# a16z/jolt

Measured on AMD Instinct MI355X. Metric: prover trace cycles/sec (sha3-shaped synthetic trace, sumcheck + HyperKZG hot path), higher is better.
Workload: dtype u256 (BN254 Fr / Fq, 8x u32 Montgomery limbs; integer, bit-exact)

## Files before the change

include/jolt_hip.h:

```cpp
#ifndef JOLT_HIP_H
#define JOLT_HIP_H

#include <stddef.h>
#include <stdint.h>

#ifdef __cplusplus
extern "C" {
#endif

#define JOLT_HIP_ABI_VERSION 1

typedef struct { uint64_t l[4]; } jolt_fr_t;
typedef struct { uint64_t l[4]; } jolt_fq_t;
typedef struct { jolt_fq_t x, y, z; } jolt_g1_t;

typedef struct jolt_ctx jolt_ctx;
typedef struct jolt_table jolt_table;
typedef struct jolt_member jolt_member;
typedef struct jolt_srs jolt_srs;

enum {
    JOLT_OK = 0,
    JOLT_ERR_INVALID_ARG = 1,
    JOLT_ERR_NO_DEVICE = 2,
// ... 297 lines not shown
int32_t jolt_host_lookup_prefix_table(uint32_t prefix, const jolt_fr_t *checkpoints, uint32_t b_len, uint32_t suffix_len, jolt_fr_t *out );
int32_t jolt_host_lookup_table_combine(uint32_t kind, const jolt_fr_t *prefixes, const jolt_fr_t *suffixes, jolt_fr_t *out);
int32_t jolt_host_read_raf_address_create(const jolt_fr_t *gamma, const uint8_t *table_present , int32_t canonical, jolt_read_raf_address **out);
int32_t jolt_host_read_raf_address_destroy(jolt_read_raf_address *h);
int32_t jolt_host_read_raf_address_init_phase(jolt_read_raf_address *h, uint32_t phase, const jolt_fr_t *raf_sums, const jolt_fr_t *suffix_sums);
int32_t jolt_host_read_raf_address_message(jolt_read_raf_address *h, const jolt_fr_t *previous_claim, jolt_fr_t *evals_out );
int32_t jolt_host_read_raf_address_bind(jolt_read_raf_address *h, const jolt_fr_t *challenge, int32_t *phase_done);
int32_t jolt_host_read_raf_address_bind_message(jolt_read_raf_address *h, const jolt_fr_t *challenge, const jolt_fr_t *previous_claim, jolt_fr_t *evals_out );
int32_t jolt_host_read_raf_address_prove_phase(jolt_read_raf_address *h, jolt_fr_t *claim, jolt_round_transcript_fn fn, void *user, jolt_host_transcript *test_transcript,
                                               jolt_fr_t *coeffs_out , jolt_fr_t *challenges_out );
int32_t jolt_host_read_raf_address_v_table(const jolt_read_raf_address *h, uint32_t phase, jolt_fr_t *out );
int32_t jolt_host_read_raf_address_finish(const jolt_read_raf_address *h, jolt_fr_t *table_values , jolt_fr_t *raf_interleaved, jolt_fr_t *raf_identity);

int32_t jolt_r1cs_uniskip_sums(jolt_ctx *ctx, jolt_table *const *inputs, size_t n_inputs, const jolt_table *eq, const jolt_fr_t *a_weights,
                               const jolt_fr_t *b_weights, size_t n_nodes, jolt_fr_t *out);
int32_t jolt_r1cs_materialize(jolt_ctx *ctx, jolt_table *const *inputs, size_t n_inputs, const jolt_fr_t *a_weights, const jolt_fr_t *b_weights,
                              jolt_table **az_out, jolt_table **bz_out);
int32_t jolt_tables_evaluate(jolt_ctx *ctx, jolt_table *const *tables, size_t k, const jolt_fr_t *point, size_t n, jolt_fr_t *out);

int32_t jolt_r1cs_uniskip_sums_small(jolt_ctx *ctx, const jolt_ints *const *inputs, size_t n_inputs, const jolt_table *eq, uint32_t n_streams,
                                     const int64_t *a_weights, const int64_t *b_weights, size_t n_nodes, jolt_fr_t *out);
int32_t jolt_r1cs_materialize_small(jolt_ctx *ctx, const jolt_ints *const *inputs, size_t n_inputs, uint32_t n_streams, const jolt_fr_t *a_weights,
                                    const jolt_fr_t *b_weights, jolt_table **az_out, jolt_table **bz_out);
int32_t jolt_ints_evaluate(jolt_ctx *ctx, const jolt_ints *const *columns, size_t k, const jolt_fr_t *point, size_t n, jolt_fr_t *out);
int32_t jolt_host_small_scalar_dot(const jolt_fr_t *values, const uint64_t *scalars, size_t n, jolt_fr_t *out);

typedef struct jolt_rw_matrix jolt_rw_matrix;
int32_t jolt_rw_matrix_create(jolt_ctx *ctx, const uint64_t *addresses, const uint64_t *pre_values, const uint64_t *post_values, size_t cycles,
                              const jolt_table *inc, const jolt_table *val_init, const jolt_fr_t *tau_low, const jolt_fr_t *gamma,
                              jolt_rw_matrix **out);
int32_t jolt_rw_matrix_create_resident(jolt_ctx *ctx, const jolt_ints *addresses, const jolt_ints *pre_values, const jolt_ints *post_values,
                                       const jolt_table *inc, const jolt_table *val_init, const jolt_fr_t *tau_low, const jolt_fr_t *gamma,
                                       jolt_rw_matrix **out);

int32_t jolt_registers_rw_create(jolt_ctx *ctx, const jolt_onehot *regs, const jolt_ints *rs1_val, const jolt_ints *rs2_val, const jolt_ints *rd_pre,
                                 const jolt_ints *rd_post, const jolt_table *inc, const jolt_fr_t *r_cycle, const jolt_fr_t *gamma, jolt_rw_matrix **out);
int32_t jolt_registers_rw_prove_round(jolt_rw_matrix *m, const jolt_fr_t *bind, jolt_fr_t *evals_out , jolt_fr_t *aux_out );
int32_t jolt_registers_rw_final_values(jolt_rw_matrix *m, jolt_fr_t *out );
int32_t jolt_registers_rw_download(jolt_rw_matrix *m, uint64_t *rows, uint64_t *cols, jolt_fr_t *val, jolt_fr_t *ra, jolt_fr_t *wa, uint64_t *prev, uint64_t *next);
int32_t jolt_rw_matrix_prove_round(jolt_rw_matrix *m, const jolt_fr_t *bind, jolt_fr_t *evals_out , jolt_fr_t *aux_out );
int32_t jolt_rw_matrix_finish(jolt_rw_matrix *m, const jolt_fr_t *bind);
int32_t jolt_rw_matrix_final_values(jolt_rw_matrix *m, jolt_fr_t *out );

typedef struct jolt_key_index jolt_key_index;
int32_t jolt_key_index_create(jolt_ctx *ctx, const jolt_ints *keys, uint64_t k, jolt_key_index **out);
int32_t jolt_key_index_size(const jolt_key_index *index, size_t *cycles, uint64_t *k, uint32_t *items);
int32_t jolt_key_index_pushforward(jolt_ctx *ctx, const jolt_key_index *index, jolt_table *const *weights, size_t n_weights, jolt_table **out);
int32_t jolt_key_index_last_value(jolt_ctx *ctx, const jolt_key_index *index, const jolt_ints *values, const jolt_table *init, jolt_table **out);
int32_t jolt_key_index_destroy(jolt_ctx *ctx, jolt_key_index *index);

int32_t jolt_rw_matrix_hold_row(jolt_rw_matrix *m);
int32_t jolt_rw_matrix_bind(jolt_rw_matrix *m, const jolt_fr_t *bind);
int32_t jolt_rw_matrix_export_row(jolt_rw_matrix *m, size_t cap, uint64_t *cols, uint64_t *prev, uint64_t *next, jolt_fr_t *val, jolt_fr_t *ra, jolt_fr_t *wa ,
                                  jolt_fr_t *inc_out, jolt_fr_t *scalar_out, size_t *n_out);
int32_t jolt_rw_matrix_create_merged(jolt_ctx *ctx, int32_t registers, size_t log_rows, size_t log_k, size_t n, const uint64_t *rows, const uint64_t *cols,
                                     const uint64_t *prev, const uint64_t *next, const jolt_fr_t *val, const jolt_fr_t *ra, const jolt_fr_t *wa, const jolt_fr_t *inc,
                                     const jolt_table *val_init, const jolt_fr_t *w, const jolt_fr_t *scalar, const jolt_fr_t *gamma, jolt_rw_matrix **out);
int32_t jolt_rw_matrix_len(const jolt_rw_matrix *m, size_t *entries);
int32_t jolt_rw_matrix_download(jolt_rw_matrix *m, uint64_t *rows, uint64_t *cols, jolt_fr_t *val, jolt_fr_t *ra, jolt_fr_t *prev, jolt_fr_t *next);
int32_t jolt_rw_matrix_destroy(jolt_rw_matrix *m);

typedef struct jolt_comm jolt_comm;
int32_t jolt_comm_unique_id(const char *rccl_path, uint8_t out[128]);
int32_t jolt_comm_create(jolt_ctx *ctx, const char *rccl_path, const uint8_t unique_id[128], int32_t rank, int32_t world, jolt_comm **out);
int32_t jolt_comm_destroy(jolt_comm *comm);
int32_t jolt_comm_world(const jolt_comm *comm, int32_t *rank, int32_t *world);
int32_t jolt_comm_all_gather_host(jolt_comm *comm, const void *local, size_t bytes, void *gathered);
int32_t jolt_comm_all_gather_device(jolt_comm *comm, const void *d_local, size_t bytes, void *d_gathered);
int32_t jolt_comm_all_gather_table(jolt_comm *comm, const jolt_table *local, size_t n, jolt_table *gathered);
int32_t jolt_comm_gather_round_sums(void *user, const jolt_fr_t *local, size_t count, jolt_fr_t *gathered);
typedef struct jolt_shm jolt_shm;
int32_t jolt_shm_create(const char *name, int32_t rank, int32_t world, size_t max_bytes, jolt_shm **out);
int32_t jolt_shm_create_nonce(const char *name, uint64_t nonce, int32_t rank, int32_t world, size_t max_bytes, jolt_shm **out);
int32_t jolt_shm_destroy(jolt_shm *shm);
int32_t jolt_shm_all_gather(jolt_shm *shm, const void *local, size_t bytes, void *gathered);
int32_t jolt_shm_gather_round_sums(void *user, const jolt_fr_t *local, size_t count, jolt_fr_t *gathered);
int32_t jolt_round_group_pack_tables(jolt_ctx *ctx, jolt_member *const *members, size_t n_members, size_t entries, jolt_table *dst);
int32_t jolt_tail_interleave(jolt_ctx *ctx, const jolt_table *gathered, size_t world, size_t n_tables, size_t entries, jolt_table *dst);
int32_t jolt_round_group_final_values(jolt_ctx *ctx, jolt_member *const *members, size_t n_members, jolt_fr_t *out, size_t capacity);

int32_t jolt_host_hyperkzg_commit(jolt_ctx *ctx, const jolt_srs *srs, const jolt_table *evals, jolt_g1_t *out);
int32_t jolt_host_hyperkzg_open(jolt_ctx *ctx, const jolt_srs *srs, const jolt_table *evals, const jolt_fr_t *point, size_t ell,
                                uint64_t transcript_label, jolt_g1_t *com, jolt_g1_t *w, jolt_fr_t *v, jolt_fr_t *challenges_out);

typedef int32_t (*jolt_open_transcript_fn)(void *user, int32_t phase, const jolt_g1_t *points, size_t n_points, const jolt_fr_t *values, size_t n_values,
                                           jolt_fr_t *challenge_out);
int32_t jolt_host_hyperkzg_open_with_transcript(jolt_ctx *ctx, const jolt_srs *srs, const jolt_table *evals, const jolt_fr_t *point, size_t ell,
                                                jolt_open_transcript_fn fn, void *user, jolt_g1_t *com, jolt_g1_t *w, jolt_fr_t *v, jolt_fr_t *challenges_out);
int32_t jolt_host_hyperkzg_open_with_levels(jolt_ctx *ctx, const jolt_srs *srs, const jolt_table *evals, const jolt_fr_t *point, size_t ell, uint64_t transcript_label,
                                            jolt_open_transcript_fn fn, void *user, const jolt_g1_t *known_levels, size_t n_known, jolt_g1_t *com, jolt_g1_t *w,
                                            jolt_fr_t *v, jolt_fr_t *challenges_out);

int32_t jolt_msm_g1_table_range(jolt_ctx *ctx, const jolt_srs *srs, size_t base_offset, const jolt_table *scalars, size_t scalar_offset,
                                size_t n, jolt_g1_t *out);
enum { JOLT_SCALAR_FR = 3 };
int32_t jolt_msm_g1_window(jolt_ctx *ctx, const jolt_srs *srs, size_t base_offset, int32_t kind, const void *host, size_t n, const jolt_g1_t *acc, jolt_g1_t *out);
int32_t jolt_grid_commit_onehot_range(jolt_ctx *ctx, const jolt_srs *srs, const jolt_onehot *source, size_t cycle_lo, size_t cycle_hi,
                                      jolt_g1_t *out );
int32_t jolt_grid_commit_onehot_classes(jolt_ctx *ctx, const jolt_srs *srs, const jolt_onehot *source, uint32_t shift, jolt_g1_t *out);
int32_t jolt_host_hyperkzg_open_sharded(jolt_ctx *ctx, const jolt_srs *srs, const jolt_table *evals, const jolt_fr_t *point, size_t ell,
                                        uint64_t transcript_label, int32_t rank, int32_t world, jolt_gather_fn gather, void *user,
                                        jolt_g1_t *com, jolt_g1_t *w, jolt_fr_t *v, jolt_fr_t *challenges_out);
int32_t jolt_host_owned_terms(size_t n, size_t block, int32_t rank, int32_t world, size_t *out);
int32_t jolt_srs_setup_from_secret_blocks(jolt_ctx *ctx, const jolt_fr_t *beta, size_t count_global, const jolt_g1_t *g1, size_t block,
                                          int32_t rank, int32_t world, jolt_srs **out);
int32_t jolt_msm_g1_table_blocks(jolt_ctx *ctx, const jolt_srs *srs, const jolt_table *scalars, size_t n, size_t block, int32_t rank,
                                 int32_t world, jolt_g1_t *out);
int32_t jolt_host_hyperkzg_open_sharded_blocks(jolt_ctx *ctx, const jolt_srs *srs, const jolt_table *evals, const jolt_fr_t *point,
                                               size_t ell, uint64_t transcript_label, int32_t rank, int32_t world, size_t block,
                                               jolt_gather_fn gather, void *user, jolt_g1_t *com, jolt_g1_t *w, jolt_fr_t *v,
                                               jolt_fr_t *challenges_out);
int32_t jolt_host_subtree_owned_terms(size_t n, int32_t rank, int32_t world, size_t *out);
int32_t jolt_host_subtree_term_index(size_t slot, int32_t rank, int32_t world, size_t *out);
int32_t jolt_srs_setup_from_secret_subtree(jolt_ctx *ctx, const jolt_fr_t *beta, size_t count_global, const jolt_g1_t *g1, int32_t rank,
                                           int32_t world, jolt_srs **out);
int32_t jolt_msm_g1_table_subtree(jolt_ctx *ctx, const jolt_srs *srs, const jolt_table *scalars, size_t n, int32_t rank, int32_t world,
                                  jolt_g1_t *out);
int32_t jolt_grid_joint_polynomial_subtree(jolt_ctx *ctx, const jolt_onehot *const *sources, size_t n_sources,
                                           const jolt_fr_t *onehot_scalars, jolt_table *const *dense, size_t n_dense,
                                           const jolt_fr_t *dense_scalars, uint32_t log_k, int32_t rank, int32_t world, jolt_table **out);
int32_t jolt_host_hyperkzg_open_subtree(jolt_ctx *ctx, const jolt_srs *srs, const jolt_table *evals, const jolt_fr_t *point, size_t ell,
                                        uint64_t transcript_label, int32_t rank, int32_t world, jolt_gather_fn gather, void *user,
                                        jolt_g1_t *com, jolt_g1_t *w, jolt_fr_t *v, jolt_fr_t *challenges_out);

typedef struct jolt_grid_hint jolt_grid_hint;
int32_t jolt_grid_hint_begin(jolt_ctx *ctx, const jolt_srs *srs, const jolt_onehot *const *sources, size_t n_sources, uint32_t levels, int32_t background,
                             jolt_grid_hint **out);
int32_t jolt_grid_hint_wait(jolt_ctx *ctx, jolt_grid_hint *hint);
int32_t jolt_grid_hint_download(jolt_ctx *ctx, jolt_grid_hint *hint, uint32_t level, jolt_g1_t *out );
int32_t jolt_grid_hint_free(jolt_ctx *ctx, jolt_grid_hint *hint);
int32_t jolt_host_hyperkzg_open_grid(jolt_ctx *ctx, const jolt_srs *srs, const jolt_table *evals, const jolt_fr_t *point, size_t ell, uint64_t transcript_label,
                                     jolt_open_transcript_fn fn, void *user, const jolt_grid_hint *hint, uint32_t levels, const jolt_fr_t *onehot_scalars,
                                     jolt_table *const *dense, size_t n_dense, const jolt_fr_t *dense_scalars, jolt_g1_t *com, jolt_g1_t *w, jolt_fr_t *v,
                                     jolt_fr_t *challenges_out);

typedef struct jolt_stage_op jolt_stage_op;
int32_t jolt_stage_op_num_rounds(const jolt_stage_op *op, size_t *rounds);
int32_t jolt_stage_op_degree(const jolt_stage_op *op, size_t *degree);
int32_t jolt_stage_op_input_claim(jolt_stage_op *op, jolt_fr_t *claim);
int32_t jolt_stage_op_prove_round(jolt_stage_op *op, const jolt_fr_t *bind, size_t round, const jolt_fr_t *previous_claim, jolt_fr_t *coeffs_out, size_t cap,
                                  size_t *n_coeffs);
int32_t jolt_stage_op_finish_rounds(jolt_stage_op *op, const jolt_fr_t *bind);
int32_t jolt_stage_op_output_claims(jolt_stage_op *op, jolt_fr_t *out, size_t cap, size_t *n);
int32_t jolt_stage_op_kept(const jolt_stage_op *op, const char *key, jolt_fr_t *out, size_t cap, size_t *n);
int32_t jolt_stage_op_window(jolt_stage_op *parent, size_t first, size_t n, jolt_stage_op **out);
int32_t jolt_stage_op_destroy(jolt_stage_op *op);

int32_t jolt_stage_spartan_uniskip_sums(jolt_ctx *ctx, const jolt_ints *const *cols, size_t n_cols, uint32_t n_streams, const jolt_fr_t *tau, size_t n_tau,
                                        const int64_t *a_weights, const int64_t *b_weights, size_t n_nodes, jolt_fr_t *sums_out);
int32_t jolt_stage_spartan_remainder_create(jolt_ctx *ctx, const jolt_ints *const *cols, size_t n_cols, uint32_t n_streams, const jolt_fr_t *a_weights,
                                            const jolt_fr_t *b_weights, const jolt_fr_t *tau, size_t n_tau, const jolt_fr_t *scale, jolt_stage_op **out);
int32_t jolt_stage_ram_read_write_create(jolt_ctx *ctx, const jolt_ints *addresses, const jolt_ints *pre_values, const jolt_ints *post_values, const jolt_ints *inc,
                                         const jolt_ints *val_init, const jolt_fr_t *tau_low, const jolt_fr_t *gamma, jolt_stage_op **out);
int32_t jolt_stage_registers_read_write_create(jolt_ctx *ctx, const jolt_onehot *regs, const jolt_ints *rs1_val, const jolt_ints *rs2_val, const jolt_ints *rd_pre,
                                               const jolt_ints *rd_post, const jolt_ints *inc, const jolt_fr_t *r_cycle, const jolt_fr_t *gamma, jolt_stage_op **out);
int32_t jolt_stage_booleanity_address_create(jolt_ctx *ctx, const jolt_onehot *cols, const jolt_fr_t *reference_cycle, size_t n_cycle, const jolt_fr_t *reference_address,
                                             const jolt_fr_t *gamma, jolt_stage_op **out);
int32_t jolt_stage_booleanity_cycle_create(jolt_ctx *ctx, const jolt_onehot *cols, const jolt_fr_t *r_address, const jolt_fr_t *reference_address, const jolt_fr_t *reference_cycle,
                                           size_t n_cycle, const jolt_fr_t *gamma, jolt_stage_op **out);
int32_t jolt_stage_hamming_weight_create(jolt_ctx *ctx, const jolt_onehot *cols, const jolt_fr_t *r_cycle, size_t n_cycle, const jolt_fr_t *r_address,
                                         const jolt_fr_t *virtualization_points, const jolt_fr_t *gamma, jolt_stage_op **out);
int32_t jolt_stage_instruction_read_raf_create(jolt_ctx *ctx, jolt_read_raf *rows, const jolt_onehot *claim_columns, const jolt_fr_t *r_reduction, size_t n_vars,
                                               const jolt_fr_t *gamma, const uint8_t *table_present , uint32_t ra_count, jolt_stage_op **out);
int32_t jolt_stage_bytecode_read_raf_address_create(jolt_ctx *ctx, const jolt_key_index *pc_index, const jolt_fr_t *stage_points , size_t n_vars,
                                                    const jolt_fr_t *stage_values , const jolt_fr_t *gamma, uint64_t first_pc, uint64_t entry_index,
                                                    jolt_stage_op **out);
// ... 22 lines not shown
```

jolt_amd/csrc/capi.hip:

```cpp
#include <algorithm>
#include <chrono>
#include <cstdlib>
#include <type_traits>

#include "host_mirror.hpp"
#include "ints.hpp"
#include "member.hpp"
#include "poly_kernels.hip.h"
#include "small_round.hip.h"
#include "onehot_kernels.hip.h"

using namespace jolt;

extern "C" const char* jolt_status_string(int32_t s) {
    switch (s) {
        case JOLT_OK: return "ok";
        case JOLT_ERR_INVALID_ARG: return "invalid argument";
        case JOLT_ERR_NO_DEVICE: return "no usable gfx950 device";
        case JOLT_ERR_OOM: return "out of device memory";
        case JOLT_ERR_HIP: return "HIP runtime error";
        case JOLT_ERR_SIZE_MISMATCH: return "size mismatch";
        case JOLT_ERR_UNSUPPORTED: return "unsupported descriptor";
        case JOLT_ERR_NOT_FULLY_BOUND: return "member not fully bound";
        case JOLT_ERR_ROUND_CHECK: return "round check failed";
// ... 13 lines not shown

extern "C" int32_t jolt_ctx_create(int32_t device_id, void* stream, jolt_ctx** out) {
    if (!out) return JOLT_ERR_INVALID_ARG;
    *out = nullptr;
    int count = 0;
    if (hipGetDeviceCount(&count) != hipSuccess || count <= 0 || device_id < 0 || device_id >= count) return JOLT_ERR_NO_DEVICE;
    hipDeviceProp_t prop;
    if (hipGetDeviceProperties(&prop, device_id) != hipSuccess) return JOLT_ERR_NO_DEVICE;
    if (std::strncmp(prop.gcnArchName, "gfx950", 6) != 0) return JOLT_ERR_NO_DEVICE;
    if (hipSetDevice(device_id) != hipSuccess) return JOLT_ERR_NO_DEVICE;
    jolt_ctx* ctx = new (std::nothrow) jolt_ctx();
    if (!ctx) return JOLT_ERR_OOM;
    ctx->device = device_id;
    if (const char* fr_ = std::getenv("JOLT_FUSE_RATIO")) ctx->fuse_ratio = (size_t)std::max(0, std::atoi(fr_));
    if (const char* tp = std::getenv("JOLT_TAIL_PAIRS")) { if (std::atoll(tp) > 0) ctx->tail_pairs = (size_t)std::atoll(tp); }
    if (const char* ft = std::getenv("JOLT_FUSE_TAIL")) ctx->fuse_tail = std::atoi(ft) != 0;
    if (const char* rt = std::getenv("JOLT_ROUND_TRACE")) ctx->round_trace = std::atoi(rt) != 0;
    if (const char* gf = std::getenv("JOLT_GRID_FLOOR")) { if (std::atoi(gf) > 0) ctx->grid_floor = (size_t)std::atoi(gf); }
    if (const char* gm = std::getenv("JOLT_GRID_MULT")) { if (std::atoi(gm) > 0) ctx->grid_mult = (size_t)std::atoi(gm); }
    if (const char* ss = std::getenv("JOLT_SERIAL_STREAMS")) ctx->serial_streams = std::atoi(ss) != 0;
    if (const char* ll = std::getenv("JOLT_LAZY_LDS")) ctx->lazy_lds = std::atoi(ll) != 0;
    if (const char* rp = std::getenv("JOLT_UNIFORM_ROWS_PAIRS")) { if (std::atoll(rp) > 0) ctx->uniform_rows_pairs = (size_t)std::atoll(rp); }
    ctx->num_cus = prop.multiProcessorCount > 0 ? prop.multiProcessorCount : 256;
    if (prop.sharedMemPerBlock > 0) ctx->max_lds_per_block = prop.sharedMemPerBlock;
    if (const char* ml = std::getenv("JOLT_MSM_LDS_SORT")) ctx->msm_lds_sort = std::atoi(ml) != 0;
    if (const char* pe = std::getenv("JOLT_POOL")) ctx->pool_enabled = std::atoi(pe) != 0;
    if (const char* la = std::getenv("JOLT_MSM_LANES")) ctx->msm_lanes = std::max(1, std::min(4, std::atoi(la)));
    if (stream) {
        ctx->stream = (hipStream_t)stream;
    } else {
        if (hipStreamCreateWithFlags(&ctx->stream, hipStreamNonBlocking) != hipSuccess) { delete ctx; return JOLT_ERR_HIP; }
        ctx->own_stream = true;
    }
    if (hipEventCreate(&ctx->ev_begin) != hipSuccess || hipEventCreate(&ctx->ev_end) != hipSuccess) { delete ctx; return JOLT_ERR_HIP; }
    int32_t s = jolt_internal_ensure_scratch(ctx, 4096 * 8, 1024);
    if (s == JOLT_OK) {
        ctx->round_cap = 1024;
        if (hipHostMalloc((void**)&ctx->h_round, ctx->round_cap * sizeof(Fr), hipHostMallocMapped | hipHostMallocCoherent) != hipSuccess ||
            hipHostMalloc((void**)&ctx->h_flag, 64, hipHostMallocMapped | hipHostMallocCoherent) != hipSuccess ||
            hipMalloc((void**)&ctx->d_counters, kTicketWords * sizeof(uint32_t)) != hipSuccess ||
            hipMalloc((void**)&ctx->d_round, ctx->round_cap * sizeof(Fr)) != hipSuccess ||
            hipMemset(ctx->d_counters, 0, kTicketWords * sizeof(uint32_t)) != hipSuccess)
            s = JOLT_ERR_HIP;
        else
            *ctx->h_flag = 0;
        for (int k = 0; k < 3 && s == JOLT_OK; ++k)
            if (hipStreamCreateWithFlags(&ctx->side[k], hipStreamNonBlocking) != hipSuccess) s = JOLT_ERR_HIP;
        if (s == JOLT_OK && hipEventCreateWithFlags(&ctx->ev_fork, hipEventDisableTiming) != hipSuccess) s = JOLT_ERR_HIP;
        for (int k = 0; k < 3 && s == JOLT_OK; ++k)
            if (hipEventCreateWithFlags(&ctx->ev_join[k], hipEventDisableTiming) != hipSuccess) s = JOLT_ERR_HIP;
    }
    if (s != JOLT_OK) { jolt_ctx_destroy(ctx); return s; }
    *out = ctx;
    return JOLT_OK;
}


extern "C" int32_t jolt_ctx_destroy(jolt_ctx* ctx) {
    if (!ctx) return JOLT_OK;
    (void)hipSetDevice(ctx->device);
    (void)jolt_internal_join_side_writers(ctx);
    (void)hipStreamSynchronize(ctx->stream);
    for (int k = 0; k < 3; ++k) if (ctx->side[k]) { (void)hipStreamSynchronize(ctx->side[k]); (void)hipStreamDestroy(ctx->side[k]); }
    if (ctx->ev_fork) (void)hipEventDestroy(ctx->ev_fork);
    for (int k = 0; k < 3; ++k) if (ctx->ev_join[k]) (void)hipEventDestroy(ctx->ev_join[k]);
    (void)jolt_internal_pool_trim(ctx);
    for (auto& kv : ctx->pool_live) (void)hipFree(kv.first);
    ctx->pool_live.clear();
    if (ctx->d_partials) (void)hipFree(ctx->d_partials);
    if (ctx->d_results) (void)hipFree(ctx->d_results);
    if (ctx->h_results) (void)hipHostFree(ctx->h_results);
    if (ctx->h_round) (void)hipHostFree(ctx->h_round);
    if (ctx->h_flag) (void)hipHostFree(ctx->h_flag);
    if (ctx->d_counters) (void)hipFree(ctx->d_counters);
    if (ctx->d_round) (void)hipFree(ctx->d_round);
    for (int k = 0; k < 4; ++k) {
        if (ctx->msm_ws[k]) (void)hipFree(ctx->msm_ws[k]);
        if (ctx->msm_host[k]) (void)hipHostFree(ctx->msm_host[k]);
    }
    if (ctx->msm_batch_stream) { (void)hipStreamSynchronize(ctx->msm_batch_stream); (void)hipStreamDestroy(ctx->msm_batch_stream); }
    if (ctx->hint_stream) { (void)hipStreamSynchronize(ctx->hint_stream); (void)hipStreamDestroy(ctx->hint_stream); }
    if (ctx->msm_batch_ws) (void)hipFree(ctx->msm_batch_ws);
    if (ctx->msm_aux_stream) { (void)hipStreamSynchronize(ctx->msm_aux_stream); (void)hipStreamDestroy(ctx->msm_aux_stream); }
    for (auto& pair : ctx->ev_aux) for (hipEvent_t e : pair) if (e) (void)hipEventDestroy(e);
    if (ctx->msm_batch_host) (void)hipHostFree(ctx->msm_batch_host);
    if (ctx->ev_begin) (void)hipEventDestroy(ctx->ev_begin);
    for (hipEvent_t e : ctx->ev_fx)
        if (e) (void)hipEventDestroy(e);
    if (ctx->copy_stream) { (void)hipStreamSynchronize(ctx->copy_stream); (void)hipStreamDestroy(ctx->copy_stream); }
    if (ctx->ev_copy_fork) (void)hipEventDestroy(ctx->ev_copy_fork);
    if (ctx->ev_end) (void)hipEventDestroy(ctx->ev_end);
    if (ctx->own_stream) (void)hipStreamDestroy(ctx->stream);
    delete ctx;
    return JOLT_OK;
}

extern "C" int32_t jolt_ctx_synchronize(jolt_ctx* ctx) {
    if (!ctx) return JOLT_ERR_INVALID_ARG;
    JOLT_TRY(jolt_internal_join_side_writers(ctx));
    for (int k = 0; k < 3; ++k) if (ctx->side[k]) JOLT_HIP_TRY(ctx, hipStreamSynchronize(ctx->side[k]));
    if (ctx->hint_stream) JOLT_HIP_TRY(ctx, hipStreamSynchronize(ctx->hint_stream));
    JOLT_HIP_TRY(ctx, hipStreamSynchronize(ctx->stream));
    return JOLT_OK;
}
extern "C" int32_t jolt_ctx_bind_thread(jolt_ctx* ctx) {
    if (!ctx) return JOLT_ERR_INVALID_ARG;
    JOLT_HIP_TRY(ctx, hipSetDevice(ctx->device));
    return JOLT_OK;
}

extern "C" int32_t jolt_ctx_synchronize_foreground(jolt_ctx* ctx) {
    if (!ctx) return JOLT_ERR_INVALID_ARG;
    JOLT_TRY(jolt_internal_join_side_writers(ctx));
    for (int k = 0; k < 3; ++k) if (ctx->side[k]) JOLT_HIP_TRY(ctx, hipStreamSynchronize(ctx->side[k]));
    JOLT_HIP_TRY(ctx, hipStreamSynchronize(ctx->stream));
    return JOLT_OK;
}
extern "C" const char* jolt_last_error(const jolt_ctx* ctx) { return ctx ? ctx->last_error.c_str() : ""; }

extern "C" int32_t jolt_timer_begin(jolt_ctx* ctx) {
    if (!ctx) return JOLT_ERR_INVALID_ARG;
    JOLT_HIP_TRY(ctx, hipEventRecord(ctx->ev_begin, ctx->stream));
    return JOLT_OK;
}
extern "C" int32_t jolt_timer_end(jolt_ctx* ctx, float* ms) {
    if (!ctx || !ms) return JOLT_ERR_INVALID_ARG;
    JOLT_HIP_TRY(ctx, hipEventRecord(ctx->ev_end, ctx->stream));
    JOLT_HIP_TRY(ctx, hipEventSynchronize(ctx->ev_end));
    JOLT_HIP_TRY(ctx, hipEventElapsedTime(ms, ctx->ev_begin, ctx->ev_end));
    return JOLT_OK;
}

static inline size_t pool_class(size_t bytes) {
    if (bytes <= 4096) return 4096;
    size_t top = (size_t)1 << (63 - __builtin_clzll((unsigned long long)bytes));
    size_t step = top >> 2;
    return (bytes + step - 1) / step * step;
}
int32_t jolt_internal_pool_trim(jolt_ctx* ctx) {
    if (ctx->pool_free.empty()) return JOLT_OK;
    (void)hipDeviceSynchronize();
    for (auto& kv : ctx->pool_free)
        for (void* p : kv.second) (void)hipFree(p);
    ctx->pool_free.clear();
    ctx->pool_cached_bytes = 0;
    return JOLT_OK;
}
int32_t jolt_internal_dev_alloc(jolt_ctx* ctx, size_t bytes, void** out) {
    const size_t cls = pool_class(std::max<size_t>(bytes, 1));
    auto it = ctx->pool_free.find(cls);
    if (it != ctx->pool_free.end() && !it->second.empty()) {
        JOLT_TRY(jolt_internal_join_side_writers(ctx));
        *out = it->second.back();
        it->second.pop_back();
        ctx->pool_cached_bytes -= cls;
    } else {
        void* p = nullptr;
        hipError_t e = hipMalloc(&p, cls);
        if (e == hipErrorOutOfMemory && ctx->pool_cached_bytes) {
            (void)hipGetLastError();
            JOLT_TRY(jolt_internal_pool_trim(ctx));
            e = hipMalloc(&p, cls);
        }
        if (e != hipSuccess) {
            (void)hipGetLastError();
            ctx->last_error = std::string("hipMalloc(") + std::to_string(cls) + "): " + hipGetErrorString(e);
            return e == hipErrorOutOfMemory ? JOLT_ERR_OOM : JOLT_ERR_HIP;
// ... 1841 lines not shown
```

jolt_amd/csrc/ctx.hpp:

```cpp
#pragma once
#include <hip/hip_runtime.h>

#include <cstdio>
#include <cstring>
#include <new>
#include <string>
#include <unordered_map>
#include <vector>

#include "../../include/jolt_hip.h"
#include "field.hip.h"

using jolt::Fq;
using jolt::Fr;

static_assert(sizeof(Fr) == sizeof(jolt_fr_t), "Fr must be layout-compatible with jolt_fr_t");

struct jolt_ctx {
    int device = 0;
    hipStream_t stream = nullptr;
    bool own_stream = false;
    int num_cus = 256;
    size_t max_lds_per_block = 65536;
    std::string last_error;
    Fr* d_partials = nullptr;
    size_t partials_cap = 0;
    Fr* d_results = nullptr;
    Fr* h_results = nullptr;
    size_t results_cap = 0;
    void* d_desc_scratch = nullptr;
    Fr* h_round = nullptr;
    uint64_t* h_flag = nullptr;
    Fr* d_round = nullptr;
    size_t d_round_count = 0;
    uint32_t* d_counters = nullptr;
    uint64_t seq = 0;
    size_t round_cap = 0;
    hipStream_t side[3] = {nullptr, nullptr, nullptr};
    hipEvent_t ev_fork = nullptr;
    hipEvent_t ev_join[3] = {nullptr, nullptr, nullptr};
    bool join_pending[3] = {false, false, false};
    void* msm_ws[4] = {nullptr, nullptr, nullptr, nullptr};
    size_t msm_ws_cap[4] = {0, 0, 0, 0};
    void* msm_host[4] = {nullptr, nullptr, nullptr, nullptr};
    hipStream_t msm_batch_stream = nullptr;
    hipStream_t hint_stream = nullptr;
    void* msm_batch_ws = nullptr;
    size_t msm_batch_ws_cap = 0;
    void* msm_batch_host = nullptr;
    size_t msm_batch_host_cap = 0;
    hipStream_t msm_aux_stream = nullptr;
    hipEvent_t ev_aux[4][2] = {{nullptr, nullptr}, {nullptr, nullptr}, {nullptr, nullptr}, {nullptr, nullptr}};
    bool msm_tables_pending = false;
    void* msm_pending_one = nullptr;
    hipEvent_t ev_begin = nullptr, ev_end = nullptr;
    hipStream_t copy_stream = nullptr;
    hipEvent_t ev_copy_fork = nullptr;
    bool fx_profile = false;
    hipEvent_t ev_fx[2] = {nullptr, nullptr};
    const uint32_t* fx_profile_info = nullptr;
    bool fx_profile_valid = false;
    size_t uniform_rows_pairs = (size_t)1 << 16;
    size_t grid_floor = 3;
    size_t grid_mult = 0;
    size_t fuse_ratio = 2;
    size_t tail_pairs = 16384;
    bool fuse_tail = false;
    bool msm_lds_attr_set = false;
    bool msm_fx_attr_set = false;
    bool grid_hint_attr_set = false;
    bool rows_many_attr_set = false;
    int msm_lanes = 4;
    int msm_fx_partition = 2;
    bool msm_uniform_scalars = false;
    bool msm_full_width_scalars = false;
    bool msm_fx_soa = true;
    bool msm_lds_sort = true;
    bool round_trace = false;
    bool serial_streams = false;
    bool lazy_lds = true;
    bool pool_enabled = true;
    std::unordered_map<void*, size_t> pool_live;
    std::unordered_map<size_t, std::vector<void*>> pool_free;
    size_t pool_cached_bytes = 0, pool_live_bytes = 0, pool_peak_bytes = 0;
};

int32_t jolt_internal_join_side_writers(jolt_ctx* ctx);

struct jolt_table {
    jolt_ctx* ctx = nullptr;
    Fr* buf[2] = {nullptr, nullptr};
    size_t cap[2] = {0, 0};
    int cur = 0;
    size_t len = 0;
    const Fr* view = nullptr;
    size_t view_len = 0;
    const void* ints = nullptr;
    const void* ints_src = nullptr;
    Fr* data() const { return cur < 0 ? const_cast<Fr*>(view) : buf[cur]; }
};

#define JOLT_HIP_TRY(ctx, expr)                                                                       \
    do {                                                                                              \
        hipError_t e_ = (expr);                                                                       \
        if (e_ != hipSuccess) {                                                                       \
            if (ctx) (ctx)->last_error = std::string(#expr) + ": " + hipGetErrorString(e_);           \
            return e_ == hipErrorOutOfMemory ? JOLT_ERR_OOM : JOLT_ERR_HIP;                           \
        }                                                                                             \
    } while (0)

#define JOLT_TRY(expr)                     \
    do {                                   \
        int32_t s_ = (expr);               \
        if (s_ != JOLT_OK) return s_;      \
    } while (0)

#define JOLT_REQUIRE(ctx, cond, msg)                            \
    do {                                                        \
        if (!(cond)) {                                          \
            if (ctx) (ctx)->last_error = (msg);                 \
            return JOLT_ERR_INVALID_ARG;                        \
        }                                                       \
    } while (0)

static inline Fr fr_from_abi(const jolt_fr_t* p) {
    Fr r;
    std::memcpy(&r, p, sizeof(Fr));
    return r;
}
static inline void fr_to_abi(jolt_fr_t* p, const Fr& v) { std::memcpy(p, &v, sizeof(Fr)); }
static inline bool fr_low_limbs_zero(const Fr& v) { return (v.l[0] | v.l[1] | v.l[2] | v.l[3]) == 0; }
static inline bool fr_is_canonical(const Fr& v) {
    Fr d;
    return jolt::sub_p(d, v) != 0;
}

int32_t jolt_internal_dev_alloc(jolt_ctx* ctx, size_t bytes, void** out);
// ... 6 lines not shown
```

jolt_amd/csrc/hyperkzg.hip:

```cpp
#include <algorithm>
#include <cstdlib>

#include "ctx.hpp"
#include "g1.hip.h"
#include "grid_hint.hpp"
#include "host_mirror.hpp"
#include "poly_kernels.hip.h"
#include "srs.hpp"
#include "term_map.hip.h"

using namespace jolt;

int32_t jolt_internal_msm(jolt_ctx* ctx, const jolt_srs* srs, const Fr* d_scalars, size_t n, G1Jac* out);
int32_t jolt_internal_msm_pair_and_one(jolt_ctx* ctx, const jolt_srs* srs, const Fr* d_a, size_t n_a, size_t shift, const Fr* d_b, size_t n_b, G1Jac* out);
int32_t jolt_internal_msm_one_begin(jolt_ctx* ctx, const jolt_srs* srs, size_t n_a, size_t shift, const Fr* d_b, size_t n_b);
int32_t jolt_internal_msm_pair_finish(jolt_ctx* ctx, const jolt_srs* srs, const Fr* d_a, size_t n_a, size_t shift, G1Jac* out);
void jolt_internal_msm_one_abandon(jolt_ctx* ctx);
int32_t jolt_internal_msm_many(jolt_ctx* ctx, const jolt_srs* srs, const Fr* const* d_scalars, const size_t* n, size_t count, G1Jac* out,
                               const size_t* base_offsets = nullptr);

namespace {

constexpr int kHornerChunk = 16;

struct Fr3 {
    Fr v[3];
};

static __global__ __launch_bounds__(kBlock) void k_power_table3(Fr3 base, Fr* __restrict__ table) {
#pragma unroll
    for (int t = 0; t < 3; ++t) {
        Fr w = Fr::one(), b = base.v[t];
        for (unsigned e = threadIdx.x; e; e >>= 1) {
            if (e & 1) w = mul(w, b);
            b = sqr(b);
        }
        st_fr(table + t * kBlock + threadIdx.x, w);
    }
}
__device__ __forceinline__ Fr fr_pow_u64(Fr b, uint64_t e) {
    Fr w = Fr::one();
    for (; e; e >>= 1) {
        if (e & 1) w = mul(w, b);
        b = sqr(b);
    }
    return w;
}
template <bool SUBTREE>
static __global__ __launch_bounds__(kBlock) void k_horner3(const Fr* __restrict__ c, size_t n, Fr3 u, const Fr* __restrict__ chunk_weights ,
                                                           Fr3 u_block , Fr* __restrict__ partials, TermMap map) {
    __shared__ Fr block_weight[3];
    if (threadIdx.x < 3) {
        if (SUBTREE) block_weight[threadIdx.x] = blockIdx.x ? fr_pow_u64(u.v[threadIdx.x], term_global(map, (size_t)blockIdx.x * kBlock * kHornerChunk)) : Fr::one();
        else block_weight[threadIdx.x] = fr_pow_u64(u_block.v[threadIdx.x], blockIdx.x);
    }
    size_t base = ((size_t)blockIdx.x * kBlock + threadIdx.x) * kHornerChunk;
    Fr acc[3] = {Fr::zero(), Fr::zero(), Fr::zero()};
    if (base < n) {
        size_t end = base + kHornerChunk < n ? base + kHornerChunk : n;
        if (SUBTREE && base == 0) {
            for (size_t i = base; i < end; ++i) {
                Fr ci = ld_fr(c + i);
                const uint64_t e = term_global(map, i);
#pragma unroll
                for (int t = 0; t < 3; ++t) acc[t] = add(acc[t], mul(ci, fr_pow_u64(u.v[t], e)));
            }
        } else {
            for (size_t i = end; i-- > base;) {
                Fr ci = ld_fr(c + i);
#pragma unroll
                for (int t = 0; t < 3; ++t) acc[t] = add(mul(acc[t], u.v[t]), ci);
            }
        }
    }
    __syncthreads();
    if (base < n) {
        if (SUBTREE && blockIdx.x == 0) {
            if (base) {
                const uint64_t e = term_global(map, base);
#pragma unroll
                for (int t = 0; t < 3; ++t) acc[t] = mul(acc[t], fr_pow_u64(u.v[t], e));
            }
        } else {
#pragma unroll
            for (int t = 0; t < 3; ++t) acc[t] = mul(mul(acc[t], ld_fr(chunk_weights + t * kBlock + threadIdx.x)), block_weight[t]);
        }
    }
    block_reduce_store<3>(acc, partials);
}

template <bool PLUS_MINUS>
static __global__ __launch_bounds__(kBlock) void k_horner3_strided(const Fr* __restrict__ c, size_t n, Fr3 u256, const Fr* __restrict__ lane_weights ,
                                                                   Fr3 u_block , Fr* __restrict__ partials) {
    __shared__ Fr block_weight[3];
    if (threadIdx.x < 3) block_weight[threadIdx.x] = fr_pow_u64(u_block.v[threadIdx.x], blockIdx.x);
    const size_t base = (size_t)blockIdx.x * kBlock * kHornerChunk + threadIdx.x;
    Fr ci[kHornerChunk];
#pragma unroll
    for (int e = 0; e < kHornerChunk; ++e) {
        const size_t i = base + (size_t)e * kBlock;
// ... 199 lines not shown
    if (!ctx || !f || !u || !out) return JOLT_ERR_INVALID_ARG;
    Fr uu = fr_from_abi(u);
    JOLT_REQUIRE(ctx, fr_is_canonical(uu), "u is not a canonical Fr");
    size_t d = f->len;
    jolt_table* h = nullptr;
    JOLT_TRY(jolt_internal_table_new(ctx, d > 1 ? d - 1 : 0, &h));
    if (d > 1) {
        int32_t s = suffix_horner(ctx, f->data(), d, uu, h->data(), 1);
        if (s != JOLT_OK) { jolt_table_free(ctx, h); return s; }
    }
    *out = h;
    return JOLT_OK;
}

using namespace jolt_host;

static void append_g1(Transcript& tr, const G1Jac& p) {
    uint8_t b[32];
    jolt_g1_t abi;
    std::memcpy(&abi, &p, sizeof(abi));
    jolt_host_g1_serialize_compressed(&abi, b);
    tr.append_bytes(b, 32);
}

extern "C" int32_t jolt_host_hyperkzg_commit(jolt_ctx* ctx, const jolt_srs* srs, const jolt_table* evals, jolt_g1_t* out) {
    if (!ctx || !srs || !evals || !out) return JOLT_ERR_INVALID_ARG;
    G1Jac r;
    JOLT_TRY(jolt_internal_msm(ctx, srs, evals->data(), evals->len, &r));
    std::memcpy(out, &r, sizeof(r));
    return JOLT_OK;
}

int32_t jolt_internal_gather_owned_terms(jolt_ctx* ctx, const Fr* src, size_t n, const TermMap& map, Fr* dst);
namespace {
int32_t gather_with_status(jolt_ctx* ctx, jolt_gather_fn gather, void* user, int32_t local_status, const jolt_fr_t* payload, size_t count, int world, std::vector<jolt_fr_t>* all);
}
static int32_t sharded_msm_many(jolt_ctx* ctx, const jolt_srs* srs, const std::vector<const Fr*>& ptrs, const std::vector<size_t>& lens, int rank, int world,
                                size_t block, jolt_gather_fn gather, void* user, G1Jac* out) {
    const size_t count = ptrs.size();
    if (count == 0) return JOLT_OK;
    if (world <= 1) return jolt_internal_msm_many(ctx, srs, ptrs.data(), lens.data(), count, out);
    std::vector<const Fr*> p(count);
    std::vector<size_t> n(count), off(count);
    std::vector<G1Jac> partial(count), all((size_t)world * count);
    int32_t ls = JOLT_OK;
    if (block) {
        TermMap map;
        if (!make_block_map(block, rank, world, &map)) return JOLT_ERR_INVALID_ARG;
        size_t total = 0;
        for (size_t i = 0; i < count; ++i) {
            n[i] = term_owned(map, lens[i]);
            if (n[i] > srs->n && ls == JOLT_OK) ls = JOLT_ERR_SRS_TOO_SMALL;
            off[i] = total;
            total += n[i];
        }
        Fr* compact = nullptr;
        int32_t s = ls;
        if (s == JOLT_OK) s = jolt_internal_dev_alloc(ctx, std::max<size_t>(total, 1) * sizeof(Fr), (void**)&compact);
        for (size_t i = 0; i < count && s == JOLT_OK; ++i) {
            s = jolt_internal_gather_owned_terms(ctx, ptrs[i], lens[i], map, compact + off[i]);
            p[i] = compact + off[i];
        }
        if (s == JOLT_OK) s = jolt_internal_msm_many(ctx, srs, p.data(), n.data(), count, partial.data());
        if (compact) jolt_internal_dev_free(ctx, compact);
        ls = s;
    } else {
        for (size_t i = 0; i < count; ++i) {
            const size_t lo = lens[i] * (size_t)rank / (size_t)world, hi = lens[i] * (size_t)(rank + 1) / (size_t)world;
            p[i] = ptrs[i] + lo;
            n[i] = hi - lo;
            off[i] = lo;
        }
        ls = jolt_internal_msm_many(ctx, srs, p.data(), n.data(), count, partial.data(), off.data());
    }
    static_assert(sizeof(G1Jac) == 3 * sizeof(jolt_fr_t), "a Jacobian point travels as three 32-byte words");
    std::vector<jolt_fr_t> raw;
    JOLT_TRY(gather_with_status(ctx, gather, user, ls, reinterpret_cast<const jolt_fr_t*>(partial.data()), 3 * count, world, &raw));
    std::memcpy(all.data(), raw.data(), raw.size() * sizeof(jolt_fr_t));
    for (size_t i = 0; i < count; ++i) {
        G1Jac acc = all[i];
        for (int r = 1; r < world; ++r) acc = g1_add(acc, all[(size_t)r * count + i]);
        out[i] = acc;
    }
    return JOLT_OK;
}

namespace {
struct OpenTranscript {
    LabelledTranscript mock;
    jolt_open_transcript_fn fn;
    void* user;
    int32_t after_points(int32_t phase, const G1Jac* pts, size_t n, Fr* out) {
        if (!fn) {
            for (size_t i = 0; i < n; ++i) append_g1(mock, pts[i]);
            *out = mock.challenge();
            return JOLT_OK;
        }
        static_assert(sizeof(G1Jac) == sizeof(jolt_g1_t), "a Jacobian point crosses the ABI as it lies in memory");
        jolt_fr_t ch;
        JOLT_TRY(fn(user, phase, reinterpret_cast<const jolt_g1_t*>(pts), n, nullptr, 0, &ch));
        *out = fr_from_abi(&ch);
        return fr_is_canonical(*out) ? JOLT_OK : JOLT_ERR_INVALID_ARG;
    }
    int32_t after_values(int32_t phase, const jolt_fr_t* vals, size_t n, Fr* out) {
        if (!fn) {
            for (size_t i = 0; i < n; ++i) mock.append_fr(fr_from_abi(&vals[i]));
            *out = mock.challenge();
            return JOLT_OK;
        }
        jolt_fr_t ch;
        JOLT_TRY(fn(user, phase, nullptr, 0, vals, n, &ch));
        *out = fr_from_abi(&ch);
        return fr_is_canonical(*out) ? JOLT_OK : JOLT_ERR_INVALID_ARG;
    }
};
}

namespace {
struct GridLinear {
    const jolt_grid_hint* hint;
    const jolt_fr_t* onehot_scalars;
    jolt_table* const* dense;
    size_t n_dense;
    const jolt_fr_t* dense_scalars;
    uint32_t levels;
};
}

static int32_t hyperkzg_open_impl(jolt_ctx* ctx, const jolt_srs* srs, const jolt_table* evals, const jolt_fr_t* point, size_t ell, uint64_t transcript_label,
                                  int rank, int world, size_t block, jolt_gather_fn gather, void* user, jolt_g1_t* com, jolt_g1_t* w, jolt_fr_t* v, jolt_fr_t* challenges_out,
                                  jolt_open_transcript_fn transcript_fn = nullptr, void* transcript_user = nullptr, const jolt_g1_t* known_levels = nullptr, size_t n_known = 0,
                                  const GridLinear* lin = nullptr) {
    if (!ctx || !srs || !evals || !point || !w || !v || (ell > 1 && !com)) return JOLT_ERR_INVALID_ARG;
    if (world < 1 || rank < 0 || rank >= world || (world > 1 && !gather)) return JOLT_ERR_INVALID_ARG;
    if (ell == 0) return JOLT_ERR_EMPTY_POINT;
    if (ell > 40) return JOLT_ERR_UNSUPPORTED;
    OpenTranscript tr{LabelledTranscript(transcript_label), transcript_fn, transcript_user};
    std::vector<jolt_table*> polys(ell, nullptr);
    auto cleanup = [&](jolt_table* extra1 = nullptr, jolt_table* extra2 = nullptr) {
        for (jolt_table* t : polys) if (t) jolt_table_free(ctx, t);
        if (extra1) jolt_table_free(ctx, extra1);
        if (extra2) jolt_table_free(ctx, extra2);
    };
    int32_t s = jolt_hyperkzg_fold(ctx, evals, point, ell, polys.data());
    if (s != JOLT_OK) { cleanup(); return s; }
    std::vector<G1Jac> coms(ell > 1 ? ell - 1 : 0);
    {
        if (n_known > coms.size() || (n_known && !known_levels) || (n_known && world != 1)) { cleanup(); return JOLT_ERR_INVALID_ARG; }
        for (size_t i = 0; i < n_known; ++i) {
            std::memcpy(&coms[i], &known_levels[i], sizeof(G1Jac));
            if (!g1_is_on_curve(coms[i])) {
                ctx->last_error = "a supplied level commitment is not a point of BN254 G1 (coordinates not canonical or off the curve)";
                cleanup();
                return JOLT_ERR_INVALID_ARG;
            }
        }
        size_t n_lin = 0;
        G1Jac* d_small = nullptr;
        void* d_temp = nullptr;
        std::vector<jolt_table*> dense_levels;
        jolt_table* dense_rlc = nullptr;
        auto lin_cleanup = [&]() {
            if (d_small) jolt_internal_dev_free(ctx, d_small);
            if (d_temp) jolt_internal_dev_free(ctx, d_temp);
            for (jolt_table* t : dense_levels) if (t) jolt_table_free(ctx, t);
            if (dense_rlc) jolt_table_free(ctx, dense_rlc);
            d_small = nullptr;
            d_temp = nullptr;
            dense_levels.clear();
            dense_rlc = nullptr;
        };
        if (lin && lin->hint && world == 1 && n_known == 0) {
            const jolt_grid_hint* h = lin->hint;
            size_t log_t = 0;
            while (((size_t)1 << log_t) < h->cycles) ++log_t;
            n_lin = std::min<size_t>({(size_t)lin->levels, (size_t)h->levels, coms.size(), log_t ? log_t - 1 : 0});
            if ((size_t)h->k * h->cycles != evals->len || (lin->n_dense && (!lin->dense || !lin->dense_scalars)) || !lin->onehot_scalars) { cleanup(); return JOLT_ERR_INVALID_ARG; }
            if (n_lin) {
                std::vector<Fr> sc(h->n_cols), xs(n_lin);
                for (size_t p = 0; p < h->n_cols; ++p) sc[p] = fr_from_abi(&lin->onehot_scalars[p]);
                for (size_t b = 0; b < n_lin; ++b) xs[b] = fr_from_abi(&point[ell - 1 - b]);
                s = jolt_internal_grid_hint_combine(ctx, h, (uint32_t)n_lin, sc.data(), xs.data(), &d_small, &d_temp);
                if (s == JOLT_OK && lin->n_dense) {
                    for (size_t dd = 0; dd < lin->n_dense && s == JOLT_OK; ++dd)
                        if (!lin->dense[dd] || lin->dense[dd]->len != h->cycles) s = JOLT_ERR_SIZE_MISMATCH;
                    if (s == JOLT_OK) s = jolt_rlc(ctx, lin->dense, lin->n_dense, lin->dense_scalars, &dense_rlc);
                    if (s == JOLT_OK) {
                        dense_levels.assign(log_t, nullptr);
                        s = jolt_hyperkzg_fold(ctx, dense_rlc, point + (ell - log_t), log_t, dense_levels.data());
                    }
                }
                if (s != JOLT_OK) { lin_cleanup(); cleanup(); return s; }
            }
        }
        const size_t first_msm = std::max(n_known, n_lin);
        std::vector<const Fr*> ptrs;
        std::vector<size_t> lens;
        for (size_t i = 1 + first_msm; i < ell; ++i) { ptrs.push_back(polys[i]->data()); lens.push_back(polys[i]->len); }
        const size_t n_level_msms = ptrs.size();
        if (n_lin && dense_rlc)
            for (size_t s_ = 1; s_ <= n_lin; ++s_) { ptrs.push_back(dense_levels[s_]->data()); lens.push_back(dense_levels[s_]->len); }
        std::vector<G1Jac> msm_out(ptrs.size());
        ctx->msm_full_width_scalars = true;
        s = ptrs.empty() ? JOLT_OK : sharded_msm_many(ctx, srs, ptrs, lens, rank, world, block, gather, user, msm_out.data());
        ctx->msm_full_width_scalars = false;
        if (s == JOLT_OK && n_lin) {
            std::vector<G1Jac> small(n_lin);
            hipError_t e = hipMemcpyAsync(small.data(), d_small, n_lin * sizeof(G1Jac), hipMemcpyDeviceToHost, lin->hint->stream);
            if (e == hipSuccess) e = hipStreamSynchronize(lin->hint->stream);
            if (e != hipSuccess) { (void)hipGetLastError(); ctx->last_error = std::string("hyperkzg open (levels by linearity): ") + hipGetErrorString(e); s = JOLT_ERR_HIP; }
            for (size_t i = 0; i < n_lin && s == JOLT_OK; ++i) coms[i] = dense_rlc ? g1_add(small[i], msm_out[n_level_msms + i]) : small[i];
        } else if (n_lin) {
            (void)hipStreamSynchronize(lin->hint->stream);
        }
        for (size_t i = 0; i < n_level_msms && s == JOLT_OK; ++i) coms[first_msm + i] = msm_out[i];
        lin_cleanup();
        if (s != JOLT_OK) { cleanup(); return s; }
    }
    Fr r;
    s = tr.after_points(0, coms.data(), coms.size(), &r);
    if (s != JOLT_OK) { cleanup(); return s; }
    Fr u[3] = {r, neg(r), mul(r, r)};
    jolt_fr_t u_abi[3];
    for (int t = 0; t < 3; ++t) fr_to_abi(&u_abi[t], u[t]);
    s = jolt_hyperkzg_eval3(ctx, polys.data(), ell, u_abi, v);
    if (s != JOLT_OK) { cleanup(); return s; }
    Fr q;
    s = tr.after_values(1, v, 3 * ell, &q);
    if (s != JOLT_OK) { cleanup(); return s; }
    jolt_fr_t q_abi;
    fr_to_abi(&q_abi, q);
    jolt_table* b_poly = nullptr;
    s = jolt_hyperkzg_rlc(ctx, polys.data(), ell, &q_abi, &b_poly);
    if (s != JOLT_OK) { cleanup(); return s; }
    G1Jac ws[3];
    bool paired = false;
    if (world == 1 && b_poly->len >= 4) {
        jolt_table *h0 = nullptr, *qp = nullptr, *h2 = nullptr;
        bool direct = false, begun = false;
        s = jolt_hyperkzg_witness_poly(ctx, b_poly, &u_abi[2], &h2);
        if (s == JOLT_OK) {
            ctx->msm_full_width_scalars = ctx->msm_uniform_scalars = true;
            const int32_t bs = jolt_internal_msm_one_begin(ctx, srs, b_poly->len - 2, 1, h2->data(), h2->len);
            ctx->msm_full_width_scalars = ctx->msm_uniform_scalars = false;
            if (bs == JOLT_OK) begun = true;
            else if (bs != JOLT_ERR_UNSUPPORTED) s = bs;
        }
        if (s == JOLT_OK && b_poly->len % 2 == 0) {
            s = jolt_internal_table_new(ctx, b_poly->len - 2, &qp);
            if (s == JOLT_OK) {
                const int32_t qs = suffix_scan<2>(ctx, b_poly->data(), b_poly->len, u[2], qp->data(), 2, Fr::zero());
                if (qs == JOLT_OK) direct = true;
                else if (qs == JOLT_ERR_UNSUPPORTED) { jolt_table_free(ctx, qp); qp = nullptr; }
                else s = qs;
            }
        }
        if (s == JOLT_OK && !direct) {
            s = jolt_hyperkzg_witness_poly(ctx, b_poly, &u_abi[0], &h0);
            if (s == JOLT_OK) s = jolt_hyperkzg_witness_poly(ctx, h0, &u_abi[1], &qp);
        }
        Fr a_lo, q_lo;
        G1Affine g0;
        if (s == JOLT_OK) {
            hipError_t e = hipMemcpyAsync(&a_lo, direct ? b_poly->data() + 1 : h0->data(), sizeof(Fr), hipMemcpyDeviceToHost, ctx->stream);
            if (e == hipSuccess) e = hipMemcpyAsync(&q_lo, direct ? qp->data() + 1 : qp->data(), sizeof(Fr), hipMemcpyDeviceToHost, ctx->stream);
            if (e == hipSuccess) e = hipMemcpyAsync(&g0, srs->pts, sizeof(G1Affine), hipMemcpyDeviceToHost, ctx->stream);
            if (e == hipSuccess) e = hipStreamSynchronize(ctx->stream);
            if (e != hipSuccess) { ctx->last_error = std::string("hyperkzg open: ") + hipGetErrorString(e); s = JOLT_ERR_HIP; }
        }
        if (s == JOLT_OK) {
            G1Jac three[3];
            ctx->msm_full_width_scalars = ctx->msm_uniform_scalars = true;
            const int32_t ps = begun ? jolt_internal_msm_pair_finish(ctx, srs, qp->data(), qp->len, 1, three)
                                     : jolt_internal_msm_pair_and_one(ctx, srs, qp->data(), qp->len, 1, h2->data(), h2->len, three);
            ctx->msm_full_width_scalars = ctx->msm_uniform_scalars = false;
            begun = false;
            if (ps == JOLT_OK) {
                const Fr alpha = direct ? add(a_lo, mul(q_lo, u[2])) : add(a_lo, mul(q_lo, u[1])), r_can = from_mont(r), a_can = from_mont(alpha);
                const G1Jac r_cq = g1_mul_canonical(three[0], r_can.l), base = g1_add(three[1], g1_mul_canonical(g1_from_affine(g0), a_can.l));
                ws[0] = g1_add(base, r_cq);
                ws[1] = g1_add(base, g1_neg(r_cq));
                ws[2] = three[2];
                paired = true;
            } else if (ps != JOLT_ERR_UNSUPPORTED) {
                s = ps;
            }
        }
        if (begun) jolt_internal_msm_one_abandon(ctx);
        for (jolt_table* t : {h0, qp, h2}) if (t) jolt_table_free(ctx, t);
        if (s != JOLT_OK) { cleanup(b_poly); return s; }
    }
    if (!paired) {
        jolt_table* h[3] = {nullptr, nullptr, nullptr};
        std::vector<const Fr*> ptrs;
        std::vector<size_t> lens;
        for (int t = 0; t < 3 && s == JOLT_OK; ++t) {
            s = jolt_hyperkzg_witness_poly(ctx, b_poly, &u_abi[t], &h[t]);
            if (s == JOLT_OK) { ptrs.push_back(h[t]->data()); lens.push_back(h[t]->len); }
        }
        if (s == JOLT_OK) s = sharded_msm_many(ctx, srs, ptrs, lens, rank, world, block, gather, user, ws);
        for (int t = 0; t < 3; ++t) if (h[t]) jolt_table_free(ctx, h[t]);
        if (s != JOLT_OK) { cleanup(b_poly); return s; }
    }
    Fr d0;
    s = tr.after_points(2, ws, 3, &d0);
    if (s != JOLT_OK) { cleanup(b_poly); return s; }
    for (size_t i = 0; i + 1 < ell; ++i) std::memcpy(&com[i], &coms[i], sizeof(G1Jac));
    for (int t = 0; t < 3; ++t) std::memcpy(&w[t], &ws[t], sizeof(G1Jac));
    if (challenges_out) { fr_to_abi(&challenges_out[0], r); fr_to_abi(&challenges_out[1], q); fr_to_abi(&challenges_out[2], d0); }
    cleanup(b_poly);
    return JOLT_OK;
}

namespace {
int32_t read_slot(jolt_ctx* ctx, const jolt_table* t, size_t slot, Fr* out) {
    JOLT_HIP_TRY(ctx, hipMemcpyAsync(out, t->data() + slot, sizeof(Fr), hipMemcpyDeviceToHost, ctx->stream));
    return JOLT_OK;
}
int32_t write_slot(jolt_ctx* ctx, Fr* dst, const Fr& v) {
    JOLT_HIP_TRY(ctx, hipMemcpyAsync(dst, &v, sizeof(Fr), hipMemcpyHostToDevice, ctx->stream));
    return JOLT_OK;
}
int32_t gather_with_status(jolt_ctx* ctx, jolt_gather_fn gather, void* user, int32_t local_status, const jolt_fr_t* payload, size_t count, int world, std::vector<jolt_fr_t>* all) {
    std::vector<jolt_fr_t> send(count + 1), recv((count + 1) * (size_t)world);
    std::memset(send.data(), 0, send.size() * sizeof(jolt_fr_t));
    send[0].l[0] = (uint64_t)(uint32_t)local_status;
    if (local_status == JOLT_OK && count) std::memcpy(&send[1], payload, count * sizeof(jolt_fr_t));
    ctx->d_round_count = 0;
    const int32_t gs = gather(user, send.data(), count + 1, recv.data());
    if (gs != JOLT_OK) return gs;
    all->resize(count * (size_t)world);
    int32_t first = JOLT_OK;
    for (int r = 0; r < world; ++r) {
        const int32_t st = (int32_t)(uint32_t)recv[(size_t)r * (count + 1)].l[0];
        if (st != JOLT_OK && first == JOLT_OK) first = st;
        if (count) std::memcpy(all->data() + (size_t)r * count, &recv[(size_t)r * (count + 1) + 1], count * sizeof(jolt_fr_t));
    }
    return local_status != JOLT_OK ? local_status : first;
}
int32_t gather_words(jolt_ctx* ctx, jolt_gather_fn gather, void* user, int32_t local_status, const std::vector<Fr>& local, int world, std::vector<Fr>* all) {
    std::vector<jolt_fr_t> raw;
    JOLT_TRY(gather_with_status(ctx, gather, user, local_status, reinterpret_cast<const jolt_fr_t*>(local.data()), local.size(), world, &raw));
    all->resize(raw.size());
    if (!raw.empty()) std::memcpy(all->data(), raw.data(), raw.size() * sizeof(jolt_fr_t));
    return JOLT_OK;
}
int32_t gather_points(jolt_ctx* ctx, jolt_gather_fn gather, void* user, int32_t local_status, const std::vector<G1Jac>& partial, int world, G1Jac* out) {
    const size_t count = partial.size();
    std::vector<jolt_fr_t> raw;
    JOLT_TRY(gather_with_status(ctx, gather, user, local_status, reinterpret_cast<const jolt_fr_t*>(partial.data()), 3 * count, world, &raw));
    const G1Jac* all = reinterpret_cast<const G1Jac*>(raw.data());
    for (size_t i = 0; i < count; ++i) {
        G1Jac acc = all[i];
        for (int r = 1; r < world; ++r) acc = g1_add(acc, all[(size_t)r * count + i]);
        out[i] = acc;
    }
    return JOLT_OK;
}
}

extern "C" int32_t jolt_host_hyperkzg_open_subtree(jolt_ctx* ctx, const jolt_srs* srs, const jolt_table* evals, const jolt_fr_t* point, size_t ell,
                                                   uint64_t transcript_label, int32_t rank, int32_t world, jolt_gather_fn gather, void* user, jolt_g1_t* com,
                                                   jolt_g1_t* w, jolt_fr_t* v, jolt_fr_t* challenges_out) {
    if (!ctx || !srs || !evals || !point || !w || !v || !gather || (ell > 1 && !com)) return JOLT_ERR_INVALID_ARG;
    TermMap map;
    if (world < 2 || !make_subtree_map(rank, world, &map)) return JOLT_ERR_INVALID_ARG;
    if (ell > 40) return JOLT_ERR_UNSUPPORTED;
    const size_t gamma = map.gamma, G = (size_t)world;
    if (ell <= gamma) return JOLT_ERR_UNSUPPORTED;
    const size_t lam = ell - gamma;
    if (evals->len != ((size_t)1 << lam)) return JOLT_ERR_SIZE_MISMATCH;
    if (srs->n < evals->len) return JOLT_ERR_SRS_TOO_SMALL;
// ... 231 lines not shown
```

jolt_amd/csrc/msm.hip:

```cpp
#include <algorithm>
#include <cstring>
#include <vector>

#include "ctx.hpp"
#include "msm_kernels.hip.h"
#include "srs.hpp"
#include "term_map.hip.h"

using namespace jolt;
using namespace jolt::msmk;

static_assert(sizeof(G1Jac) == sizeof(jolt_g1_t), "G1Jac must be layout-compatible with jolt_g1_t");

namespace {

__global__ __launch_bounds__(kBlock) void k_jac_to_affine(const G1Jac* __restrict__ in, G1Affine* __restrict__ out, size_t n) {
    size_t i = (size_t)blockIdx.x * kBlock + threadIdx.x;
    if (i < n) out[i] = g1_to_affine(in[i]);
}
__global__ __launch_bounds__(kBlock) void k_affine_to_jac(const G1Affine* __restrict__ in, G1Jac* __restrict__ out, size_t n) {
    size_t i = (size_t)blockIdx.x * kBlock + threadIdx.x;
    if (i < n) out[i] = g1_from_affine(in[i]);
}

__global__ __launch_bounds__(kBlock) void k_srs_powers(Fr beta, G1Jac g, G1Affine* __restrict__ out, size_t n, TermMap map) {
    size_t i = (size_t)blockIdx.x * kBlock + threadIdx.x;
    if (i >= n) return;
    const size_t exponent = term_global(map, i);
    Fr acc = Fr::one(), base = beta;
    for (size_t e = exponent; e; e >>= 1) {
        if (e & 1) acc = mul(acc, base);
        base = sqr(base);
    }
    Fr k = from_mont(acc);
    out[i] = g1_to_affine(g1_mul_canonical(g, k.l));
}

}
struct MsmJob {
    size_t n = 0;
    int lane = 0, c = 0, W = 0;
    uint32_t nb = 0;
    int results = 1;
};
int32_t jolt_internal_msm_fixed_enqueue(jolt_ctx* ctx, const jolt_srs* srs, const Fr* d_scalars, size_t n, int lane, MsmJob* job, size_t pair_shift = 0);
namespace {
struct MsmPlan {
    int c, W, L;
    uint32_t B, G, nb, heavy_threshold;
};
MsmPlan plan_for(size_t n) {
    int lg = 0;
    while (((size_t)2 << lg) <= n) lg++;
    MsmPlan p;
    p.c = std::max(2, std::min(16, lg - 4));
    p.W = (255 + p.c - 1) / p.c;
    p.B = 1u << (p.c - 1);
    uint32_t threads = std::min<uint32_t>(p.B, 4096);
    p.nb = (threads + kBlock - 1) / kBlock;
    p.G = (p.B + p.nb * kBlock - 1) / (p.nb * kBlock);
    size_t wb = (size_t)p.W * p.B;
    p.L = 1;
    while (p.L < 64 && wb * (size_t)(2 * p.L) <= 524288) p.L *= 2;
    size_t avg = (n + (size_t)p.B - 1) / (size_t)p.B;
    p.heavy_threshold = (uint32_t)std::min<size_t>((size_t)p.L * std::max<size_t>(kLaneCap, 4 * avg), 0x7FFFFFFFu);
    return p;
}

}

extern "C" int32_t jolt_srs_upload_g1(jolt_ctx* ctx, const jolt_g1_t* bases, size_t n, jolt_srs** out) {
    if (!ctx || !out || (!bases && n)) return JOLT_ERR_INVALID_ARG;
    jolt_srs* s = new (std::nothrow) jolt_srs();
    if (!s) return JOLT_ERR_OOM;
    s->ctx = ctx;
    s->n = n;
    G1Jac* tmp = nullptr;
    hipError_t e = hipMalloc((void**)&s->pts, std::max<size_t>(n, 1) * sizeof(G1Affine));
    if (e == hipSuccess && n) e = hipMalloc((void**)&tmp, n * sizeof(G1Jac));
    if (e == hipSuccess && n) e = hipMemcpyAsync(tmp, bases, n * sizeof(G1Jac), hipMemcpyHostToDevice, ctx->stream);
    if (e == hipSuccess && n) {
        hipLaunchKernelGGL(k_jac_to_affine, dim3((unsigned)((n + kBlock - 1) / kBlock)), dim3(kBlock), 0, ctx->stream, (const G1Jac*)tmp, s->pts, n);
        e = hipGetLastError();
    }
    if (e == hipSuccess) e = hipStreamSynchronize(ctx->stream);
    if (tmp) (void)hipFree(tmp);
    if (e != hipSuccess) {
        ctx->last_error = std::string("srs upload: ") + hipGetErrorString(e);
        if (s->pts) (void)hipFree(s->pts);
        delete s;
        return e == hipErrorOutOfMemory ? JOLT_ERR_OOM : JOLT_ERR_HIP;
    }
    *out = s;
    return JOLT_OK;
}

static int32_t srs_setup_impl(jolt_ctx* ctx, const jolt_fr_t* beta, size_t count, const jolt_g1_t* g1, const TermMap& map, jolt_srs** out);
extern "C" int32_t jolt_srs_setup_from_secret(jolt_ctx* ctx, const jolt_fr_t* beta, size_t count, const jolt_g1_t* g1, jolt_srs** out) {
    return srs_setup_impl(ctx, beta, count, g1, TermMap{}, out);
}
extern "C" int32_t jolt_srs_setup_from_secret_blocks(jolt_ctx* ctx, const jolt_fr_t* beta, size_t count_global, const jolt_g1_t* g1, size_t block, int32_t rank,
                                                     int32_t world, jolt_srs** out) {
    TermMap m;
    if (!make_block_map(block, rank, world, &m)) return JOLT_ERR_INVALID_ARG;
    if (count_global % (block * (size_t)world) != 0) return JOLT_ERR_SIZE_MISMATCH;
    return srs_setup_impl(ctx, beta, count_global / (size_t)world, g1, m, out);
}
extern "C" int32_t jolt_srs_setup_from_secret_subtree(jolt_ctx* ctx, const jolt_fr_t* beta, size_t count_global, const jolt_g1_t* g1, int32_t rank, int32_t world,
                                                      jolt_srs** out) {
    TermMap m;
    if (!make_subtree_map(rank, world, &m)) return JOLT_ERR_INVALID_ARG;
    if (count_global < (size_t)world || (count_global & (count_global - 1)) != 0) return JOLT_ERR_SIZE_MISMATCH;
    return srs_setup_impl(ctx, beta, count_global / (size_t)world, g1, m, out);
}
static int32_t srs_setup_impl(jolt_ctx* ctx, const jolt_fr_t* beta, size_t count, const jolt_g1_t* g1, const TermMap& map, jolt_srs** out) {
    if (!ctx || !beta || !g1 || !out) return JOLT_ERR_INVALID_ARG;
    Fr b = fr_from_abi(beta);
    JOLT_REQUIRE(ctx, fr_is_canonical(b), "beta is not a canonical Fr");
    G1Jac g;
    std::memcpy(&g, g1, sizeof(g));
    jolt_srs* s = new (std::nothrow) jolt_srs();
    if (!s) return JOLT_ERR_OOM;
    s->ctx = ctx;
    s->n = count;
    hipError_t e = hipMalloc((void**)&s->pts, std::max<size_t>(count, 1) * sizeof(G1Affine));
    if (e == hipSuccess && count) {
        hipLaunchKernelGGL(k_srs_powers, dim3((unsigned)((count + kBlock - 1) / kBlock)), dim3(kBlock), 0, ctx->stream, b, g, s->pts, count, map);
        e = hipGetLastError();
// ... 77 lines not shown
            ctx->msm_ws_cap[lane] = 0;
        }
        JOLT_HIP_TRY(ctx, hipMalloc(&ctx->msm_ws[lane], off));
        ctx->msm_ws_cap[lane] = off;
    }
    if (!ctx->msm_host[lane]) JOLT_HIP_TRY(ctx, hipHostMalloc(&ctx->msm_host[lane], kMsmHostEntries * sizeof(G1Jac), hipHostMallocDefault));
    if ((size_t)p.W > kMsmHostEntries) return JOLT_ERR_UNSUPPORTED;
    char* ws = (char*)ctx->msm_ws[lane];
    uint32_t* keys = (uint32_t*)(ws + o_keys);
    uint32_t* sorted = (uint32_t*)(ws + o_sorted);
    uint32_t* hist = (uint32_t*)(ws + o_hist);
    uint32_t* offs = (uint32_t*)(ws + o_offs);
    uint32_t* cur = (uint32_t*)(ws + o_cur);
    uint32_t* heavy = (uint32_t*)(ws + o_heavy);
    uint32_t* hcnt = (uint32_t*)(ws + o_hcnt);
    G1Jac* buckets = (G1Jac*)(ws + o_buckets);
    G1Jac* part = (G1Jac*)(ws + o_part);
    G1Jac* seg = (G1Jac*)(ws + o_seg);
    G1Jac* wsum = (G1Jac*)(ws + o_wsum);
    hipError_t e = hipMemsetAsync(hist, 0, WB * 4, st);
    if (e == hipSuccess) e = hipMemsetAsync(hcnt, 0, 256, st);
    if (e == hipSuccess) e = hipMemsetAsync(buckets, 0, WB * sizeof(G1Jac), st);
    if (e == hipSuccess) {
        unsigned gn = (unsigned)((n + kBlock - 1) / kBlock);
        unsigned gh = std::min<uint32_t>((heavy_cap + 3) / 4, 4096);
        const size_t lds_bytes = ((size_t)p.B + 1) * sizeof(uint32_t);
        const bool lds_sort = ctx->msm_lds_sort && n >= ((size_t)1 << 16) && lds_bytes <= ctx->max_lds_per_block;
        const unsigned slices = (unsigned)std::max<size_t>(1, std::min<size_t>((size_t)ctx->num_cus / p.W, n / 8192));
        if (lds_sort && !ctx->msm_lds_attr_set) {
            hipError_t a1 = hipFuncSetAttribute((const void*)k_msm_hist_lds, hipFuncAttributeMaxDynamicSharedMemorySize, (int)ctx->max_lds_per_block);
            hipError_t a2 = hipFuncSetAttribute((const void*)k_msm_scatter_lds, hipFuncAttributeMaxDynamicSharedMemorySize, (int)ctx->max_lds_per_block);
            if (a1 != hipSuccess || a2 != hipSuccess) {
                (void)hipGetLastError();
                ctx->msm_lds_sort = false;
            }
            ctx->msm_lds_attr_set = true;
        }
        const bool use_lds_sort = lds_sort && ctx->msm_lds_sort;
        if (use_lds_sort) {
            hipLaunchKernelGGL(k_msm_digits, dim3(gn), dim3(kBlock), 0, st, d_scalars, n, p.c, p.W, keys, (uint32_t*)nullptr);
            hipLaunchKernelGGL(k_msm_hist_lds, dim3(slices, p.W), dim3(kSortBlock), lds_bytes, st, (const uint32_t*)keys, n, p.B, hist);
        } else {
            hipLaunchKernelGGL(k_msm_digits, dim3(gn), dim3(kBlock), 0, st, d_scalars, n, p.c, p.W, keys, hist);
        }
        hipLaunchKernelGGL(k_msm_scan, dim3(p.W), dim3(kBlock), 0, st, (const uint32_t*)hist, offs, cur, p.B, p.heavy_threshold, heavy, hcnt, heavy_cap);
        if (use_lds_sort) hipLaunchKernelGGL(k_msm_scatter_lds, dim3(slices, p.W), dim3(kSortBlock), lds_bytes, st, (const uint32_t*)keys, n, p.B, cur, sorted);
        else hipLaunchKernelGGL(k_msm_scatter, dim3(gn, p.W), dim3(kBlock), 0, st, (const uint32_t*)keys, n, p.B, cur, sorted, (size_t)p.W);
        hipLaunchKernelGGL(k_msm_buckets_light<true>, dim3((unsigned)(((size_t)p.B * p.L + kBlock - 1) / kBlock), p.W), dim3(kBlock), 0, st, (const uint32_t*)hist,
                           (const uint32_t*)offs, (const uint32_t*)sorted, (const G1Affine*)srs->pts, n, p.B, p.L, p.heavy_threshold, buckets, (size_t)p.W);
        hipLaunchKernelGGL(k_msm_buckets_heavy<false>, dim3(gh), dim3(kBlock), 0, st, (const uint32_t*)heavy, (const uint32_t*)hcnt, (const uint32_t*)hist,
                           (const uint32_t*)offs, (const uint32_t*)sorted, (const G1Affine*)srs->pts, n, p.B, seg, LformConsts{});
        hipLaunchKernelGGL(k_msm_heavy_combine, dim3(gh), dim3(kBlock), 0, st, (const uint32_t*)heavy, (const uint32_t*)hcnt, (const uint32_t*)hist,
                           (const G1Jac*)seg, buckets);
        hipLaunchKernelGGL(k_msm_window_reduce, dim3(p.nb, p.W), dim3(kBlock), 0, st, (const G1Jac*)buckets, p.B, p.G, part);
        hipLaunchKernelGGL(k_msm_window_combine, dim3(p.W), dim3(64), 0, st, (const G1Jac*)part, p.nb, wsum);
        e = hipGetLastError();
    }
    if (e == hipSuccess) e = hipMemcpyAsync(ctx->msm_host[lane], wsum, (size_t)p.W * sizeof(G1Jac), hipMemcpyDeviceToHost, st);
    if (e != hipSuccess) {
        ctx->last_error = std::string("msm: ") + hipGetErrorString(e);
        return e == hipErrorOutOfMemory ? JOLT_ERR_OOM : JOLT_ERR_HIP;
    }
    return JOLT_OK;
}

int32_t jolt_internal_msm_collect(jolt_ctx* ctx, const MsmJob* job, G1Jac* out) {
    if (job->n == 0) {
        for (int r = 0; r < job->results; ++r) out[r] = g1_identity();
        return JOLT_OK;
    }
    hipStream_t st = job->lane == 0 ? ctx->stream : ctx->side[job->lane - 1];
    JOLT_HIP_TRY(ctx, hipStreamSynchronize(st));
    for (int r = 0; r < job->results; ++r) {
        const G1Jac* wsum = (const G1Jac*)ctx->msm_host[job->lane] + (size_t)r * job->W;
        G1Jac acc = g1_identity();
        for (int w = job->W - 1; w >= 0; --w) {
            for (int k = 0; k < job->c; ++k) acc = g1_double(acc);
            acc = g1_add(acc, wsum[w]);
        }
        out[r] = acc;
    }
    return JOLT_OK;
}
int32_t jolt_internal_msm_enqueue_pair(jolt_ctx* ctx, const jolt_srs* srs, const Fr* d_scalars, size_t n, size_t shift, int lane, MsmJob* job) {
    job->n = n;
    job->lane = lane;
    job->results = 2;
    if (shift > srs->n || n > srs->n - shift) return JOLT_ERR_SRS_TOO_SMALL;
    if (n == 0) return JOLT_OK;
    if (n >= ((size_t)1 << 31)) return JOLT_ERR_UNSUPPORTED;
    if (!(srs->pre && n >= srs->pre_min_n)) return JOLT_ERR_UNSUPPORTED;
    return jolt_internal_msm_fixed_enqueue(ctx, srs, d_scalars, n, lane, job, shift);
}

extern "C" int32_t jolt_host_owned_terms(size_t n, size_t block, int32_t rank, int32_t world, size_t* out) {
    TermMap m;
    if (!out || !make_block_map(block, rank, world, &m)) return JOLT_ERR_INVALID_ARG;
    *out = term_owned(m, n);
    return JOLT_OK;
}
extern "C" int32_t jolt_host_subtree_owned_terms(size_t n, int32_t rank, int32_t world, size_t* out) {
    TermMap m;
    if (!out || !make_subtree_map(rank, world, &m)) return JOLT_ERR_INVALID_ARG;
    *out = term_owned(m, n);
    return JOLT_OK;
}
extern "C" int32_t jolt_host_subtree_term_index(size_t slot, int32_t rank, int32_t world, size_t* out) {
    TermMap m;
    if (!out || !make_subtree_map(rank, world, &m)) return JOLT_ERR_INVALID_ARG;
    *out = term_global(m, slot);
    return JOLT_OK;
}
namespace {
__global__ __launch_bounds__(kBlock) void k_gather_owned_terms(const Fr* __restrict__ src, Fr* __restrict__ dst, size_t len, TermMap map) {
    const size_t j = (size_t)blockIdx.x * kBlock + threadIdx.x;
    if (j >= len) return;
    dst[j] = src[term_global(map, j)];
}
}
int32_t jolt_internal_gather_owned_terms(jolt_ctx* ctx, const Fr* src, size_t n, const TermMap& map, Fr* dst) {
    const size_t len = term_owned(map, n);
    if (!len) return JOLT_OK;
    hipLaunchKernelGGL(k_gather_owned_terms, dim3((unsigned)((len + kBlock - 1) / kBlock)), dim3(kBlock), 0, ctx->stream, src, dst, len, map);
    JOLT_HIP_TRY(ctx, hipGetLastError());
    return JOLT_OK;
}

int32_t jolt_internal_msm(jolt_ctx* ctx, const jolt_srs* srs, const Fr* d_scalars, size_t n, G1Jac* out) {
    MsmJob job;
    if (ctx->msm_tables_pending) { ctx->last_error = "an MSM while jolt_msm_g1_tables_begin's MSMs are in flight (finish them first)"; return JOLT_ERR_INVALID_ARG; }
    JOLT_TRY(jolt_internal_msm_enqueue(ctx, srs, d_scalars, n, 0, &job));
    return jolt_internal_msm_collect(ctx, &job, out);
}

constexpr int kBatchMax = 32;
constexpr size_t kBatchMaxLen = (size_t)1 << 18;
struct BatchScalars {
    const Fr* ptr[kBatchMax];
    uint32_t len[kBatchMax];
};
struct MsmBatchJob {
    int count = 0, c = 0, W = 0;
    bool queued = false;
};
namespace {
__global__ __launch_bounds__(kBlock) void k_msm_digits_batch(BatchScalars b, size_t N, int c, int W, uint32_t* __restrict__ keys) {
    const size_t i = (size_t)blockIdx.x * kBlock + threadIdx.x;
    const uint32_t j = blockIdx.y;
    if (i >= N) return;
    const bool live = i < b.len[j];
    Fr s = live ? from_mont(ld_fr(b.ptr[j] + i)) : Fr::zero();
    const uint32_t B = 1u << (c - 1);
    uint32_t carry = 0;
    for (int w = 0; w < W; ++w) {
        const int bit = w * c;
        uint32_t raw = 0;
        if (bit < 256) {
            const int limb = bit >> 5, off = bit & 31;
            const uint64_t two = (uint64_t)s.l[limb] | (limb + 1 < 8 ? (uint64_t)s.l[limb + 1] << 32 : 0ull);
            raw = (uint32_t)(two >> off) & ((1u << c) - 1);
        }
        raw += carry;
        uint32_t mag, negf;
        if (raw > B) { mag = (1u << c) - raw; negf = 1; carry = 1; }
        else { mag = raw; negf = 0; carry = 0; }
        keys[((size_t)j * W + w) * N + i] = mag | (negf << 31);
    }
}
}
static int32_t msm_batch_enqueue(jolt_ctx* ctx, const jolt_srs* srs, const Fr* const* d_scalars, const size_t* n, const int* members, int count, MsmBatchJob* job) {
    job->count = count;
    job->queued = false;
    if (count == 0) return JOLT_OK;
    size_t N = 0;
    BatchScalars bs;
// ... 35 lines not shown
             *heavy = (uint32_t*)(ws + o_heavy), *hcnt = (uint32_t*)(ws + o_hcnt);
    G1Jac *buckets = (G1Jac*)(ws + o_buckets), *part = (G1Jac*)(ws + o_part), *seg = (G1Jac*)(ws + o_seg), *wsum = (G1Jac*)(ws + o_wsum);
    JOLT_HIP_TRY(ctx, hipStreamWaitEvent(st, ctx->ev_fork, 0));
    JOLT_HIP_TRY(ctx, hipMemsetAsync(hist, 0, WB * 4, st));
    JOLT_HIP_TRY(ctx, hipMemsetAsync(hcnt, 0, 256, st));
    JOLT_HIP_TRY(ctx, hipMemsetAsync(buckets, 0, WB * sizeof(G1Jac), st));
    const unsigned gn = (unsigned)((N + kBlock - 1) / kBlock), gh = std::min<uint32_t>((heavy_cap + 3) / 4, 4096);
    hipLaunchKernelGGL(k_msm_digits_batch, dim3(gn, count), dim3(kBlock), 0, st, bs, N, c, W, keys);
    const size_t lds_bytes = ((size_t)B + 1) * sizeof(uint32_t);
    hipLaunchKernelGGL(k_msm_hist_lds, dim3(1, Wv), dim3(kSortBlock), lds_bytes, st, (const uint32_t*)keys, N, B, hist);
    hipLaunchKernelGGL(k_msm_scan, dim3(Wv), dim3(kBlock), 0, st, (const uint32_t*)hist, offs, cur, B, heavy_threshold, heavy, hcnt, heavy_cap);
    hipLaunchKernelGGL(k_msm_scatter_lds, dim3(1, Wv), dim3(kSortBlock), lds_bytes, st, (const uint32_t*)keys, N, B, cur, sorted);
    hipLaunchKernelGGL(k_msm_buckets_light<true>, dim3((unsigned)(((size_t)B + kBlock - 1) / kBlock), Wv), dim3(kBlock), 0, st, (const uint32_t*)hist, (const uint32_t*)offs,
                       (const uint32_t*)sorted, (const G1Affine*)srs->pts, N, B, 1, heavy_threshold, buckets, (size_t)Wv);
    hipLaunchKernelGGL(k_msm_buckets_heavy<false>, dim3(gh), dim3(kBlock), 0, st, (const uint32_t*)heavy, (const uint32_t*)hcnt, (const uint32_t*)hist, (const uint32_t*)offs,
                       (const uint32_t*)sorted, (const G1Affine*)srs->pts, N, B, seg, LformConsts{});
    hipLaunchKernelGGL(k_msm_heavy_combine, dim3(gh), dim3(kBlock), 0, st, (const uint32_t*)heavy, (const uint32_t*)hcnt, (const uint32_t*)hist, (const G1Jac*)seg, buckets);
    hipLaunchKernelGGL(k_msm_window_reduce, dim3(nb, Wv), dim3(kBlock), 0, st, (const G1Jac*)buckets, B, G, part);
    hipLaunchKernelGGL(k_msm_window_combine, dim3(Wv), dim3(64), 0, st, (const G1Jac*)part, nb, wsum);
    JOLT_HIP_TRY(ctx, hipGetLastError());
    JOLT_HIP_TRY(ctx, hipMemcpyAsync(ctx->msm_batch_host, wsum, (size_t)Wv * sizeof(G1Jac), hipMemcpyDeviceToHost, st));
    job->c = c;
    job->W = W;
    job->queued = true;
    return JOLT_OK;
}
static int32_t msm_batch_collect(jolt_ctx* ctx, const MsmBatchJob* job, const int* members, G1Jac* out) {
    if (!job->queued) return JOLT_OK;
    JOLT_HIP_TRY(ctx, hipStreamSynchronize(ctx->msm_batch_stream));
    for (int k = 0; k < job->count; ++k) {
        const G1Jac* wsum = (const G1Jac*)ctx->msm_batch_host + (size_t)k * job->W;
        G1Jac acc = g1_identity();
        for (int w = job->W - 1; w >= 0; --w) {
            for (int d = 0; d < job->c; ++d) acc = g1_double(acc);
            acc = g1_add(acc, wsum[w]);
        }
        out[members[k]] = acc;
    }
    return JOLT_OK;
}

int32_t jolt_internal_msm_many(jolt_ctx* ctx, const jolt_srs* srs, const Fr* const* d_scalars, const size_t* n, size_t count, G1Jac* out,
                               const size_t* base_offsets ) {
    if (count == 0) return JOLT_OK;
    if (ctx->msm_tables_pending) { ctx->last_error = "MSMs while jolt_msm_g1_tables_begin's MSMs are in flight (finish them first)"; return JOLT_ERR_INVALID_ARG; }
    JOLT_HIP_TRY(ctx, hipEventRecord(ctx->ev_fork, ctx->stream));
    for (int k = 0; k < 3; ++k) JOLT_HIP_TRY(ctx, hipStreamWaitEvent(ctx->side[k], ctx->ev_fork, 0));
    MsmJob jobs[4];
    int32_t status = JOLT_OK;
    const size_t L = (size_t)ctx->msm_lanes;
    int members[kBatchMax], n_members = 0;
    std::vector<size_t> rest;
    for (size_t i = 0; i < count; ++i) {
        const bool prefix = !base_offsets || base_offsets[i] == 0;
        if (prefix && n[i] >= 2 && n[i] <= kBatchMaxLen && n[i] <= srs->n && n_members < kBatchMax) members[n_members++] = (int)i;
        else rest.push_back(i);
    }
    if (n_members < 2) {
        rest.clear();
        for (size_t i = 0; i < count; ++i) rest.push_back(i);
        n_members = 0;
    }
    MsmBatchJob batch;
    if (n_members) status = msm_batch_enqueue(ctx, srs, d_scalars, n, members, n_members, &batch);
    const size_t R = rest.size();
    for (size_t k = 0; k < R + L; ++k) {
        int lane = (int)(k % L);
        if (k == R && status == JOLT_OK && n_members) status = msm_batch_collect(ctx, &batch, members, out);
        if (k >= L && k - L < R && status == JOLT_OK) status = jolt_internal_msm_collect(ctx, &jobs[lane], &out[rest[k - L]]);
        if (k < R && status == JOLT_OK) {
            const size_t i = rest[k];
            if (base_offsets && base_offsets[i] + n[i] > srs->n) status = JOLT_ERR_SRS_TOO_SMALL;
            const jolt_srs view = jolt_srs_range_view(*srs, base_offsets && status == JOLT_OK ? base_offsets[i] : 0);
            if (status == JOLT_OK) status = jolt_internal_msm_enqueue(ctx, &view, d_scalars[i], n[i], lane, &jobs[lane]);
        }
    }
    if (status != JOLT_OK) {
        for (int k = 0; k < 3; ++k) (void)hipStreamSynchronize(ctx->side[k]);
        if (ctx->msm_batch_stream) (void)hipStreamSynchronize(ctx->msm_batch_stream);
    }
    return status;
}

int32_t jolt_internal_msm_pair_and_one(jolt_ctx* ctx, const jolt_srs* srs, const Fr* d_a, size_t n_a, size_t shift, const Fr* d_b, size_t n_b, G1Jac* out) {
    if (shift > srs->n || n_a > srs->n - shift) return JOLT_ERR_SRS_TOO_SMALL;
    if (n_a == 0 || !(srs->pre && n_a >= srs->pre_min_n) || ctx->msm_tables_pending) return JOLT_ERR_UNSUPPORTED;
    JOLT_HIP_TRY(ctx, hipEventRecord(ctx->ev_fork, ctx->stream));
    for (int k = 0; k < 3; ++k) JOLT_HIP_TRY(ctx, hipStreamWaitEvent(ctx->side[k], ctx->ev_fork, 0));
    MsmJob pair, one;
    int32_t status = jolt_internal_msm_enqueue_pair(ctx, srs, d_a, n_a, shift, 0, &pair);
    if (status == JOLT_ERR_UNSUPPORTED) return status;
    const int lane_b = ctx->msm_lanes > 1 ? 1 : 0;
    if (status == JOLT_OK && lane_b == 0) status = jolt_internal_msm_collect(ctx, &pair, out);
    if (status == JOLT_OK) status = jolt_internal_msm_enqueue(ctx, srs, d_b, n_b, lane_b, &one);
    if (status == JOLT_OK && lane_b != 0) status = jolt_internal_msm_collect(ctx, &pair, out);
    if (status == JOLT_OK) status = jolt_internal_msm_collect(ctx, &one, out + 2);
    if (status != JOLT_OK)
        for (int k = 0; k < 3; ++k) (void)hipStreamSynchronize(ctx->side[k]);
    return status;
}

struct MsmPendingOne {
    MsmJob job;
};
int32_t jolt_internal_msm_one_begin(jolt_ctx* ctx, const jolt_srs* srs, size_t n_a, size_t shift, const Fr* d_b, size_t n_b) {
    if (shift > srs->n || n_a > srs->n - shift) return JOLT_ERR_SRS_TOO_SMALL;
    if (n_a == 0 || !(srs->pre && n_a >= srs->pre_min_n) || ctx->msm_lanes < 2 || ctx->msm_pending_one || ctx->msm_tables_pending) return JOLT_ERR_UNSUPPORTED;
    if ((size_t)srs->pre_W * n_a >= ((size_t)1 << 32)) return JOLT_ERR_UNSUPPORTED;
    MsmPendingOne* p = new (std::nothrow) MsmPendingOne();
    if (!p) return JOLT_ERR_OOM;
    int32_t status = JOLT_OK;
    hipError_t e = hipEventRecord(ctx->ev_fork, ctx->stream);
    if (e == hipSuccess) e = hipStreamWaitEvent(ctx->side[0], ctx->ev_fork, 0);
    if (e != hipSuccess) { ctx->last_error = hipGetErrorString(e); status = JOLT_ERR_HIP; }
    if (status == JOLT_OK) status = jolt_internal_msm_enqueue(ctx, srs, d_b, n_b, 1, &p->job);
    if (status != JOLT_OK) { (void)hipStreamSynchronize(ctx->side[0]); delete p; return status; }
    ctx->msm_pending_one = p;
    return JOLT_OK;
}
int32_t jolt_internal_msm_pair_finish(jolt_ctx* ctx, const jolt_srs* srs, const Fr* d_a, size_t n_a, size_t shift, G1Jac* out) {
    MsmPendingOne* p = static_cast<MsmPendingOne*>(ctx->msm_pending_one);
    if (!p) return JOLT_ERR_INVALID_ARG;
    ctx->msm_pending_one = nullptr;
    MsmJob pair;
    int32_t status = jolt_internal_msm_enqueue_pair(ctx, srs, d_a, n_a, shift, 0, &pair);
    if (status == JOLT_OK) status = jolt_internal_msm_collect(ctx, &pair, out);
    else if (status == JOLT_ERR_UNSUPPORTED) {
        status = jolt_internal_msm(ctx, srs, d_a, n_a, &out[0]);
        const jolt_srs view = jolt_srs_range_view(*srs, shift);
        if (status == JOLT_OK) status = jolt_internal_msm(ctx, &view, d_a, n_a, &out[1]);
    }
    const int32_t one_status = jolt_internal_msm_collect(ctx, &p->job, out + 2);
    delete p;
    if (status != JOLT_OK) (void)hipStreamSynchronize(ctx->side[0]);
    return status != JOLT_OK ? status : one_status;
}
void jolt_internal_msm_one_abandon(jolt_ctx* ctx) {
    MsmPendingOne* p = static_cast<MsmPendingOne*>(ctx->msm_pending_one);
    if (!p) return;
    ctx->msm_pending_one = nullptr;
    (void)hipStreamSynchronize(ctx->side[0]);
    delete p;
}

struct jolt_msm_pending {
    int count = 0;
    MsmJob jobs[3];
};
extern "C" int32_t jolt_msm_g1_tables_begin(jolt_ctx* ctx, const jolt_srs* srs, const jolt_table* const* scalars, const size_t* n, size_t count, jolt_msm_pending** out) {
    if (!ctx || !srs || !scalars || !n || !out || count == 0) return JOLT_ERR_INVALID_ARG;
    *out = nullptr;
    if (count > 3 || (size_t)ctx->msm_lanes < count + 1 || ctx->msm_tables_pending || ctx->msm_pending_one) return JOLT_ERR_UNSUPPORTED;
    for (size_t i = 0; i < count; ++i) {
        if (!scalars[i]) return JOLT_ERR_INVALID_ARG;
        if (n[i] > scalars[i]->len) return JOLT_ERR_SIZE_MISMATCH;
        if (n[i] > srs->n) return JOLT_ERR_SRS_TOO_SMALL;
    }
    JOLT_TRY(jolt_internal_join_side_writers(ctx));
    jolt_msm_pending* p = new (std::nothrow) jolt_msm_pending();
    if (!p) return JOLT_ERR_OOM;
    int32_t status = JOLT_OK;
    hipError_t e = hipEventRecord(ctx->ev_fork, ctx->stream);
    for (size_t i = 0; i < count && e == hipSuccess; ++i) e = hipStreamWaitEvent(ctx->side[i], ctx->ev_fork, 0);
    if (e != hipSuccess) { ctx->last_error = hipGetErrorString(e); status = JOLT_ERR_HIP; }
    for (size_t i = 0; i < count && status == JOLT_OK; ++i) {
        status = jolt_internal_msm_enqueue(ctx, srs, scalars[i]->data(), n[i], (int)i + 1, &p->jobs[i]);
        if (status == JOLT_OK) p->count = (int)i + 1;
    }
    if (status != JOLT_OK) {
        for (int k = 0; k < 3; ++k) (void)hipStreamSynchronize(ctx->side[k]);
        delete p;
        return status;
    }
    ctx->msm_tables_pending = true;
    *out = p;
    return JOLT_OK;
}
extern "C" int32_t jolt_msm_g1_tables_finish(jolt_ctx* ctx, jolt_msm_pending* p, jolt_g1_t* out) {
    if (!ctx || !p) return JOLT_ERR_INVALID_ARG;
    int32_t status = JOLT_OK;
    for (int i = 0; i < p->count; ++i) {
        G1Jac r;
        const int32_t s = jolt_internal_msm_collect(ctx, &p->jobs[i], &r);
        if (s == JOLT_OK && out) std::memcpy(&out[i], &r, sizeof(r));
        if (status == JOLT_OK) status = s;
    }
    ctx->msm_tables_pending = false;
    delete p;
    if (status == JOLT_OK && !out) status = JOLT_ERR_INVALID_ARG;
    return status;
}

extern "C" int32_t jolt_msm_g1_table(jolt_ctx* ctx, const jolt_srs* srs, const jolt_table* scalars, size_t n, jolt_g1_t* out) {
    if (!ctx || !srs || !scalars || !out) return JOLT_ERR_INVALID_ARG;
    if (n > scalars->len) return JOLT_ERR_SIZE_MISMATCH;
    G1Jac r;
    JOLT_TRY(jolt_internal_msm(ctx, srs, scalars->data(), n, &r));
    std::memcpy(out, &r, sizeof(r));
    return JOLT_OK;
}

extern "C" int32_t jolt_msm_g1_table_full_width(jolt_ctx* ctx, const jolt_srs* srs, const jolt_table* scalars, size_t n, jolt_g1_t* out) {
    if (!ctx) return JOLT_ERR_INVALID_ARG;
    ctx->msm_full_width_scalars = ctx->msm_uniform_scalars = true;
    const int32_t s = jolt_msm_g1_table(ctx, srs, scalars, n, out);
    ctx->msm_full_width_scalars = ctx->msm_uniform_scalars = false;
    return s;
}

extern "C" int32_t jolt_msm_g1_table_range(jolt_ctx* ctx, const jolt_srs* srs, size_t base_offset, const jolt_table* scalars, size_t scalar_offset, size_t n,
                                           jolt_g1_t* out) {
    if (!ctx || !srs || !scalars || !out) return JOLT_ERR_INVALID_ARG;
    if (n > scalars->len || scalar_offset > scalars->len - n) return JOLT_ERR_SIZE_MISMATCH;
    if (n > srs->n || base_offset > srs->n - n) return JOLT_ERR_SRS_TOO_SMALL;
    const jolt_srs view = jolt_srs_range_view(*srs, base_offset);
    G1Jac r;
    JOLT_TRY(jolt_internal_msm(ctx, &view, scalars->data() + scalar_offset, n, &r));
    std::memcpy(out, &r, sizeof(r));
    return JOLT_OK;
}

extern "C" int32_t jolt_msm_g1_window(jolt_ctx* ctx, const jolt_srs* srs, size_t base_offset, int32_t kind, const void* host, size_t n, const jolt_g1_t* acc, jolt_g1_t* out) {
    if (!ctx || !srs || !out || (!host && n)) return JOLT_ERR_INVALID_ARG;
    if (kind != JOLT_SCALAR_FR && kind != JOLT_INT_U64 && kind != JOLT_INT_I64 && kind != JOLT_INT_I128) return JOLT_ERR_INVALID_ARG;
    if (n > srs->n || base_offset > srs->n - n) return JOLT_ERR_SRS_TOO_SMALL;
    G1Jac sum = g1_identity();
    if (acc) std::memcpy(&sum, acc, sizeof(sum));
    if (n) {
        jolt_table* t = nullptr;
        if (kind == JOLT_SCALAR_FR) {
            JOLT_TRY(jolt_table_upload(ctx, (const jolt_fr_t*)host, n, &t));
        } else {
            jolt_ints* v = nullptr;
            JOLT_TRY(jolt_ints_upload(ctx, host, kind, n, &v));
            const int32_t s = jolt_table_from_ints(ctx, v, 0, n, &t);
// ... 93 lines not shown
```

jolt_amd/csrc/msm_fixed.hip:

```cpp
#include <algorithm>
#include <cstdlib>

#include "ctx.hpp"
#include "msm_kernels.hip.h"
#include "srs.hpp"

using namespace jolt;
using namespace jolt::msmk;

struct MsmJob {
    size_t n = 0;
    int lane = 0, c = 0, W = 0;
    uint32_t nb = 0;
    int results = 1;
};

namespace {

constexpr int kLoBitsMin = 8;
static inline int fx_lo_bits(int c) { return c > 24 ? 11 : 8; }
constexpr uint32_t kFxHeavySeg = 128;
constexpr uint32_t kClasses = 512;
__device__ __forceinline__ uint32_t bucket_class(uint32_t count, uint32_t heavy_threshold) {
    return count > heavy_threshold ? 0u : (count < kClasses ? count : kClasses - 1);
}

__global__ __launch_bounds__(kBlock) void k_fx_next_window(const G1Affine* __restrict__ prev, G1Affine* __restrict__ next, size_t n, int c) {
    size_t i = (size_t)blockIdx.x * kBlock + threadIdx.x;
    if (i >= n) return;
    G1Jac p = g1_from_affine(ld_aff(prev + i));
    for (int k = 0; k < c; ++k) p = g1_double(p);
    next[i] = g1_to_affine(p);
}

JOLT_HD void fx_digits_of(Fr s , int c, int W, uint32_t* __restrict__ keys, size_t key_stride) {
    bool flip = false;
#pragma unroll
    for (int j = 7; j >= 0; --j) {
        const uint32_t half = ((uint32_t)FrParams::P[j] >> 1) | (j < 7 ? (uint32_t)FrParams::P[j + 1] << 31 : 0u);
        if (s.l[j] != half) { flip = s.l[j] > half; break; }
    }
    if (flip) {
        uint32_t br = 0;
#pragma unroll
        for (int j = 0; j < 8; ++j) s.l[j] = __builtin_subc((uint32_t)FrParams::P[j], s.l[j], br, &br);
    }
    const uint32_t B = 1u << (c - 1), fl = flip ? 0x80000000u : 0u;
    uint32_t carry = 0;
    for (int w = 0; w < W; ++w) {
        const int bit = w * c, limb = bit >> 5, off = bit & 31;
        const uint64_t two = (uint64_t)s.l[limb] | (limb + 1 < 8 ? (uint64_t)s.l[limb + 1] << 32 : 0ull);
        if (w + 1 < W) {
            uint32_t raw = ((uint32_t)(two >> off) & ((1u << c) - 1)) + carry;
            uint32_t mag, negf;
            if (raw > B) { mag = (1u << c) - raw; negf = 0x80000000u; carry = 1; }
            else { mag = raw; negf = 0u; carry = 0; }
            keys[(size_t)w * key_stride] = mag | (negf ^ fl);
        } else {
            keys[(size_t)w * key_stride] = (((uint32_t)(two >> off) & 0x7FFFFFFFu) + carry) | fl;
        }
    }
}
__global__ __launch_bounds__(kBlock) void k_fx_digits(const Fr* __restrict__ scalars, size_t n, int c, int W, uint32_t* __restrict__ keys) {
    size_t i = (size_t)blockIdx.x * kBlock + threadIdx.x;
    if (i >= n) return;
    fx_digits_of(from_mont(ld_fr(scalars + i)), c, W, keys + i, n);
}

template <int LO>
__global__ __launch_bounds__(kSortBlock) void k_fx_hist(const uint32_t* __restrict__ keys, size_t total, uint32_t nb1, uint32_t* __restrict__ hist1) {
    extern __shared__ uint32_t fx_sh[];
    for (uint32_t b = threadIdx.x; b < nb1; b += kSortBlock) fx_sh[b] = 0;
    __syncthreads();
    const size_t per = (total + gridDim.x - 1) / gridDim.x, lo = blockIdx.x * per, hi = lo + per < total ? lo + per : total;
    for (size_t base = lo; base < hi; base += kSortBlock) {
        size_t k = base + threadIdx.x;
        uint32_t mag = k < hi ? keys[k] & 0x7FFFFFFFu : 0u;
        WaveAgg ag = wave_aggregate(mag >> LO, mag != 0);
        if (ag.do_atomic) atomicAdd(&fx_sh[mag >> LO], ag.count);
    }
    __syncthreads();
    for (uint32_t b = threadIdx.x; b < nb1; b += kSortBlock) {
        uint32_t cnt = fx_sh[b];
        if (cnt) atomicAdd(&hist1[b], cnt);
    }
}
__global__ __launch_bounds__(kSortBlock) void k_fx_scan(const uint32_t* __restrict__ hist1, uint32_t nb1, uint32_t* __restrict__ offs1, uint32_t* __restrict__ cursor1,
                                                       uint32_t* __restrict__ info, const uint32_t* __restrict__ run_if = nullptr) {
    __shared__ uint32_t sm[kSortBlock];
    __shared__ uint32_t smax[kSortBlock];
    if (run_if && *run_if == 0) return;
    const uint32_t per = (nb1 + kSortBlock - 1) / kSortBlock;
    const uint32_t lo = min(threadIdx.x * per, nb1), hi = min(lo + per, nb1);
    uint32_t local = 0, mx = 0;
    for (uint32_t k = lo; k < hi; ++k) { local += hist1[k]; mx = max(mx, hist1[k]); }
    sm[threadIdx.x] = local;
    smax[threadIdx.x] = mx;
    __syncthreads();
// ... 739 lines not shown
    JOLT_TRY(fx_precompute_into(ctx, srs, window_bits, min_terms));
    constexpr size_t kMidN = (size_t)1 << 23, kMidMin = (size_t)1 << 19;
    if (window_bits == 0 && srs->n >= 4 * kMidN && srs->pre_c >= 23 && srs->pre_min_n > kMidMin && !srs->mid_tables) {
        jolt_srs* mt = new (std::nothrow) jolt_srs();
        if (!mt) return JOLT_ERR_OOM;
        mt->ctx = ctx;
        mt->pts = srs->pts;
        mt->n = kMidN;
        const int32_t s = fx_precompute_into(ctx, mt, 20, kMidMin);
        if (s != JOLT_OK) { delete mt; (void)hipGetLastError(); return JOLT_OK; }
        srs->mid_tables = mt;
    }
    return JOLT_OK;
}
static int32_t fx_precompute_into(jolt_ctx* ctx, jolt_srs* srs, uint32_t window_bits, size_t min_terms) {
    if (srs->n == 0) return JOLT_ERR_INVALID_ARG;
    int lg = 0;
    while (((size_t)2 << lg) <= srs->n) lg++;
    int c = window_bits ? (int)window_bits : (lg >= 24 ? 23 : std::max(kLoBitsMin + 1, std::min(24, lg - 2)));
    if (c <= kLoBitsMin || c > 26) return JOLT_ERR_UNSUPPORTED;
    const int W = (253 + c - 1) / c;
    const int shift = c * (W - 1) + 1;
    if (254 - shift > 31) return JOLT_ERR_UNSUPPORTED;
    auto limb32 = [](int j) -> uint64_t { return j < 8 ? (uint64_t)(uint32_t)FrParams::P[j] : 0ull; };
    const uint64_t top_max = ((limb32(shift >> 5) | (limb32((shift >> 5) + 1) << 32)) >> (shift & 31)) + 1;
    if (top_max >= ((uint64_t)1 << 31)) return JOLT_ERR_UNSUPPORTED;
    const uint32_t n_bucket_max = (uint32_t)std::max<uint64_t>((uint64_t)1 << (c - 1), top_max);
    if ((size_t)W * srs->n >= ((size_t)1 << 31)) return JOLT_ERR_UNSUPPORTED;
    G1Affine* pre = nullptr;
    hipError_t e = hipMalloc((void**)&pre, (size_t)W * srs->n * sizeof(G1Affine));
    if (e != hipSuccess) {
        (void)hipGetLastError();
        ctx->last_error = std::string("precompute windows: ") + hipGetErrorString(e);
        return e == hipErrorOutOfMemory ? JOLT_ERR_OOM : JOLT_ERR_HIP;
    }
    e = hipMemcpyAsync(pre, srs->pts, srs->n * sizeof(G1Affine), hipMemcpyDeviceToDevice, ctx->stream);
    const unsigned grid = (unsigned)((srs->n + kBlock - 1) / kBlock);
    for (int w = 1; w < W && e == hipSuccess; ++w) {
        hipLaunchKernelGGL(k_fx_next_window, dim3(grid), dim3(kBlock), 0, ctx->stream, (const G1Affine*)(pre + (size_t)(w - 1) * srs->n), pre + (size_t)w * srs->n, srs->n, c);
        e = hipGetLastError();
    }
    if (e == hipSuccess) {
        Fq thirty_two = Fq::zero();
        thirty_two.l[0] = 32;
        const size_t count = (size_t)W * srs->n;
        hipLaunchKernelGGL(k_fx_to_lform, dim3((unsigned)((count + kBlock - 1) / kBlock)), dim3(kBlock), 0, ctx->stream, pre, count, to_mont(thirty_two));
        e = hipGetLastError();
    }
    if (e == hipSuccess) e = hipStreamSynchronize(ctx->stream);
    if (e != hipSuccess) { (void)hipFree(pre); ctx->last_error = std::string("precompute windows: ") + hipGetErrorString(e); return JOLT_ERR_HIP; }
    srs->pre = pre;
    srs->pre_c = c;
    srs->pre_W = W;
    srs->pre_B = n_bucket_max;
    srs->pre_stride = srs->n;
    srs->pre_min_n = min_terms ? min_terms : std::max<size_t>((size_t)1 << (c - 2), 256);
    return JOLT_OK;
}

constexpr size_t kMsmHostEntries = 128;

static bool fx_capacity_model(size_t n, int c, int W, FxCapModel* m) {
    const int top_shift = c * (W - 1) + 1;
    if (254 - top_shift > 31 || top_shift < 1) return false;
    auto limb32 = [](int j) -> uint64_t { return j < 8 ? (uint64_t)(uint32_t)FrParams::P[j] : 0ull; };
    const uint64_t top_max = ((limb32(top_shift >> 5) | (limb32((top_shift >> 5) + 1) << 32)) >> (top_shift & 31)) + 1;
    if (top_max == 0 || top_max > 0xFFFFFFFFull) return false;
    m->n = (double)n;
    m->p_signed = 2.0 / (double)((uint64_t)1 << c) * (double)(W - 1);
    m->p_top = 1.0 / (double)top_max;
    m->half = 1u << (c - 1);
    m->top_max = (uint32_t)top_max;
    return true;
}
extern "C" int32_t jolt_host_fx_segment_capacity(uint64_t n, uint32_t window_bits, uint32_t segment, uint32_t* capacity) {
    if (!capacity || window_bits < 2 || window_bits > 26) return JOLT_ERR_INVALID_ARG;
    const int c = (int)window_bits, W = (253 + c - 1) / c;
    FxCapModel m;
    if (!fx_capacity_model((size_t)n, c, W, &m)) return JOLT_ERR_UNSUPPORTED;
    *capacity = fx_segment_capacity(m, segment, 1u << fx_lo_bits(c));
    return JOLT_OK;
}

int32_t jolt_internal_msm_fixed_enqueue(jolt_ctx* ctx, const jolt_srs* srs, const Fr* d_scalars, size_t n, int lane, MsmJob* job, size_t pair_shift) {
    const int c = srs->pre_c, W = srs->pre_W;
    const int lo_bits = fx_lo_bits(c);
    const uint32_t kSegBuckets = 1u << lo_bits;
    const uint32_t B = srs->pre_B;
    const uint32_t nb1 = (B >> lo_bits) + 1;
    const size_t total = (size_t)W * n;
    if (total >= ((size_t)1 << 32)) return JOLT_ERR_UNSUPPORTED;
    const size_t n_buckets = (size_t)nb1 * kSegBuckets;
    const uint32_t threads = (uint32_t)std::min<size_t>(std::max<size_t>(B / (size_t)24, std::min<size_t>(B, 4096)), 262144);
    const uint32_t nb = (threads + kBlock - 1) / kBlock;
    const uint32_t G = (B + nb * kBlock - 1) / (nb * kBlock);
    const bool grid_reduce = B >= (1u << 16);
    const uint32_t red_H = (B >> kRedS) + 1, red_chunks = (red_H + kRedRC - 1) / kRedRC, red_per_row = kRedCols / kRedCW;
    const size_t red_points = grid_reduce ? (size_t)red_chunks * kRedCols + (size_t)red_H * red_per_row + kRedCols + red_H + 64 : 0;
    const size_t avg = (total + B - 1) / B;
    const uint32_t heavy_threshold = (uint32_t)std::min<size_t>(std::max<size_t>(2 * kLaneCap, 4 * avg), kClasses - 2);
    const uint32_t heavy_cap = (uint32_t)(total / kFxHeavySeg + total / heavy_threshold + 16);
    const bool wide = W > kPartPerS;
    const bool soa = ctx->msm_fx_soa && lo_bits == 8 && ctx->msm_fx_partition == 2 && W <= kPartPerWide &&
                     ((nb1 + kGroupBins - 1) >> kGroupBits) <= (uint32_t)kPartBins &&
                     (wide ? sizeof(PartSharedN<kPartPerWide, kPartThreadsS>) : sizeof(PartSharedN<kPartPerS, kPartThreadsS>)) + 2048 <= ctx->max_lds_per_block;
    FxCapModel cap_model;
    size_t cap_total = 0;
    bool capacity = soa && ctx->msm_uniform_scalars && n >= ((size_t)1 << 16);
    if (capacity) {
        capacity = fx_capacity_model(n, c, W, &cap_model);
        const uint64_t top_max = cap_model.top_max;
        if (capacity) {
            uint64_t key_prev = ~0ull;
            uint32_t cap_prev = 0;
            for (uint32_t sgm = 0; sgm < nb1; ++sgm) {
                const uint64_t lo = (uint64_t)sgm * kSegBuckets, hi = lo + kSegBuckets;
                const uint64_t below_half = lo < cap_model.half ? std::min<uint64_t>(hi, cap_model.half) - lo : 0, below_top = lo < top_max ? std::min<uint64_t>(hi, top_max) - lo : 0;
                const uint64_t key = below_half | (below_top << 20) | ((uint64_t)(lo <= cap_model.half && cap_model.half < hi) << 40);
                if (key != key_prev) { cap_prev = fx_segment_capacity(cap_model, sgm, kSegBuckets); key_prev = key; }
                cap_total += cap_prev + 8;
            }
            capacity = cap_total < ((size_t)1 << 32) - 4096;
        }
    }
    const size_t span = capacity ? std::max(cap_total, total) : total;
    size_t off = 0;
    auto take = [&](size_t bytes) { size_t o = off; off += (bytes + 255) & ~(size_t)255; return o; };
    size_t o_keys = soa ? 0 : take(span * 4);
    const size_t o_entries = take(soa ? span * 5 + 512 : total * 8), o_hist = take((size_t)nb1 * 4), o_offs = take((size_t)nb1 * 4), o_cur = take((size_t)nb1 * 4),
                 o_info = take(256), o_buckets = take(n_buckets * sizeof(G1Jac)), o_part = take((size_t)nb * sizeof(G1Jac)), o_wsum = take(2 * sizeof(G1Jac)),
                 o_red = take(std::max<size_t>(red_points, 1) * sizeof(G1Jac)),
                 o_bhist = take(n_buckets * 4), o_boffs = take(n_buckets * 4), o_heavy = take((size_t)heavy_cap * 8), o_hcnt = take(256),
                 o_seg = take((size_t)heavy_cap * sizeof(G1Jac)), o_cls = take(kClasses * 4 * 2), o_order = take(n_buckets * 4),
                 o_grouped = take(soa ? span * 6 + 512 : (ctx->msm_fx_partition == 2 ? total * 8 : 256)), o_gcur = take(kPartBins * 4), o_glim = take(kPartBins * 4);
    if (soa) o_keys = o_grouped;
    const bool overlap_reduction = pair_shift != 0 && grid_reduce;
    const size_t o_buckets2 = take(overlap_reduction ? n_buckets * sizeof(G1Jac) : 256), o_red2 = take(overlap_reduction ? red_points * sizeof(G1Jac) : 256),
                 o_wsum2 = take(2 * sizeof(G1Jac));
    hipStream_t st = lane == 0 ? ctx->stream : ctx->side[lane - 1];
    if (off > ctx->msm_ws_cap[lane]) {
        if (ctx->msm_ws[lane]) {
            JOLT_HIP_TRY(ctx, hipStreamSynchronize(st));
            JOLT_HIP_TRY(ctx, hipFree(ctx->msm_ws[lane]));
            ctx->msm_ws[lane] = nullptr;
            ctx->msm_ws_cap[lane] = 0;
        }
        JOLT_HIP_TRY(ctx, hipMalloc(&ctx->msm_ws[lane], off));
        ctx->msm_ws_cap[lane] = off;
    }
    if (!ctx->msm_host[lane]) JOLT_HIP_TRY(ctx, hipHostMalloc(&ctx->msm_host[lane], kMsmHostEntries * sizeof(G1Jac), hipHostMallocDefault));
    char* ws = (char*)ctx->msm_ws[lane];
    uint32_t* keys = (uint32_t*)(ws + o_keys);
    uint64_t* entries = (uint64_t*)(ws + o_entries);
    uint32_t *hist1 = (uint32_t*)(ws + o_hist), *offs1 = (uint32_t*)(ws + o_offs), *cur1 = (uint32_t*)(ws + o_cur), *info = (uint32_t*)(ws + o_info);
    G1Jac *buckets = (G1Jac*)(ws + o_buckets), *part = (G1Jac*)(ws + o_part), *wsum = (G1Jac*)(ws + o_wsum), *seg = (G1Jac*)(ws + o_seg);
    uint32_t *hist = (uint32_t*)(ws + o_bhist), *offs = (uint32_t*)(ws + o_boffs), *heavy = (uint32_t*)(ws + o_heavy), *hcnt = (uint32_t*)(ws + o_hcnt);
    uint32_t *class_hist = (uint32_t*)(ws + o_cls), *class_cursor = class_hist + kClasses, *order = (uint32_t*)(ws + o_order);
    uint64_t* grouped = (uint64_t*)(ws + o_grouped);
    uint32_t* group_cursor = (uint32_t*)(ws + o_gcur);
    uint32_t* group_limit = (uint32_t*)(ws + o_glim);
    const uint32_t n_groups = (nb1 + kGroupBins - 1) >> kGroupBits;
    const size_t lds_bytes = (size_t)nb1 * sizeof(uint32_t);
    if (lds_bytes > ctx->max_lds_per_block) return JOLT_ERR_UNSUPPORTED;
    if (!ctx->msm_fx_attr_set) {
        hipError_t a1 = hipFuncSetAttribute((const void*)k_fx_hist<8>, hipFuncAttributeMaxDynamicSharedMemorySize, (int)ctx->max_lds_per_block);
        hipError_t a2 = hipFuncSetAttribute((const void*)k_fx_scatter<8>, hipFuncAttributeMaxDynamicSharedMemorySize, (int)ctx->max_lds_per_block);
        hipError_t a3 = hipFuncSetAttribute((const void*)k_fx_hist<11>, hipFuncAttributeMaxDynamicSharedMemorySize, (int)ctx->max_lds_per_block);
        hipError_t a4 = hipFuncSetAttribute((const void*)k_fx_scatter<11>, hipFuncAttributeMaxDynamicSharedMemorySize, (int)ctx->max_lds_per_block);
        (void)hipFuncSetAttribute((const void*)k_fx_segment_sort_staged<8>, hipFuncAttributeMaxDynamicSharedMemorySize, (int)(ctx->max_lds_per_block > 12288 ? ctx->max_lds_per_block - 12288 : 0));
        (void)hipGetLastError();
        hipError_t p1 = hipFuncSetAttribute((const void*)k_fx_partition_groups<8>, hipFuncAttributeMaxDynamicSharedMemorySize, (int)sizeof(PartShared));
        hipError_t p2 = hipFuncSetAttribute((const void*)k_fx_partition_groups<11>, hipFuncAttributeMaxDynamicSharedMemorySize, (int)sizeof(PartShared));
        hipError_t p3 = hipFuncSetAttribute((const void*)k_fx_partition_segments<8>, hipFuncAttributeMaxDynamicSharedMemorySize, (int)sizeof(PartShared));
        hipError_t p4 = hipFuncSetAttribute((const void*)k_fx_partition_segments<11>, hipFuncAttributeMaxDynamicSharedMemorySize, (int)sizeof(PartShared));
        hipError_t q1 = hipFuncSetAttribute((const void*)k_fx_hist_scalars<8>, hipFuncAttributeMaxDynamicSharedMemorySize, (int)ctx->max_lds_per_block);
        hipError_t q2 = hipFuncSetAttribute((const void*)k_fx_partition_groups_scalars<8>, hipFuncAttributeMaxDynamicSharedMemorySize, (int)sizeof(PartSharedN<kPartPerS, kPartThreadsS>));
        (void)hipFuncSetAttribute((const void*)k_fx_hist_scalars<8, kPartPerWide>, hipFuncAttributeMaxDynamicSharedMemorySize, (int)ctx->max_lds_per_block);
        (void)hipFuncSetAttribute((const void*)k_fx_partition_groups_scalars<8, kPartPerWide>, hipFuncAttributeMaxDynamicSharedMemorySize, (int)sizeof(PartSharedN<kPartPerWide, kPartThreadsS>));
        (void)hipGetLastError();
        hipError_t q3 = hipFuncSetAttribute((const void*)k_fx_partition_segments_soa<8>, hipFuncAttributeMaxDynamicSharedMemorySize, (int)sizeof(PartSharedN<kPartPer>));
        (void)hipFuncSetAttribute((const void*)k_fx_segment_sort_staged<8, true>, hipFuncAttributeMaxDynamicSharedMemorySize, (int)(ctx->max_lds_per_block > 12288 ? ctx->max_lds_per_block - 12288 : 0));
        (void)hipGetLastError();
        if (q1 != hipSuccess || q2 != hipSuccess || q3 != hipSuccess) ctx->msm_fx_soa = false;
        if (p1 != hipSuccess || p2 != hipSuccess || p3 != hipSuccess || p4 != hipSuccess) {
            (void)hipGetLastError();
            ctx->msm_fx_partition = 1;
        }
        if (a1 != hipSuccess || a2 != hipSuccess || a3 != hipSuccess || a4 != hipSuccess) {
            (void)hipGetLastError();
            if (lds_bytes > 64 * 1024) return JOLT_ERR_UNSUPPORTED;
        }
        ctx->msm_fx_attr_set = true;
    }
    const unsigned gn = (unsigned)((n + kBlock - 1) / kBlock);
    const unsigned slices = (unsigned)std::max<size_t>(1, std::min<size_t>((size_t)ctx->num_cus * 2, total / 16384));
    const unsigned hist_grid = (unsigned)std::max<size_t>(1, std::min<size_t>((size_t)ctx->num_cus * 2, n / 4096));
    auto hist_from_scalars = [&](const uint32_t* run_if) {
        if (wide) hipLaunchKernelGGL((k_fx_hist_scalars<8, kPartPerWide>), dim3(hist_grid), dim3(kSortBlock), lds_bytes, st, d_scalars, n, c, W, nb1, hist1, run_if);
        else hipLaunchKernelGGL(k_fx_hist_scalars<8>, dim3(hist_grid), dim3(kSortBlock), lds_bytes, st, d_scalars, n, c, W, nb1, hist1, run_if);
    };
    if (capacity) {
        hipLaunchKernelGGL(k_fx_capacity_regions, dim3((nb1 + kBlock - 1) / kBlock), dim3(kBlock), 0, st, cap_model, nb1, kSegBuckets, hist1, info);
    } else if (soa) {
        JOLT_HIP_TRY(ctx, hipMemsetAsync(hist1, 0, (size_t)nb1 * 4, st));
        hist_from_scalars(nullptr);
    } else {
        JOLT_HIP_TRY(ctx, hipMemsetAsync(hist1, 0, (size_t)nb1 * 4, st));
        hipLaunchKernelGGL(k_fx_digits, dim3(gn), dim3(kBlock), 0, st, d_scalars, n, c, W, keys);
        if (lo_bits == 8) hipLaunchKernelGGL(k_fx_hist<8>, dim3(slices), dim3(kSortBlock), lds_bytes, st, (const uint32_t*)keys, total, nb1, hist1);
        else hipLaunchKernelGGL(k_fx_hist<11>, dim3(slices), dim3(kSortBlock), lds_bytes, st, (const uint32_t*)keys, total, nb1, hist1);
    }
    hipLaunchKernelGGL(k_fx_scan, dim3(1), dim3(kSortBlock), 0, st, (const uint32_t*)hist1, nb1, offs1, cur1, info);
    JOLT_HIP_TRY(ctx, hipGetLastError());
    JOLT_HIP_TRY(ctx, hipMemsetAsync(buckets, 0, n_buckets * sizeof(G1Jac), st));
    JOLT_HIP_TRY(ctx, hipMemsetAsync(hcnt, 0, 256, st));
    JOLT_HIP_TRY(ctx, hipMemsetAsync(class_hist, 0, kClasses * 4, st));
    const bool two_pass = ctx->msm_fx_partition == 2 && n_groups <= (uint32_t)kPartBins && sizeof(PartShared) + 2048 <= ctx->max_lds_per_block;
    const unsigned part_grid = (unsigned)std::max<size_t>(1, std::min<size_t>((size_t)ctx->num_cus * 2, (total + kPartTile - 1) / kPartTile));
    uint32_t* g_val = (uint32_t*)grouped;
    uint16_t* g_low = (uint16_t*)((char*)grouped + ((span * 4 + 255) & ~(size_t)255));
    uint32_t* s_val = (uint32_t*)entries;
    uint8_t* s_low = (uint8_t*)((char*)entries + ((span * 4 + 255) & ~(size_t)255));
    if (soa) {
        const unsigned grid_s = (unsigned)std::max<size_t>(1, std::min<size_t>((size_t)ctx->num_cus, (n + kPartThreadsS - 1) / kPartThreadsS));
        auto partition_passes = [&](bool regions, const uint32_t* run_if) {
            const uint32_t* glim = regions ? group_limit : nullptr;
            uint32_t* flag = regions ? info + 2 : nullptr;
            if (wide)
                hipLaunchKernelGGL((k_fx_partition_groups_scalars<8, kPartPerWide>), dim3(grid_s), dim3(kPartThreadsS), sizeof(PartSharedN<kPartPerWide, kPartThreadsS>), st, d_scalars, n, c, W,
                                   srs->pre_stride, n_groups, group_cursor, g_val, g_low, glim, flag, run_if);
            else
                hipLaunchKernelGGL(k_fx_partition_groups_scalars<8>, dim3(grid_s), dim3(kPartThreadsS), sizeof(PartSharedN<kPartPerS, kPartThreadsS>), st, d_scalars, n, c, W, srs->pre_stride,
                                   n_groups, group_cursor, g_val, g_low, glim, flag, run_if);
            hipLaunchKernelGGL(k_fx_partition_segments_soa<8>, dim3(part_grid), dim3(kPartThreads), sizeof(PartSharedN<kPartPer>), st, (const uint32_t*)g_val, (const uint16_t*)g_low,
                               (const uint32_t*)offs1, nb1, (const uint32_t*)info, cur1, s_val, s_low, regions ? (const uint32_t*)group_cursor : nullptr, glim,
                               regions ? (const uint32_t*)hist1 : nullptr, flag, run_if);
        };
        if (capacity) {
            hipLaunchKernelGGL(k_fx_group_regions, dim3(1), dim3(kPartBins), 0, st, (const uint32_t*)offs1, (const uint32_t*)hist1, nb1, n_groups, group_cursor, group_limit);
            partition_passes(true, nullptr);
            hipLaunchKernelGGL(k_fx_counts_from_cursors, dim3((nb1 + kBlock - 1) / kBlock), dim3(kBlock), 0, st, (const uint32_t*)offs1, (const uint32_t*)cur1, nb1, hist1, info);
            const uint32_t* flag = info + 2;
            hipLaunchKernelGGL(k_fx_clear_if, dim3((nb1 + kBlock - 1) / kBlock), dim3(kBlock), 0, st, hist1, nb1, flag);
            hist_from_scalars(flag);
            hipLaunchKernelGGL(k_fx_scan, dim3(1), dim3(kSortBlock), 0, st, (const uint32_t*)hist1, nb1, offs1, cur1, info, flag);
            hipLaunchKernelGGL(k_fx_group_cursors, dim3(1), dim3(kPartBins), 0, st, (const uint32_t*)offs1, n_groups, group_cursor, flag);
            partition_passes(false, flag);
        } else {
            hipLaunchKernelGGL(k_fx_group_cursors, dim3(1), dim3(kPartBins), 0, st, (const uint32_t*)offs1, n_groups, group_cursor);
            partition_passes(false, nullptr);
        }
    } else if (two_pass) {
        hipLaunchKernelGGL(k_fx_group_cursors, dim3(1), dim3(kPartBins), 0, st, (const uint32_t*)offs1, n_groups, group_cursor);
        if (lo_bits == 8) {
            hipLaunchKernelGGL(k_fx_partition_groups<8>, dim3(part_grid), dim3(kPartThreads), sizeof(PartShared), st, (const uint32_t*)keys, total, n, srs->pre_stride, n_groups,
                               group_cursor, grouped);
            hipLaunchKernelGGL(k_fx_partition_segments<8>, dim3(part_grid), dim3(kPartThreads), sizeof(PartShared), st, (const uint64_t*)grouped, (const uint32_t*)offs1, nb1,
                               (const uint32_t*)info, cur1, entries);
        } else {
            hipLaunchKernelGGL(k_fx_partition_groups<11>, dim3(part_grid), dim3(kPartThreads), sizeof(PartShared), st, (const uint32_t*)keys, total, n, srs->pre_stride, n_groups,
                               group_cursor, grouped);
            hipLaunchKernelGGL(k_fx_partition_segments<11>, dim3(part_grid), dim3(kPartThreads), sizeof(PartShared), st, (const uint64_t*)grouped, (const uint32_t*)offs1, nb1,
                               (const uint32_t*)info, cur1, entries);
        }
    } else if (lo_bits == 8) {
        hipLaunchKernelGGL(k_fx_scatter<8>, dim3(slices), dim3(kSortBlock), lds_bytes, st, (const uint32_t*)keys, total, n, srs->pre_stride, nb1, cur1, entries);
    } else {
        hipLaunchKernelGGL(k_fx_scatter<11>, dim3(slices), dim3(kSortBlock), lds_bytes, st, (const uint32_t*)keys, total, n, srs->pre_stride, nb1, cur1, entries);
    }
    if (lo_bits == 8) {
        const size_t lds_max = ctx->max_lds_per_block > 12288 ? ctx->max_lds_per_block - 12288 : 0;
        const size_t want = (2 * (total / nb1) + 2048) * 4;
        const size_t stage_bytes = std::min(lds_max, want);
        if (soa)
            hipLaunchKernelGGL((k_fx_segment_sort_staged<8, true>), dim3(nb1), dim3(kSegThreads), stage_bytes, st, (const uint32_t*)hist1, (const uint32_t*)offs1, (const uint64_t*)nullptr,
                               (const uint32_t*)s_val, (const uint8_t*)s_low, keys, hist, offs, heavy_threshold, heavy, hcnt, heavy_cap, class_hist, (uint32_t)(stage_bytes / 4));
        else
            hipLaunchKernelGGL((k_fx_segment_sort_staged<8, false>), dim3(nb1), dim3(kSegThreads), stage_bytes, st, (const uint32_t*)hist1, (const uint32_t*)offs1, (const uint64_t*)entries,
                               (const uint32_t*)nullptr, (const uint8_t*)nullptr, keys, hist, offs, heavy_threshold, heavy, hcnt, heavy_cap, class_hist, (uint32_t)(stage_bytes / 4));
    }
    else
        hipLaunchKernelGGL(k_fx_segment_sort<11>, dim3(nb1), dim3(kBlock), 0, st, (const uint32_t*)hist1, (const uint32_t*)offs1, (const uint64_t*)entries, keys, hist, offs,
                           heavy_threshold, heavy, hcnt, heavy_cap, class_hist);
    const unsigned gh = std::min<uint32_t>((heavy_cap + kBlock - 1) / kBlock, (uint32_t)ctx->num_cus * 64);
    hipLaunchKernelGGL(k_fx_order_scan, dim3(1), dim3(kClasses), 0, st, (const uint32_t*)class_hist, class_cursor);
    hipLaunchKernelGGL(k_fx_order, dim3((unsigned)((n_buckets + kBlock * kOrderPer - 1) / (kBlock * kOrderPer))), dim3(kBlock), 0, st, (const uint32_t*)hist, (uint32_t)n_buckets,
                       heavy_threshold, class_cursor, order);
    LformConsts lc;
    {
        Fq thirty_two = Fq::zero();
        thirty_two.l[0] = 32;
        lc.one_l = to_mont(thirty_two);
        lc.r256 = Fq::one();
    }
    const unsigned bucket_grid = (unsigned)((n_buckets + kBlock - 1) / kBlock);
    const int per_result = grid_reduce ? 2 : 1;
    if ((size_t)per_result * (pair_shift ? 2 : 1) > kMsmHostEntries) return JOLT_ERR_UNSUPPORTED;
    auto bucket_sums = [&](const G1Affine* bases, G1Jac* buckets) -> int32_t {
        const bool profile = ctx->fx_profile && ctx->ev_fx[0] && ctx->ev_fx[1];
        if (profile) JOLT_HIP_TRY(ctx, hipEventRecord(ctx->ev_fx[0], st));
        hipLaunchKernelGGL(k_fx_buckets_ordered_staged, dim3(bucket_grid), dim3(kBlock), 0, st, (const uint32_t*)order, (uint32_t)n_buckets, (const uint32_t*)hist,
                           (const uint32_t*)offs, (const uint32_t*)keys, bases, heavy_threshold, buckets, lc);
        if (profile) {
            JOLT_HIP_TRY(ctx, hipEventRecord(ctx->ev_fx[1], st));
            ctx->fx_profile_info = info;
            ctx->fx_profile_valid = true;
        }
        hipLaunchKernelGGL(k_fx_heavy_segments_staged, dim3(gh), dim3(kBlock), 0, st, (const uint32_t*)heavy, (const uint32_t*)hcnt, heavy_cap, (const uint32_t*)hist,
                           (const uint32_t*)offs, (const uint32_t*)keys, bases, seg, lc);
        hipLaunchKernelGGL(k_fx_heavy_combine, dim3(std::min<uint32_t>(gh, 2048)), dim3(kBlock), 0, st, (const uint32_t*)heavy, (const uint32_t*)hcnt, heavy_cap, (const uint32_t*)hist,
                           (const G1Jac*)seg, buckets);
        JOLT_HIP_TRY(ctx, hipGetLastError());
        return JOLT_OK;
    };
    auto reduction = [&](const G1Jac* buckets, size_t o_red, G1Jac* wsum, int slot, hipStream_t rs) -> int32_t {
        if (grid_reduce) {
            G1Jac* colpart = (G1Jac*)(ws + o_red);
            G1Jac* rowpart = colpart + (size_t)red_chunks * kRedCols;
            G1Jac* cols = rowpart + (size_t)red_H * red_per_row;
            G1Jac* rows = cols + kRedCols;
            G1Jac* small_part = rows + red_H;
            hipLaunchKernelGGL(k_fx_red_cols, dim3(kRedCols / kBlock, red_chunks), dim3(kBlock), 0, rs, (const G1Jac*)buckets, B, red_H, colpart);
            hipLaunchKernelGGL(k_fx_red_rows, dim3((red_H * red_per_row + kBlock - 1) / kBlock), dim3(kBlock), 0, rs, (const G1Jac*)buckets, B, red_H, rowpart);
            hipLaunchKernelGGL(k_fx_red_fold, dim3(kRedCols * 64 / kBlock), dim3(kBlock), 0, rs, (const G1Jac*)colpart, kRedCols, red_chunks, (size_t)kRedCols, (size_t)1, cols);
            hipLaunchKernelGGL(k_fx_red_fold, dim3((red_H * 64 + kBlock - 1) / kBlock), dim3(kBlock), 0, rs, (const G1Jac*)rowpart, red_H, red_per_row, (size_t)1, (size_t)red_per_row, rows);
            const uint32_t g_small = 8, nb_c = (kRedCols / g_small + kBlock - 1) / kBlock, nb_r = (red_H / g_small + kBlock) / kBlock;
            hipLaunchKernelGGL(k_msm_window_reduce, dim3(nb_c, 1), dim3(kBlock), 0, rs, (const G1Jac*)cols, kRedCols - 1, g_small, small_part);
            hipLaunchKernelGGL(k_msm_window_combine, dim3(1), dim3(64), 0, rs, (const G1Jac*)small_part, nb_c, wsum);
            if (red_H > 1) {
                hipLaunchKernelGGL(k_msm_window_reduce, dim3(nb_r, 1), dim3(kBlock), 0, rs, (const G1Jac*)rows, red_H - 1, g_small, small_part + 32);
                hipLaunchKernelGGL(k_msm_window_combine, dim3(1), dim3(64), 0, rs, (const G1Jac*)(small_part + 32), nb_r, wsum + 1);
            } else {
                JOLT_HIP_TRY(ctx, hipMemsetAsync(wsum + 1, 0, sizeof(G1Jac), rs));
            }
        } else {
            hipLaunchKernelGGL(k_msm_window_reduce, dim3(nb, 1), dim3(kBlock), 0, rs, (const G1Jac*)buckets, B, G, part);
            hipLaunchKernelGGL(k_msm_window_combine, dim3(1), dim3(64), 0, rs, (const G1Jac*)part, nb, wsum);
        }
        JOLT_HIP_TRY(ctx, hipGetLastError());
        JOLT_HIP_TRY(ctx, hipMemcpyAsync((G1Jac*)ctx->msm_host[lane] + slot, wsum, (size_t)per_result * sizeof(G1Jac), hipMemcpyDeviceToHost, rs));
        return JOLT_OK;
    };
    JOLT_TRY(bucket_sums((const G1Affine*)srs->pre, buckets));
    if (!pair_shift) {
        JOLT_TRY(reduction(buckets, o_red, wsum, 0, st));
    } else if (overlap_reduction) {
        if (!ctx->msm_aux_stream) JOLT_HIP_TRY(ctx, hipStreamCreateWithFlags(&ctx->msm_aux_stream, hipStreamNonBlocking));
        if (!ctx->ev_aux[lane][0]) for (hipEvent_t& ev : ctx->ev_aux[lane]) JOLT_HIP_TRY(ctx, hipEventCreateWithFlags(&ev, hipEventDisableTiming));
        G1Jac* buckets2 = (G1Jac*)(ws + o_buckets2);
        JOLT_HIP_TRY(ctx, hipEventRecord(ctx->ev_aux[lane][0], st));
        JOLT_HIP_TRY(ctx, hipStreamWaitEvent(ctx->msm_aux_stream, ctx->ev_aux[lane][0], 0));
        JOLT_TRY(reduction(buckets, o_red, wsum, 0, ctx->msm_aux_stream));
        JOLT_HIP_TRY(ctx, hipEventRecord(ctx->ev_aux[lane][1], ctx->msm_aux_stream));
        JOLT_HIP_TRY(ctx, hipMemsetAsync(buckets2, 0, n_buckets * sizeof(G1Jac), st));
        JOLT_TRY(bucket_sums((const G1Affine*)srs->pre + pair_shift, buckets2));
        JOLT_TRY(reduction(buckets2, o_red2, (G1Jac*)(ws + o_wsum2), per_result, st));
        JOLT_HIP_TRY(ctx, hipStreamWaitEvent(st, ctx->ev_aux[lane][1], 0));
    } else {
        JOLT_TRY(reduction(buckets, o_red, wsum, 0, st));
        JOLT_HIP_TRY(ctx, hipMemsetAsync(buckets, 0, n_buckets * sizeof(G1Jac), st));
        JOLT_TRY(bucket_sums((const G1Affine*)srs->pre + pair_shift, buckets));
        JOLT_TRY(reduction(buckets, o_red, wsum, per_result, st));
    }
    job->n = n;
    job->lane = lane;
    job->c = grid_reduce ? kRedS : 0;
    job->W = per_result;
    job->nb = nb;
    job->results = pair_shift ? 2 : 1;
    return JOLT_OK;
}

extern "C" int32_t jolt_host_fx_digits(const jolt_fr_t* scalar, uint32_t window_bits, uint32_t* keys_out, uint32_t* n_windows_out, uint32_t* buckets_out) {
    if (!scalar || !keys_out || window_bits < 2 || window_bits > 26) return JOLT_ERR_INVALID_ARG;
    const int c = (int)window_bits, W = (253 + c - 1) / c;
    const int shift = c * (W - 1) + 1;
    if (254 - shift > 31) return JOLT_ERR_UNSUPPORTED;
    auto limb32 = [](int j) -> uint64_t { return j < 8 ? (uint64_t)(uint32_t)FrParams::P[j] : 0ull; };
    const uint64_t top_max = ((limb32(shift >> 5) | (limb32((shift >> 5) + 1) << 32)) >> (shift & 31)) + 1;
    Fr s = fr_from_abi(scalar);
    if (!fr_is_canonical(s)) return JOLT_ERR_INVALID_ARG;
    fx_digits_of(from_mont(s), c, W, keys_out, 1);
    if (n_windows_out) *n_windows_out = (uint32_t)W;
    if (buckets_out) *buckets_out = (uint32_t)std::max<uint64_t>((uint64_t)1 << (c - 1), top_max);
    return JOLT_OK;
}


extern "C" int32_t jolt_msm_profile_buckets(jolt_ctx* ctx, int32_t enable) {
    if (!ctx) return JOLT_ERR_INVALID_ARG;
    if (enable && !ctx->ev_fx[0]) {
        JOLT_HIP_TRY(ctx, hipEventCreate(&ctx->ev_fx[0]));
        JOLT_HIP_TRY(ctx, hipEventCreate(&ctx->ev_fx[1]));
    }
    ctx->fx_profile = enable != 0;
    ctx->fx_profile_valid = false;
    return JOLT_OK;
}
extern "C" int32_t jolt_msm_profile_buckets_last(jolt_ctx* ctx, float* ms, uint64_t* additions) {
    if (!ctx || !ms || !additions) return JOLT_ERR_INVALID_ARG;
    if (!ctx->fx_profile_valid) { ctx->last_error = "no profiled fixed-base MSM since jolt_msm_profile_buckets"; return JOLT_ERR_INVALID_ARG; }
    JOLT_HIP_TRY(ctx, hipEventSynchronize(ctx->ev_fx[1]));
    JOLT_HIP_TRY(ctx, hipEventElapsedTime(ms, ctx->ev_fx[0], ctx->ev_fx[1]));
    uint32_t info[4] = {0, 0, 0, 0};
    JOLT_HIP_TRY(ctx, hipMemcpy(info, ctx->fx_profile_info, sizeof(info), hipMemcpyDeviceToHost));
    *additions = info[3] ? info[3] : info[1];
    return JOLT_OK;
}


namespace {
__global__ __launch_bounds__(256) void k_mad_peak(uint64_t* out, uint32_t a0, uint32_t b0, int iters) {
    uint32_t a = a0 + threadIdx.x, b = b0 ^ threadIdx.x;
    uint64_t acc[8];
#pragma unroll
    for (int k = 0; k < 8; ++k) acc[k] = k;
    for (int it = 0; it < iters; ++it) {
#pragma unroll
        for (int k = 0; k < 8; ++k) acc[k] = (uint64_t)a * (uint32_t)(b + k) + acc[k];
        a += (uint32_t)acc[0];
    }
    uint64_t s = 0;
#pragma unroll
    for (int k = 0; k < 8; ++k) s ^= acc[k];
    out[(size_t)blockIdx.x * blockDim.x + threadIdx.x] = s;
}
}
extern "C" int32_t jolt_ctx_measure_mad_peak(jolt_ctx* ctx, float target_ms, double* mads_per_s, float* timed_ms, uint32_t* launches) {
    if (!ctx || !mads_per_s || !(target_ms > 0.f) || target_ms > 5000.f) return JOLT_ERR_INVALID_ARG;
    JOLT_TRY(jolt_internal_join_side_writers(ctx));
    const int blocks = (int)ctx->num_cus * 8, iters = 4096;
    uint64_t* out = nullptr;
    JOLT_TRY(jolt_internal_dev_alloc(ctx, (size_t)blocks * 256 * sizeof(uint64_t), (void**)&out));
    hipEvent_t e0 = nullptr, e1 = nullptr;
    hipError_t e = hipEventCreate(&e0);
    if (e == hipSuccess) e = hipEventCreate(&e1);
    double best = 0.0;
    float total = 0.f;
    uint32_t count = 0;
    const double mads = (double)blocks * 256.0 * (double)iters * 8.0;
    if (e == hipSuccess) {
        hipLaunchKernelGGL(k_mad_peak, dim3(blocks), dim3(256), 0, ctx->stream, out, 12345u, 67891u, iters);
        e = hipStreamSynchronize(ctx->stream);
    }
    while (e == hipSuccess && total < target_ms && count < 10000) {
        e = hipEventRecord(e0, ctx->stream);
        hipLaunchKernelGGL(k_mad_peak, dim3(blocks), dim3(256), 0, ctx->stream, out, 12345u + count, 67891u, iters);
        if (e == hipSuccess) e = hipEventRecord(e1, ctx->stream);
        if (e == hipSuccess) e = hipEventSynchronize(e1);
        float ms = 0.f;
        if (e == hipSuccess) e = hipEventElapsedTime(&ms, e0, e1);
        if (e != hipSuccess || !(ms > 0.f)) break;
// ... 18 lines not shown
```

jolt_amd/ffi.py:

```python
import ctypes as C
import os

import numpy as np

_HERE = os.path.dirname(os.path.abspath(__file__))
LIB_PATH = os.path.join(_HERE, "libjolt_hip.so")

STATUS = {0: "ok", 1: "invalid argument", 2: "no device", 3: "oom", 4: "hip error", 5: "size mismatch", 6: "unsupported",
          7: "not fully bound", 8: "round check failed", 9: "srs too small", 10: "empty point", 11: "not invertible"}
ORDER_LOW_TO_HIGH, ORDER_HIGH_TO_LOW = 0, 1
MEMBER_FLAG_SKIP_ONE = 1
MEMBER_FLAG_BORROW_TABLES = 2


class JoltError(RuntimeError):
    def __init__(self, status, where, detail=""):
        self.status = status
        super().__init__(f"{where}: status {status} ({STATUS.get(status, '?')}) {detail}")


class MemberDesc(C.Structure):
    _fields_ = [("n_tables", C.c_uint32), ("n_terms", C.c_uint32), ("degree", C.c_uint32), ("order", C.c_int32),
                ("term_offsets", C.c_void_p), ("factors", C.c_void_p), ("coeffs", C.c_void_p)]

# ... 1112 lines not shown
    w = fr(w).reshape(-1, 4)
    co = np.ascontiguousarray(np.stack([fr(c) for c in coeffs])).reshape(-1, 4)
    st = np.ascontiguousarray(scale_tables, dtype=np.uint64).reshape(-1, 4)
    h = C.c_void_p()
    if shard_scale is not None:
        _ck(lib().jolt_member_create_lazy_ra_uniform_sharded(self.h, source.h, _p(st), C.c_uint32(V), C.c_uint32(F), _p(co), _p(w), C.c_size_t(w.shape[0]),
                                                             _p(fr(scale)) if scale is not None else None, _p(fr(shard_scale)), C.byref(h)),
            "jolt_member_create_lazy_ra_uniform_sharded", self)
    else:
        _ck(lib().jolt_member_create_lazy_ra_uniform(self.h, source.h, _p(st), C.c_uint32(V), C.c_uint32(F), _p(co), _p(w), C.c_size_t(w.shape[0]),
                                                     _p(fr(scale)) if scale is not None else None, C.byref(h)), "jolt_member_create_lazy_ra_uniform", self)
    m = Member(self, h, F + 1, V * F, True, False)
    m.n_evals = F
    m.uniform = True
    m._keepalive = [source]
    return m


def _member_lazy_booleanity(self, source, scale_tables, rho, w, scale=None):
    w = fr(w).reshape(-1, 4)
    st = np.ascontiguousarray(scale_tables, dtype=np.uint64).reshape(-1, 4)
    rh = np.ascontiguousarray(np.stack([fr(c) for c in rho])).reshape(-1, 4)
    h = C.c_void_p()
    _ck(lib().jolt_member_create_lazy_booleanity(self.h, source.h, _p(st), _p(rh), _p(w), C.c_size_t(w.shape[0]),
                                                 _p(fr(scale)) if scale is not None else None, C.byref(h)), "jolt_member_create_lazy_booleanity", self)
    m = Member(self, h, 3, rh.shape[0], True, False)
    m.n_evals = 2
    m._keepalive = [source]
    return m


Context.member_lazy_booleanity = _member_lazy_booleanity
Context.member_lazy_ra_uniform = _member_lazy_ra_uniform
Context.onehot = lambda self, indices, k: OneHot(self, indices, k)
Context.ints = lambda self, values, kind=None: Ints(self, values, kind)
Context.dory_commit_rows = _dory_commit_rows
Context.dory_commit_onehot = _dory_commit_onehot


DORY_COMBINE_WINDOW = 5


def dory_combine_ops_per_row(n_hints, window=DORY_COMBINE_WINDOW):
    windows = (254 + 1 + window - 1) // window
    return windows * (n_hints + (1 << (window - 1)) + window + 1)


def dory_onehot_hint(chunk_commitments):
    c = np.asarray(chunk_commitments, dtype=np.uint64)
    return np.ascontiguousarray(c.transpose(1, 0, 2)).reshape(-1, c.shape[2])


def _dory_fold_rows_grid(self, sources, onehot_scalars, dense, dense_scalars, log_k, sigma, left):
    hs = (C.c_void_p * max(len(sources), 1))(*[s.h for s in sources])
    ds = (C.c_void_p * max(len(dense), 1))(*[t.h for t in dense])
    osc = fr(np.stack([fr(c) for c in onehot_scalars])).reshape(-1, 4) if len(onehot_scalars) else None
    dsc = fr(np.stack([fr(c) for c in dense_scalars])).reshape(-1, 4) if len(dense_scalars) else None
    h = C.c_void_p()
    _ck(lib().jolt_dory_fold_rows_grid(self.h, hs if sources else None, C.c_size_t(len(sources)), _p(osc), ds if dense else None, C.c_size_t(len(dense)),
                                       _p(dsc), C.c_uint32(log_k), C.c_uint32(sigma), left.h, C.byref(h)), "jolt_dory_fold_rows_grid", self)
    return Table(self, h)


def _dory_combine_hints(self, hints, scalars):
    hs = [np.ascontiguousarray(h, dtype=np.uint64).reshape(-1, 12) for h in hints]
    n = len(hs)
    ptrs = (C.c_void_p * max(n, 1))(*[h.ctypes.data for h in hs])
    rows = (C.c_size_t * max(n, 1))(*[h.shape[0] for h in hs])
    sc = fr(np.stack([fr(c) for c in scalars])).reshape(-1, 4) if n else fr_array(1)
    width = max([h.shape[0] for h in hs], default=0)
    out = g1_array(max(width, 1))
    _ck(lib().jolt_dory_combine_hints(self.h, ptrs, rows, C.c_size_t(n), _p(sc), _p(out)), "jolt_dory_combine_hints", self)
    return out[:width]


def host_dory_combine_row(points, scalars):
    pts = np.ascontiguousarray(points, dtype=np.uint64).reshape(-1, 12)
    sc = fr(np.stack([fr(c) for c in scalars])).reshape(-1, 4) if pts.shape[0] else fr_array(1)
    out = g1_array(1)
    _ck(lib().jolt_host_dory_combine_row(_p(pts), _p(sc), C.c_size_t(pts.shape[0]), _p(out)), "jolt_host_dory_combine_row")
    return out[0]


Context.dory_fold_rows_grid = _dory_fold_rows_grid
Context.dory_combine_hints = _dory_combine_hints


def _table_op2(name):
    def f(self, a, b):
        h = C.c_void_p()
        _ck(getattr(lib(), name)(self.h, a.h, b.h, C.byref(h)), name, self)
        return Table(self, h)
    return f


def _tile(self, base, copies):
    h = C.c_void_p()
    _ck(lib().jolt_tile(self.h, base.h, C.c_size_t(copies), C.byref(h)), "jolt_tile", self)
    return Table(self, h)


def _replicate_stream_lsb(self, base):
    h = C.c_void_p()
    _ck(lib().jolt_replicate_stream_lsb(self.h, base.h, C.byref(h)), "jolt_replicate_stream_lsb", self)
    return Table(self, h)


def _rlc(self, tables, scalars):
    hs = (C.c_void_p * len(tables))(*[t.h for t in tables])
    sc = fr(scalars).reshape(-1, 4)
    h = C.c_void_p()
    _ck(lib().jolt_rlc(self.h, hs, C.c_size_t(len(tables)), _p(sc), C.byref(h)), "jolt_rlc", self)
    return Table(self, h)


Context.address_fold = _table_op2("jolt_address_fold")
Context.cycle_fold = _table_op2("jolt_cycle_fold")
Context.tile = _tile
Context.replicate_stream_lsb = _replicate_stream_lsb
Context.rlc = _rlc


def _table_from_ints(self, values, offset=0, length=None):
    length = values.count - offset if length is None else length
    h = C.c_void_p()
    _ck(lib().jolt_table_from_ints(self.h, values.h, C.c_size_t(offset), C.c_size_t(length), C.byref(h)), "jolt_table_from_ints", self)
    return Table(self, h)


def _grid_commit_onehot(self, srs, source):
    out = g1_array(source.n_polys)
    _ck(lib().jolt_grid_commit_onehot(self.h, srs.h, source.h, _p(out)), "jolt_grid_commit_onehot", self)
    return out


def _grid_commit_onehot_classes(self, srs, source, shift):
    out = g1_array(source.n_polys << shift)
    _ck(lib().jolt_grid_commit_onehot_classes(self.h, srs.h, source.h, C.c_uint32(shift), _p(out)), "jolt_grid_commit_onehot_classes", self)
    return out.reshape(1 << shift, source.n_polys, 12)


def _grid_joint_polynomial(self, sources, onehot_scalars, dense, dense_scalars, log_k):
    hs = (C.c_void_p * max(len(sources), 1))(*[s.h for s in sources])
    ds = (C.c_void_p * max(len(dense), 1))(*[t.h for t in dense])
    osc = fr(np.stack([fr(c) for c in onehot_scalars])).reshape(-1, 4) if len(onehot_scalars) else None
    dsc = fr(np.stack([fr(c) for c in dense_scalars])).reshape(-1, 4) if len(dense_scalars) else None
    h = C.c_void_p()
    _ck(lib().jolt_grid_joint_polynomial(self.h, hs if sources else None, C.c_size_t(len(sources)), _p(osc), ds if dense else None, C.c_size_t(len(dense)),
                                         _p(dsc), C.c_uint32(log_k), C.byref(h)), "jolt_grid_joint_polynomial", self)
    return Table(self, h)


def _grid_joint_polynomial_subtree(self, sources, onehot_scalars, dense, dense_scalars, log_k, rank, world):
    hs = (C.c_void_p * max(len(sources), 1))(*[s.h for s in sources])
    ds = (C.c_void_p * max(len(dense), 1))(*[t.h for t in dense])
    osc = fr(np.stack([fr(c) for c in onehot_scalars])).reshape(-1, 4) if len(onehot_scalars) else None
    dsc = fr(np.stack([fr(c) for c in dense_scalars])).reshape(-1, 4) if len(dense_scalars) else None
    h = C.c_void_p()
    _ck(lib().jolt_grid_joint_polynomial_subtree(self.h, hs if sources else None, C.c_size_t(len(sources)), _p(osc), ds if dense else None, C.c_size_t(len(dense)),
                                                 _p(dsc), C.c_uint32(log_k), C.c_int32(rank), C.c_int32(world), C.byref(h)), "jolt_grid_joint_polynomial_subtree", self)
    return Table(self, h)


def _trim(self):
    _ck(lib().jolt_ctx_trim(self.h), "jolt_ctx_trim", self)

# ... 782 lines not shown
```

rust/jolt-kernels-hip/src/ffi.rs:

```rust
#![allow(non_camel_case_types, clippy::too_many_arguments, clippy::missing_safety_doc)]
use core::ffi::{c_char, c_void};

pub const JOLT_HIP_ABI_VERSION: i32 = 1;

#[repr(C)]
#[derive(Clone, Copy, Debug, Default, PartialEq, Eq)]
pub struct jolt_fr_t {
    pub l: [u64; 4],
}
#[repr(C)]
#[derive(Clone, Copy, Debug, Default, PartialEq, Eq)]
pub struct jolt_fq_t {
    pub l: [u64; 4],
}
#[repr(C)]
#[derive(Clone, Copy, Debug, Default, PartialEq, Eq)]
pub struct jolt_g1_t {
    pub x: jolt_fq_t,
    pub y: jolt_fq_t,
    pub z: jolt_fq_t,
}
#[repr(C)]
pub struct jolt_ctx {
    _private: [u8; 0],
// ... 283 lines not shown
    pub fn jolt_onehot_from_rows_sentinel(ctx: *mut jolt_ctx, rows: *const jolt_rows, offset: usize, width: u32, shifts: *const u32, n_polys: usize, log_k: u32, cycles: usize, out: *mut *mut jolt_onehot) -> i32;
    pub fn jolt_member_create_lazy_booleanity(ctx: *mut jolt_ctx, source: *const jolt_onehot, scale_tables: *const jolt_fr_t, rho: *const jolt_fr_t, w: *const jolt_fr_t, n: usize, scale: *const jolt_fr_t, out: *mut *mut jolt_member) -> i32;
    pub fn jolt_ints_upload(ctx: *mut jolt_ctx, host: *const c_void, kind: i32, count: usize, out: *mut *mut jolt_ints) -> i32;
    pub fn jolt_ints_free(ctx: *mut jolt_ctx, values: *mut jolt_ints) -> i32;
    pub fn jolt_dory_commit_rows(ctx: *mut jolt_ctx, srs: *const jolt_srs, values: *const jolt_ints, row_width: usize, out: *mut jolt_g1_t) -> i32;
    pub fn jolt_dory_commit_onehot(ctx: *mut jolt_ctx, srs: *const jolt_srs, source: *const jolt_onehot, poly: usize, chunk_width: usize, out: *mut jolt_g1_t) -> i32;
    pub fn jolt_dory_fold_rows_grid(ctx: *mut jolt_ctx, sources: *const *const jolt_onehot, n_sources: usize, onehot_scalars: *const jolt_fr_t, dense: *const *mut jolt_table, n_dense: usize, dense_scalars: *const jolt_fr_t, log_k: u32, sigma: u32, left: *const jolt_table, out: *mut *mut jolt_table) -> i32;
    pub fn jolt_dory_combine_hints(ctx: *mut jolt_ctx, hints: *const *const jolt_g1_t, hint_rows: *const usize, n_hints: usize, scalars: *const jolt_fr_t, out: *mut jolt_g1_t) -> i32;
    pub fn jolt_host_dory_combine_row(points: *const jolt_g1_t, scalars: *const jolt_fr_t, n: usize, out: *mut jolt_g1_t) -> i32;
    pub fn jolt_table_from_ints(ctx: *mut jolt_ctx, values: *const jolt_ints, offset: usize, len: usize, out: *mut *mut jolt_table) -> i32;
    pub fn jolt_grid_commit_onehot(ctx: *mut jolt_ctx, srs: *const jolt_srs, source: *const jolt_onehot, out: *mut jolt_g1_t) -> i32;
    pub fn jolt_grid_joint_polynomial(ctx: *mut jolt_ctx, sources: *const *const jolt_onehot, n_sources: usize, onehot_scalars: *const jolt_fr_t, dense: *const *mut jolt_table, n_dense: usize, dense_scalars: *const jolt_fr_t, log_k: u32, out: *mut *mut jolt_table) -> i32;
    pub fn jolt_read_raf_create(ctx: *mut jolt_ctx, lookup_index: *const u64, table_index: *const u8, raf_flag: *const u8, cycles: usize, n_tables: u32, out: *mut *mut jolt_read_raf) -> i32;
    pub fn jolt_read_raf_destroy(ctx: *mut jolt_ctx, rr: *mut jolt_read_raf) -> i32;
    pub fn jolt_read_raf_cycles(rr: *const jolt_read_raf, cycles: *mut usize, n_tables: *mut u32) -> i32;
    pub fn jolt_read_raf_phase_scan(ctx: *mut jolt_ctx, rr: *mut jolt_read_raf, u: *const jolt_table, suffix_len: u32, address_bits: u32, canonical: i32, suffix_offsets: *const u32, suffix_kinds: *const u8, raf_out: *mut jolt_fr_t, suffix_out: *mut jolt_fr_t) -> i32;
    pub fn jolt_read_raf_condense(ctx: *mut jolt_ctx, rr: *mut jolt_read_raf, u: *mut jolt_table, v_table: *const jolt_fr_t, shift: u32) -> i32;
    pub fn jolt_read_raf_cycle_tables(ctx: *mut jolt_ctx, rr: *mut jolt_read_raf, table_values: *const jolt_fr_t, raf_interleaved: *const jolt_fr_t, raf_identity: *const jolt_fr_t, v_tables: *const jolt_fr_t, phases: u32, address_bits: u32, ra_count: u32, combined_out: *mut *mut jolt_table, ra_out: *mut *mut jolt_table) -> i32;
    pub fn jolt_host_suffix_mle(kind: u32, lo: u64, hi: u64, len: u32, out: *mut u64) -> i32;
    pub fn jolt_lookup_table_count() -> u32;
    pub fn jolt_lookup_prefix_count() -> u32;
    pub fn jolt_lookup_table_suffixes(kind: u32, kinds_out: *mut u8, n_out: *mut u32) -> i32;
    pub fn jolt_lookup_table_prefixes(kind: u32, prefixes_out: *mut u8, n_out: *mut u32) -> i32;
    pub fn jolt_lookup_suffix_layout(offsets_out: *mut u32, kinds_out: *mut u8) -> i32;
    pub fn jolt_host_lookup_prefix_default_checkpoints(out: *mut jolt_fr_t) -> i32;
    pub fn jolt_host_lookup_prefix_evaluate(prefix: u32, checkpoints: *const jolt_fr_t, b: u32, b_len: u32, suffix_len: u32, out: *mut jolt_fr_t) -> i32;
    pub fn jolt_host_lookup_prefix_table(prefix: u32, checkpoints: *const jolt_fr_t, b_len: u32, suffix_len: u32, out: *mut jolt_fr_t) -> i32;
    pub fn jolt_host_lookup_table_combine(kind: u32, prefixes: *const jolt_fr_t, suffixes: *const jolt_fr_t, out: *mut jolt_fr_t) -> i32;
    pub fn jolt_host_read_raf_address_create(gamma: *const jolt_fr_t, table_present: *const u8, canonical: i32, out: *mut *mut jolt_read_raf_address) -> i32;
    pub fn jolt_host_read_raf_address_destroy(h: *mut jolt_read_raf_address) -> i32;
    pub fn jolt_host_read_raf_address_init_phase(h: *mut jolt_read_raf_address, phase: u32, raf_sums: *const jolt_fr_t, suffix_sums: *const jolt_fr_t) -> i32;
    pub fn jolt_host_read_raf_address_message(h: *mut jolt_read_raf_address, previous_claim: *const jolt_fr_t, evals_out: *mut jolt_fr_t) -> i32;
    pub fn jolt_host_read_raf_address_bind(h: *mut jolt_read_raf_address, challenge: *const jolt_fr_t, phase_done: *mut i32) -> i32;
    pub fn jolt_host_read_raf_address_bind_message(h: *mut jolt_read_raf_address, challenge: *const jolt_fr_t, previous_claim: *const jolt_fr_t, evals_out: *mut jolt_fr_t) -> i32;
    pub fn jolt_host_read_raf_address_prove_phase(h: *mut jolt_read_raf_address, claim: *mut jolt_fr_t, r#fn: jolt_round_transcript_fn, user: *mut c_void, test_transcript: *mut jolt_host_transcript, coeffs_out: *mut jolt_fr_t, challenges_out: *mut jolt_fr_t) -> i32;
    pub fn jolt_host_read_raf_address_v_table(h: *const jolt_read_raf_address, phase: u32, out: *mut jolt_fr_t) -> i32;
    pub fn jolt_host_read_raf_address_finish(h: *const jolt_read_raf_address, table_values: *mut jolt_fr_t, raf_interleaved: *mut jolt_fr_t, raf_identity: *mut jolt_fr_t) -> i32;
    pub fn jolt_r1cs_uniskip_sums(ctx: *mut jolt_ctx, inputs: *const *mut jolt_table, n_inputs: usize, eq: *const jolt_table, a_weights: *const jolt_fr_t, b_weights: *const jolt_fr_t, n_nodes: usize, out: *mut jolt_fr_t) -> i32;
    pub fn jolt_r1cs_materialize(ctx: *mut jolt_ctx, inputs: *const *mut jolt_table, n_inputs: usize, a_weights: *const jolt_fr_t, b_weights: *const jolt_fr_t, az_out: *mut *mut jolt_table, bz_out: *mut *mut jolt_table) -> i32;
    pub fn jolt_tables_evaluate(ctx: *mut jolt_ctx, tables: *const *mut jolt_table, k: usize, point: *const jolt_fr_t, n: usize, out: *mut jolt_fr_t) -> i32;
    pub fn jolt_r1cs_uniskip_sums_small(ctx: *mut jolt_ctx, inputs: *const *const jolt_ints, n_inputs: usize, eq: *const jolt_table, n_streams: u32, a_weights: *const i64, b_weights: *const i64, n_nodes: usize, out: *mut jolt_fr_t) -> i32;
    pub fn jolt_r1cs_materialize_small(ctx: *mut jolt_ctx, inputs: *const *const jolt_ints, n_inputs: usize, n_streams: u32, a_weights: *const jolt_fr_t, b_weights: *const jolt_fr_t, az_out: *mut *mut jolt_table, bz_out: *mut *mut jolt_table) -> i32;
    pub fn jolt_ints_evaluate(ctx: *mut jolt_ctx, columns: *const *const jolt_ints, k: usize, point: *const jolt_fr_t, n: usize, out: *mut jolt_fr_t) -> i32;
    pub fn jolt_host_small_scalar_dot(values: *const jolt_fr_t, scalars: *const u64, n: usize, out: *mut jolt_fr_t) -> i32;
    pub fn jolt_rw_matrix_create(ctx: *mut jolt_ctx, addresses: *const u64, pre_values: *const u64, post_values: *const u64, cycles: usize, inc: *const jolt_table, val_init: *const jolt_table, tau_low: *const jolt_fr_t, gamma: *const jolt_fr_t, out: *mut *mut jolt_rw_matrix) -> i32;
    pub fn jolt_rw_matrix_create_resident(ctx: *mut jolt_ctx, addresses: *const jolt_ints, pre_values: *const jolt_ints, post_values: *const jolt_ints, inc: *const jolt_table, val_init: *const jolt_table, tau_low: *const jolt_fr_t, gamma: *const jolt_fr_t, out: *mut *mut jolt_rw_matrix) -> i32;
    pub fn jolt_registers_rw_create(ctx: *mut jolt_ctx, regs: *const jolt_onehot, rs1_val: *const jolt_ints, rs2_val: *const jolt_ints, rd_pre: *const jolt_ints, rd_post: *const jolt_ints, inc: *const jolt_table, r_cycle: *const jolt_fr_t, gamma: *const jolt_fr_t, out: *mut *mut jolt_rw_matrix) -> i32;
    pub fn jolt_registers_rw_prove_round(m: *mut jolt_rw_matrix, bind: *const jolt_fr_t, evals_out: *mut jolt_fr_t, aux_out: *mut jolt_fr_t) -> i32;
    pub fn jolt_registers_rw_final_values(m: *mut jolt_rw_matrix, out: *mut jolt_fr_t) -> i32;
    pub fn jolt_registers_rw_download(m: *mut jolt_rw_matrix, rows: *mut u64, cols: *mut u64, val: *mut jolt_fr_t, ra: *mut jolt_fr_t, wa: *mut jolt_fr_t, prev: *mut u64, next: *mut u64) -> i32;
    pub fn jolt_rw_matrix_prove_round(m: *mut jolt_rw_matrix, bind: *const jolt_fr_t, evals_out: *mut jolt_fr_t, aux_out: *mut jolt_fr_t) -> i32;
    pub fn jolt_rw_matrix_finish(m: *mut jolt_rw_matrix, bind: *const jolt_fr_t) -> i32;
    pub fn jolt_rw_matrix_final_values(m: *mut jolt_rw_matrix, out: *mut jolt_fr_t) -> i32;
    pub fn jolt_key_index_create(ctx: *mut jolt_ctx, keys: *const jolt_ints, k: u64, out: *mut *mut jolt_key_index) -> i32;
    pub fn jolt_key_index_size(index: *const jolt_key_index, cycles: *mut usize, k: *mut u64, items: *mut u32) -> i32;
    pub fn jolt_key_index_pushforward(ctx: *mut jolt_ctx, index: *const jolt_key_index, weights: *const *mut jolt_table, n_weights: usize, out: *mut *mut jolt_table) -> i32;
    pub fn jolt_key_index_last_value(ctx: *mut jolt_ctx, index: *const jolt_key_index, values: *const jolt_ints, init: *const jolt_table, out: *mut *mut jolt_table) -> i32;
    pub fn jolt_key_index_destroy(ctx: *mut jolt_ctx, index: *mut jolt_key_index) -> i32;
    pub fn jolt_rw_matrix_hold_row(m: *mut jolt_rw_matrix) -> i32;
    pub fn jolt_rw_matrix_bind(m: *mut jolt_rw_matrix, bind: *const jolt_fr_t) -> i32;
    pub fn jolt_rw_matrix_export_row(m: *mut jolt_rw_matrix, cap: usize, cols: *mut u64, prev: *mut u64, next: *mut u64, val: *mut jolt_fr_t, ra: *mut jolt_fr_t, wa: *mut jolt_fr_t, inc_out: *mut jolt_fr_t, scalar_out: *mut jolt_fr_t, n_out: *mut usize) -> i32;
    pub fn jolt_rw_matrix_create_merged(ctx: *mut jolt_ctx, registers: i32, log_rows: usize, log_k: usize, n: usize, rows: *const u64, cols: *const u64, prev: *const u64, next: *const u64, val: *const jolt_fr_t, ra: *const jolt_fr_t, wa: *const jolt_fr_t, inc: *const jolt_fr_t, val_init: *const jolt_table, w: *const jolt_fr_t, scalar: *const jolt_fr_t, gamma: *const jolt_fr_t, out: *mut *mut jolt_rw_matrix) -> i32;
    pub fn jolt_rw_matrix_len(m: *const jolt_rw_matrix, entries: *mut usize) -> i32;
    pub fn jolt_rw_matrix_download(m: *mut jolt_rw_matrix, rows: *mut u64, cols: *mut u64, val: *mut jolt_fr_t, ra: *mut jolt_fr_t, prev: *mut jolt_fr_t, next: *mut jolt_fr_t) -> i32;
    pub fn jolt_rw_matrix_destroy(m: *mut jolt_rw_matrix) -> i32;
    pub fn jolt_comm_unique_id(rccl_path: *const c_char, out: *mut u8) -> i32;
    pub fn jolt_comm_create(ctx: *mut jolt_ctx, rccl_path: *const c_char, unique_id: *const u8, rank: i32, world: i32, out: *mut *mut jolt_comm) -> i32;
    pub fn jolt_comm_destroy(comm: *mut jolt_comm) -> i32;
    pub fn jolt_comm_world(comm: *const jolt_comm, rank: *mut i32, world: *mut i32) -> i32;
    pub fn jolt_comm_all_gather_host(comm: *mut jolt_comm, local: *const c_void, bytes: usize, gathered: *mut c_void) -> i32;
    pub fn jolt_comm_all_gather_device(comm: *mut jolt_comm, d_local: *const c_void, bytes: usize, d_gathered: *mut c_void) -> i32;
    pub fn jolt_comm_all_gather_table(comm: *mut jolt_comm, local: *const jolt_table, n: usize, gathered: *mut jolt_table) -> i32;
    pub fn jolt_comm_gather_round_sums(user: *mut c_void, local: *const jolt_fr_t, count: usize, gathered: *mut jolt_fr_t) -> i32;
    pub fn jolt_shm_create(name: *const c_char, rank: i32, world: i32, max_bytes: usize, out: *mut *mut jolt_shm) -> i32;
    pub fn jolt_shm_create_nonce(name: *const c_char, nonce: u64, rank: i32, world: i32, max_bytes: usize, out: *mut *mut jolt_shm) -> i32;
    pub fn jolt_shm_destroy(shm: *mut jolt_shm) -> i32;
    pub fn jolt_shm_all_gather(shm: *mut jolt_shm, local: *const c_void, bytes: usize, gathered: *mut c_void) -> i32;
    pub fn jolt_shm_gather_round_sums(user: *mut c_void, local: *const jolt_fr_t, count: usize, gathered: *mut jolt_fr_t) -> i32;
    pub fn jolt_round_group_pack_tables(ctx: *mut jolt_ctx, members: *const *mut jolt_member, n_members: usize, entries: usize, dst: *mut jolt_table) -> i32;
    pub fn jolt_tail_interleave(ctx: *mut jolt_ctx, gathered: *const jolt_table, world: usize, n_tables: usize, entries: usize, dst: *mut jolt_table) -> i32;
    pub fn jolt_round_group_final_values(ctx: *mut jolt_ctx, members: *const *mut jolt_member, n_members: usize, out: *mut jolt_fr_t, capacity: usize) -> i32;
    pub fn jolt_host_hyperkzg_commit(ctx: *mut jolt_ctx, srs: *const jolt_srs, evals: *const jolt_table, out: *mut jolt_g1_t) -> i32;
    pub fn jolt_host_hyperkzg_open(ctx: *mut jolt_ctx, srs: *const jolt_srs, evals: *const jolt_table, point: *const jolt_fr_t, ell: usize, transcript_label: u64, com: *mut jolt_g1_t, w: *mut jolt_g1_t, v: *mut jolt_fr_t, challenges_out: *mut jolt_fr_t) -> i32;
    pub fn jolt_host_hyperkzg_open_with_transcript(ctx: *mut jolt_ctx, srs: *const jolt_srs, evals: *const jolt_table, point: *const jolt_fr_t, ell: usize, r#fn: jolt_open_transcript_fn, user: *mut c_void, com: *mut jolt_g1_t, w: *mut jolt_g1_t, v: *mut jolt_fr_t, challenges_out: *mut jolt_fr_t) -> i32;
    pub fn jolt_host_hyperkzg_open_with_levels(ctx: *mut jolt_ctx, srs: *const jolt_srs, evals: *const jolt_table, point: *const jolt_fr_t, ell: usize, transcript_label: u64, r#fn: jolt_open_transcript_fn, user: *mut c_void, known_levels: *const jolt_g1_t, n_known: usize, com: *mut jolt_g1_t, w: *mut jolt_g1_t, v: *mut jolt_fr_t, challenges_out: *mut jolt_fr_t) -> i32;
    pub fn jolt_msm_g1_table_range(ctx: *mut jolt_ctx, srs: *const jolt_srs, base_offset: usize, scalars: *const jolt_table, scalar_offset: usize, n: usize, out: *mut jolt_g1_t) -> i32;
    pub fn jolt_msm_g1_window(ctx: *mut jolt_ctx, srs: *const jolt_srs, base_offset: usize, kind: i32, host: *const c_void, n: usize, acc: *const jolt_g1_t, out: *mut jolt_g1_t) -> i32;
    pub fn jolt_grid_commit_onehot_range(ctx: *mut jolt_ctx, srs: *const jolt_srs, source: *const jolt_onehot, cycle_lo: usize, cycle_hi: usize, out: *mut jolt_g1_t) -> i32;
    pub fn jolt_grid_commit_onehot_classes(ctx: *mut jolt_ctx, srs: *const jolt_srs, source: *const jolt_onehot, shift: u32, out: *mut jolt_g1_t) -> i32;
    pub fn jolt_host_hyperkzg_open_sharded(ctx: *mut jolt_ctx, srs: *const jolt_srs, evals: *const jolt_table, point: *const jolt_fr_t, ell: usize, transcript_label: u64, rank: i32, world: i32, gather: jolt_gather_fn, user: *mut c_void, com: *mut jolt_g1_t, w: *mut jolt_g1_t, v: *mut jolt_fr_t, challenges_out: *mut jolt_fr_t) -> i32;
    pub fn jolt_host_owned_terms(n: usize, block: usize, rank: i32, world: i32, out: *mut usize) -> i32;
    pub fn jolt_srs_setup_from_secret_blocks(ctx: *mut jolt_ctx, beta: *const jolt_fr_t, count_global: usize, g1: *const jolt_g1_t, block: usize, rank: i32, world: i32, out: *mut *mut jolt_srs) -> i32;
    pub fn jolt_msm_g1_table_blocks(ctx: *mut jolt_ctx, srs: *const jolt_srs, scalars: *const jolt_table, n: usize, block: usize, rank: i32, world: i32, out: *mut jolt_g1_t) -> i32;
    pub fn jolt_host_hyperkzg_open_sharded_blocks(ctx: *mut jolt_ctx, srs: *const jolt_srs, evals: *const jolt_table, point: *const jolt_fr_t, ell: usize, transcript_label: u64, rank: i32, world: i32, block: usize, gather: jolt_gather_fn, user: *mut c_void, com: *mut jolt_g1_t, w: *mut jolt_g1_t, v: *mut jolt_fr_t, challenges_out: *mut jolt_fr_t) -> i32;
    pub fn jolt_host_subtree_owned_terms(n: usize, rank: i32, world: i32, out: *mut usize) -> i32;
    pub fn jolt_host_subtree_term_index(slot: usize, rank: i32, world: i32, out: *mut usize) -> i32;
    pub fn jolt_srs_setup_from_secret_subtree(ctx: *mut jolt_ctx, beta: *const jolt_fr_t, count_global: usize, g1: *const jolt_g1_t, rank: i32, world: i32, out: *mut *mut jolt_srs) -> i32;
    pub fn jolt_msm_g1_table_subtree(ctx: *mut jolt_ctx, srs: *const jolt_srs, scalars: *const jolt_table, n: usize, rank: i32, world: i32, out: *mut jolt_g1_t) -> i32;
    pub fn jolt_grid_joint_polynomial_subtree(ctx: *mut jolt_ctx, sources: *const *const jolt_onehot, n_sources: usize, onehot_scalars: *const jolt_fr_t, dense: *const *mut jolt_table, n_dense: usize, dense_scalars: *const jolt_fr_t, log_k: u32, rank: i32, world: i32, out: *mut *mut jolt_table) -> i32;
    pub fn jolt_host_hyperkzg_open_subtree(ctx: *mut jolt_ctx, srs: *const jolt_srs, evals: *const jolt_table, point: *const jolt_fr_t, ell: usize, transcript_label: u64, rank: i32, world: i32, gather: jolt_gather_fn, user: *mut c_void, com: *mut jolt_g1_t, w: *mut jolt_g1_t, v: *mut jolt_fr_t, challenges_out: *mut jolt_fr_t) -> i32;
    pub fn jolt_grid_hint_begin(ctx: *mut jolt_ctx, srs: *const jolt_srs, sources: *const *const jolt_onehot, n_sources: usize, levels: u32, background: i32, out: *mut *mut jolt_grid_hint) -> i32;
    pub fn jolt_grid_hint_wait(ctx: *mut jolt_ctx, hint: *mut jolt_grid_hint) -> i32;
    pub fn jolt_grid_hint_download(ctx: *mut jolt_ctx, hint: *mut jolt_grid_hint, level: u32, out: *mut jolt_g1_t) -> i32;
    pub fn jolt_grid_hint_free(ctx: *mut jolt_ctx, hint: *mut jolt_grid_hint) -> i32;
    pub fn jolt_host_hyperkzg_open_grid(ctx: *mut jolt_ctx, srs: *const jolt_srs, evals: *const jolt_table, point: *const jolt_fr_t, ell: usize, transcript_label: u64, r#fn: jolt_open_transcript_fn, user: *mut c_void, hint: *const jolt_grid_hint, levels: u32, onehot_scalars: *const jolt_fr_t, dense: *const *mut jolt_table, n_dense: usize, dense_scalars: *const jolt_fr_t, com: *mut jolt_g1_t, w: *mut jolt_g1_t, v: *mut jolt_fr_t, challenges_out: *mut jolt_fr_t) -> i32;
    pub fn jolt_stage_op_num_rounds(op: *const jolt_stage_op, rounds: *mut usize) -> i32;
    pub fn jolt_stage_op_degree(op: *const jolt_stage_op, degree: *mut usize) -> i32;
    pub fn jolt_stage_op_input_claim(op: *mut jolt_stage_op, claim: *mut jolt_fr_t) -> i32;
    pub fn jolt_stage_op_prove_round(op: *mut jolt_stage_op, bind: *const jolt_fr_t, round: usize, previous_claim: *const jolt_fr_t, coeffs_out: *mut jolt_fr_t, cap: usize, n_coeffs: *mut usize) -> i32;
    pub fn jolt_stage_op_finish_rounds(op: *mut jolt_stage_op, bind: *const jolt_fr_t) -> i32;
    pub fn jolt_stage_op_output_claims(op: *mut jolt_stage_op, out: *mut jolt_fr_t, cap: usize, n: *mut usize) -> i32;
    pub fn jolt_stage_op_kept(op: *const jolt_stage_op, key: *const c_char, out: *mut jolt_fr_t, cap: usize, n: *mut usize) -> i32;
    pub fn jolt_stage_op_window(parent: *mut jolt_stage_op, first: usize, n: usize, out: *mut *mut jolt_stage_op) -> i32;
    pub fn jolt_stage_op_destroy(op: *mut jolt_stage_op) -> i32;
    pub fn jolt_stage_spartan_uniskip_sums(ctx: *mut jolt_ctx, cols: *const *const jolt_ints, n_cols: usize, n_streams: u32, tau: *const jolt_fr_t, n_tau: usize, a_weights: *const i64, b_weights: *const i64, n_nodes: usize, sums_out: *mut jolt_fr_t) -> i32;
    pub fn jolt_stage_spartan_remainder_create(ctx: *mut jolt_ctx, cols: *const *const jolt_ints, n_cols: usize, n_streams: u32, a_weights: *const jolt_fr_t, b_weights: *const jolt_fr_t, tau: *const jolt_fr_t, n_tau: usize, scale: *const jolt_fr_t, out: *mut *mut jolt_stage_op) -> i32;
    pub fn jolt_stage_ram_read_write_create(ctx: *mut jolt_ctx, addresses: *const jolt_ints, pre_values: *const jolt_ints, post_values: *const jolt_ints, inc: *const jolt_ints, val_init: *const jolt_ints, tau_low: *const jolt_fr_t, gamma: *const jolt_fr_t, out: *mut *mut jolt_stage_op) -> i32;
    pub fn jolt_stage_registers_read_write_create(ctx: *mut jolt_ctx, regs: *const jolt_onehot, rs1_val: *const jolt_ints, rs2_val: *const jolt_ints, rd_pre: *const jolt_ints, rd_post: *const jolt_ints, inc: *const jolt_ints, r_cycle: *const jolt_fr_t, gamma: *const jolt_fr_t, out: *mut *mut jolt_stage_op) -> i32;
    pub fn jolt_stage_booleanity_address_create(ctx: *mut jolt_ctx, cols: *const jolt_onehot, reference_cycle: *const jolt_fr_t, n_cycle: usize, reference_address: *const jolt_fr_t, gamma: *const jolt_fr_t, out: *mut *mut jolt_stage_op) -> i32;
    pub fn jolt_stage_booleanity_cycle_create(ctx: *mut jolt_ctx, cols: *const jolt_onehot, r_address: *const jolt_fr_t, reference_address: *const jolt_fr_t, reference_cycle: *const jolt_fr_t, n_cycle: usize, gamma: *const jolt_fr_t, out: *mut *mut jolt_stage_op) -> i32;
    pub fn jolt_stage_hamming_weight_create(ctx: *mut jolt_ctx, cols: *const jolt_onehot, r_cycle: *const jolt_fr_t, n_cycle: usize, r_address: *const jolt_fr_t, virtualization_points: *const jolt_fr_t, gamma: *const jolt_fr_t, out: *mut *mut jolt_stage_op) -> i32;
    pub fn jolt_stage_instruction_read_raf_create(ctx: *mut jolt_ctx, rows: *mut jolt_read_raf, claim_columns: *const jolt_onehot, r_reduction: *const jolt_fr_t, n_vars: usize, gamma: *const jolt_fr_t, table_present: *const u8, ra_count: u32, out: *mut *mut jolt_stage_op) -> i32;
    pub fn jolt_stage_bytecode_read_raf_address_create(ctx: *mut jolt_ctx, pc_index: *const jolt_key_index, stage_points: *const jolt_fr_t, n_vars: usize, stage_values: *const jolt_fr_t, gamma: *const jolt_fr_t, first_pc: u64, entry_index: u64, out: *mut *mut jolt_stage_op) -> i32;
    pub fn jolt_stage_bytecode_read_raf_cycle_create(ctx: *mut jolt_ctx, address: *mut jolt_stage_op, pc_chunks: *const jolt_onehot, chunk_bits: u32, out: *mut *mut jolt_stage_op) -> i32;
    pub fn jolt_stage_ram_raf_evaluation_create(ctx: *mut jolt_ctx, ram_index: *const jolt_key_index, tau_low: *const jolt_fr_t, n_vars: usize, lowest_address: u64, out: *mut *mut jolt_stage_op) -> i32;
    pub fn jolt_stage_ram_output_check_create(ctx: *mut jolt_ctx, ram_index: *const jolt_key_index, post_values: *const jolt_ints, val_init: *const u64, val_io: *const u64, io_lo: u64, io_len: u64, r_address: *const jolt_fr_t, out: *mut *mut jolt_stage_op) -> i32;
    pub fn jolt_stage_member_create(ctx: *mut jolt_ctx, member: *mut jolt_member, flags: u32, out: *mut *mut jolt_stage_op) -> i32;
    pub fn jolt_stage_host_expr_create(tables: *const *const jolt_fr_t, len: usize, desc: *const jolt_member_desc, out: *mut *mut jolt_stage_op) -> i32;
    pub fn jolt_host_prove_batch_ops(ctx: *mut jolt_ctx, ops: *const *mut jolt_stage_op, n_ops: usize, input_claims: *const jolt_fr_t, coefficients: *const jolt_fr_t, offsets: *const usize, max_num_vars: usize, max_degree: usize, transcript_label: u64, challenge_mode: i32, out_polys: *mut jolt_fr_t, out_challenges: *mut jolt_fr_t, out_member_claims: *mut jolt_fr_t, out_final_claim: *mut jolt_fr_t) -> i32;
    pub fn jolt_host_stage_op_prove_alone(op: *mut jolt_stage_op, transcript: *mut jolt_host_transcript, claim: *mut jolt_fr_t, coeffs_out: *mut jolt_fr_t, stride: usize, n_coeffs_out: *mut u32, challenges_out: *mut jolt_fr_t) -> i32;
    pub fn jolt_host_prove_batch_ops_grouped(ctx: *mut jolt_ctx, ops: *const *mut jolt_stage_op, n_ops: usize, input_claims: *const jolt_fr_t, coefficients: *const jolt_fr_t, offsets: *const usize, max_num_vars: usize, max_degree: usize, transcript_label: u64, challenge_mode: i32, out_polys: *mut jolt_fr_t, out_challenges: *mut jolt_fr_t, out_member_claims: *mut jolt_fr_t, out_final_claim: *mut jolt_fr_t) -> i32;
}
```

Before: 11.32 million.

## Compute HyperKZG witness triple from one shifted MSM of a third quotient

The three opening witnesses were computed as a pair MSM on one quotient plus a separate full MSM on another polynomial, run on a side lane. Now one more quotient level (q3) is derived, and a single three-pass shifted MSM over q3 (shifts 0,1,2) feeds an algebraic host-side combination. That combination uses eight parallel scalar multiplications on CPU threads to rebuild the witnesses. The fixed-base enqueue is generalised to N shifts, with reductions alternating between two bucket sets on an aux stream. This trades the independent second MSM for extra passes over a slightly shorter scalar vector, plus more host scalar multiplications and thread spawns.

```diff
diff --git a/include/jolt_hip.h b/include/jolt_hip.h
--- a/include/jolt_hip.h
+++ b/include/jolt_hip.h
@@ -403,6 +403,8 @@
 int32_t jolt_host_hyperkzg_commit(jolt_ctx *ctx, const jolt_srs *srs, const jolt_table *evals, jolt_g1_t *out);
 int32_t jolt_host_hyperkzg_open(jolt_ctx *ctx, const jolt_srs *srs, const jolt_table *evals, const jolt_fr_t *point, size_t ell,
                                 uint64_t transcript_label, jolt_g1_t *com, jolt_g1_t *w, jolt_fr_t *v, jolt_fr_t *challenges_out);
+int32_t jolt_host_hyperkzg_witness_triple(const jolt_g1_t *c , const jolt_g1_t *g0, const jolt_g1_t *g1, const jolt_fr_t *r, const jolt_fr_t *a,
+                                          const jolt_fr_t *alpha, jolt_g1_t *w );
 
 typedef int32_t (*jolt_open_transcript_fn)(void *user, int32_t phase, const jolt_g1_t *points, size_t n_points, const jolt_fr_t *values, size_t n_values,
                                            jolt_fr_t *challenge_out);
diff --git a/jolt_amd/csrc/capi.hip b/jolt_amd/csrc/capi.hip
--- a/jolt_amd/csrc/capi.hip
+++ b/jolt_amd/csrc/capi.hip
@@ -119,7 +119,7 @@
     if (ctx->hint_stream) { (void)hipStreamSynchronize(ctx->hint_stream); (void)hipStreamDestroy(ctx->hint_stream); }
     if (ctx->msm_batch_ws) (void)hipFree(ctx->msm_batch_ws);
     if (ctx->msm_aux_stream) { (void)hipStreamSynchronize(ctx->msm_aux_stream); (void)hipStreamDestroy(ctx->msm_aux_stream); }
-    for (auto& pair : ctx->ev_aux) for (hipEvent_t e : pair) if (e) (void)hipEventDestroy(e);
+    for (auto& lane_events : ctx->ev_aux) for (hipEvent_t e : lane_events) if (e) (void)hipEventDestroy(e);
     if (ctx->msm_batch_host) (void)hipHostFree(ctx->msm_batch_host);
     if (ctx->ev_begin) (void)hipEventDestroy(ctx->ev_begin);
     for (hipEvent_t e : ctx->ev_fx)
diff --git a/jolt_amd/csrc/ctx.hpp b/jolt_amd/csrc/ctx.hpp
--- a/jolt_amd/csrc/ctx.hpp
+++ b/jolt_amd/csrc/ctx.hpp
@@ -50,9 +50,8 @@
     void* msm_batch_host = nullptr;
     size_t msm_batch_host_cap = 0;
     hipStream_t msm_aux_stream = nullptr;
-    hipEvent_t ev_aux[4][2] = {{nullptr, nullptr}, {nullptr, nullptr}, {nullptr, nullptr}, {nullptr, nullptr}};
+    hipEvent_t ev_aux[4][4] = {};
     bool msm_tables_pending = false;
-    void* msm_pending_one = nullptr;
     hipEvent_t ev_begin = nullptr, ev_end = nullptr;
     hipStream_t copy_stream = nullptr;
     hipEvent_t ev_copy_fork = nullptr;
diff --git a/jolt_amd/csrc/hyperkzg.hip b/jolt_amd/csrc/hyperkzg.hip
--- a/jolt_amd/csrc/hyperkzg.hip
+++ b/jolt_amd/csrc/hyperkzg.hip
@@ -1,5 +1,7 @@
 #include <algorithm>
 #include <cstdlib>
+#include <system_error>
+#include <thread>
 
 #include "ctx.hpp"
 #include "g1.hip.h"
@@ -12,10 +14,7 @@
 using namespace jolt;
 
 int32_t jolt_internal_msm(jolt_ctx* ctx, const jolt_srs* srs, const Fr* d_scalars, size_t n, G1Jac* out);
-int32_t jolt_internal_msm_pair_and_one(jolt_ctx* ctx, const jolt_srs* srs, const Fr* d_a, size_t n_a, size_t shift, const Fr* d_b, size_t n_b, G1Jac* out);
-int32_t jolt_internal_msm_one_begin(jolt_ctx* ctx, const jolt_srs* srs, size_t n_a, size_t shift, const Fr* d_b, size_t n_b);
-int32_t jolt_internal_msm_pair_finish(jolt_ctx* ctx, const jolt_srs* srs, const Fr* d_a, size_t n_a, size_t shift, G1Jac* out);
-void jolt_internal_msm_one_abandon(jolt_ctx* ctx);
+int32_t jolt_internal_msm_shifted(jolt_ctx* ctx, const jolt_srs* srs, const Fr* d_scalars, size_t n, const size_t* shifts, int n_shifts, G1Jac* out);
 int32_t jolt_internal_msm_many(jolt_ctx* ctx, const jolt_srs* srs, const Fr* const* d_scalars, const size_t* n, size_t count, G1Jac* out,
                                const size_t* base_offsets = nullptr);
 
@@ -381,6 +380,45 @@
         for (int r = 1; r < world; ++r) acc = g1_add(acc, all[(size_t)r * count + i]);
         out[i] = acc;
     }
+    return JOLT_OK;
+}
+
+static void witness_triple_combine(const G1Jac c[3], const G1Jac& g0, const G1Jac& g1, const Fr& r, const Fr& a, const Fr& alpha, G1Jac w[3]) {
+    const Fr u = mul(r, r);
+    enum { R_C1, U_C1, UR_C0, U_C0, A_G1, AR_G0, AU_G0, ALPHA_G0, N_MUL };
+    const G1Jac* const base[N_MUL] = {&c[1], &c[1], &c[0], &c[0], &g1, &g0, &g0, &g0};
+    const Fr scalar[N_MUL] = {from_mont(r), from_mont(u), from_mont(mul(u, r)), from_mont(u), from_mont(a), from_mont(mul(a, r)), from_mont(mul(a, u)), from_mont(alpha)};
+    G1Jac m[N_MUL];
+    std::thread workers[N_MUL];
+    for (int i = 0; i < N_MUL; ++i) {
+        auto one = [&m, &base, &scalar, i]() { m[i] = g1_mul_canonical(*base[i], scalar[i].l); };
+        try {
+            if (i + 1 < N_MUL) workers[i] = std::thread(one);
+        } catch (const std::system_error&) {
+        }
+        if (!workers[i].joinable()) one();
+    }
+    for (std::thread& t : workers) if (t.joinable()) t.join();
+    const G1Jac e = g1_add(g1_add(c[2], m[A_G1]), m[ALPHA_G0]);
+    const G1Jac o = g1_add(g1_add(m[R_C1], g1_neg(m[UR_C0])), m[AR_G0]);
+    const G1Jac even = g1_add(e, g1_neg(m[U_C1]));
+    w[0] = g1_add(even, o);
+    w[1] = g1_add(even, g1_neg(o));
+    w[2] = g1_add(g1_add(e, g1_neg(m[U_C0])), m[AU_G0]);
+}
+extern "C" int32_t jolt_host_hyperkzg_witness_triple(const jolt_g1_t* c, const jolt_g1_t* g0, const jolt_g1_t* g1, const jolt_fr_t* r, const jolt_fr_t* a,
+                                                     const jolt_fr_t* alpha, jolt_g1_t* w) {
+    if (!c || !g0 || !g1 || !r || !a || !alpha || !w) return JOLT_ERR_INVALID_ARG;
+    G1Jac pts[5], out[3];
+    std::memcpy(&pts[0], c, 3 * sizeof(G1Jac));
+    std::memcpy(&pts[3], g0, sizeof(G1Jac));
+    std::memcpy(&pts[4], g1, sizeof(G1Jac));
+    for (const G1Jac& p : pts) if (!g1_is_on_curve(p)) return JOLT_ERR_INVALID_ARG;
+    const Fr rr = fr_from_abi(r), aa = fr_from_abi(a), al = fr_from_abi(alpha);
+    if (!fr_is_canonical(rr) || !fr_is_canonical(aa) || !fr_is_canonical(al)) return JOLT_ERR_INVALID_ARG;
+    witness_triple_combine(pts, pts[3], pts[4], rr, aa, al, out);
+    for (G1Jac& p : out) if (g1_is_identity(p)) p = g1_identity();
+    std::memcpy(w, out, sizeof(out));
     return JOLT_OK;
 }
 
@@ -535,16 +573,10 @@
     G1Jac ws[3];
     bool paired = false;
     if (world == 1 && b_poly->len >= 4) {
-        jolt_table *h0 = nullptr, *qp = nullptr, *h2 = nullptr;
-        bool direct = false, begun = false;
-        s = jolt_hyperkzg_witness_poly(ctx, b_poly, &u_abi[2], &h2);
-        if (s == JOLT_OK) {
-            ctx->msm_full_width_scalars = ctx->msm_uniform_scalars = true;
-            const int32_t bs = jolt_internal_msm_one_begin(ctx, srs, b_poly->len - 2, 1, h2->data(), h2->len);
-            ctx->msm_full_width_scalars = ctx->msm_uniform_scalars = false;
-            if (bs == JOLT_OK) begun = true;
-            else if (bs != JOLT_ERR_UNSUPPORTED) s = bs;
-        }
+        jolt_table *h0 = nullptr, *qp = nullptr, *q3 = nullptr;
+        bool direct = false;
+        const size_t q3_len = b_poly->len - 3;
+        if (srs->n < 2 || q3_len > srs->n - 2) s = JOLT_ERR_SRS_TOO_SMALL;
         if (s == JOLT_OK && b_poly->len % 2 == 0) {
             s = jolt_internal_table_new(ctx, b_poly->len - 2, &qp);
             if (s == JOLT_OK) {
@@ -558,35 +590,36 @@
             s = jolt_hyperkzg_witness_poly(ctx, b_poly, &u_abi[0], &h0);
             if (s == JOLT_OK) s = jolt_hyperkzg_witness_poly(ctx, h0, &u_abi[1], &qp);
         }
-        Fr a_lo, q_lo;
-        G1Affine g0;
+        if (s == JOLT_OK) s = jolt_hyperkzg_witness_poly(ctx, qp, &u_abi[2], &q3);
+        static_assert(2 * sizeof(G1Affine) == 4 * sizeof(Fr), "two affine points take four result slots");
+        if (s == JOLT_OK) s = jolt_internal_ensure_scratch(ctx, 1, 8);
         if (s == JOLT_OK) {
-            hipError_t e = hipMemcpyAsync(&a_lo, direct ? b_poly->data() + 1 : h0->data(), sizeof(Fr), hipMemcpyDeviceToHost, ctx->stream);
-            if (e == hipSuccess) e = hipMemcpyAsync(&q_lo, direct ? qp->data() + 1 : qp->data(), sizeof(Fr), hipMemcpyDeviceToHost, ctx->stream);
-            if (e == hipSuccess) e = hipMemcpyAsync(&g0, srs->pts, sizeof(G1Affine), hipMemcpyDeviceToHost, ctx->stream);
-            if (e == hipSuccess) e = hipStreamSynchronize(ctx->stream);
-            if (e != hipSuccess) { ctx->last_error = std::string("hyperkzg open: ") + hipGetErrorString(e); s = JOLT_ERR_HIP; }
+            Fr* hr = ctx->h_results;
+            hipError_t e = hipMemcpyAsync(&hr[0], direct ? b_poly->data() + 1 : h0->data(), sizeof(Fr), hipMemcpyDeviceToHost, ctx->stream);
+            if (e == hipSuccess) e = hipMemcpyAsync(&hr[1], direct ? qp->data() + 1 : qp->data(), sizeof(Fr), hipMemcpyDeviceToHost, ctx->stream);
+            if (e == hipSuccess) e = hipMemcpyAsync(&hr[2], qp->data(), sizeof(Fr), hipMemcpyDeviceToHost, ctx->stream);
+            if (e == hipSuccess) e = hipMemcpyAsync(&hr[3], q3->data(), sizeof(Fr), hipMemcpyDeviceToHost, ctx->stream);
+            if (e == hipSuccess) e = hipMemcpyAsync(&hr[4], srs->pts, 2 * sizeof(G1Affine), hipMemcpyDeviceToHost, ctx->stream);
+            if (e != hipSuccess) { (void)hipStreamSynchronize(ctx->stream); ctx->last_error = std::string("hyperkzg open: ") + hipGetErrorString(e); s = JOLT_ERR_HIP; }
         }
         if (s == JOLT_OK) {
             G1Jac three[3];
+            const size_t shifts[3] = {0, 1, 2};
             ctx->msm_full_width_scalars = ctx->msm_uniform_scalars = true;
-            const int32_t ps = begun ? jolt_internal_msm_pair_finish(ctx, srs, qp->data(), qp->len, 1, three)
-                                     : jolt_internal_msm_pair_and_one(ctx, srs, qp->data(), qp->len, 1, h2->data(), h2->len, three);
+            const int32_t ts = jolt_internal_msm_shifted(ctx, srs, q3->data(), q3->len, shifts, 3, three);
             ctx->msm_full_width_scalars = ctx->msm_uniform_scalars = false;
-            begun = false;
-            if (ps == JOLT_OK) {
-                const Fr alpha = direct ? add(a_lo, mul(q_lo, u[2])) : add(a_lo, mul(q_lo, u[1])), r_can = from_mont(r), a_can = from_mont(alpha);
-                const G1Jac r_cq = g1_mul_canonical(three[0], r_can.l), base = g1_add(three[1], g1_mul_canonical(g1_from_affine(g0), a_can.l));
-                ws[0] = g1_add(base, r_cq);
-                ws[1] = g1_add(base, g1_neg(r_cq));
-                ws[2] = three[2];
+            if (ts == JOLT_OK) {
+                const Fr* hr = ctx->h_results;
+                G1Affine g01[2];
+                std::memcpy(g01, &hr[4], sizeof(g01));
+                const Fr alpha = add(hr[0], mul(hr[1], direct ? u[2] : u[1])), a = add(hr[2], mul(hr[3], u[2]));
+                witness_triple_combine(three, g1_from_affine(g01[0]), g1_from_affine(g01[1]), r, a, alpha, ws);
                 paired = true;
-            } else if (ps != JOLT_ERR_UNSUPPORTED) {
-                s = ps;
-            }
-        }
-        if (begun) jolt_internal_msm_one_abandon(ctx);
-        for (jolt_table* t : {h0, qp, h2}) if (t) jolt_table_free(ctx, t);
+            } else if (ts != JOLT_ERR_UNSUPPORTED) {
+                s = ts;
+            }
+        }
+        for (jolt_table* t : {h0, qp, q3}) if (t) jolt_table_free(ctx, t);
         if (s != JOLT_OK) { cleanup(b_poly); return s; }
     }
     if (!paired) {
diff --git a/jolt_amd/csrc/msm.hip b/jolt_amd/csrc/msm.hip
--- a/jolt_amd/csrc/msm.hip
+++ b/jolt_amd/csrc/msm.hip
@@ -43,7 +43,9 @@
     uint32_t nb = 0;
     int results = 1;
 };
-int32_t jolt_internal_msm_fixed_enqueue(jolt_ctx* ctx, const jolt_srs* srs, const Fr* d_scalars, size_t n, int lane, MsmJob* job, size_t pair_shift = 0);
+constexpr int kFxMaxShifts = 3;
+int32_t jolt_internal_msm_fixed_enqueue(jolt_ctx* ctx, const jolt_srs* srs, const Fr* d_scalars, size_t n, int lane, MsmJob* job, const size_t* shifts = nullptr,
+                                        int n_shifts = 0);
 namespace {
 struct MsmPlan {
     int c, W, L;
@@ -287,15 +289,17 @@
     }
     return JOLT_OK;
 }
-int32_t jolt_internal_msm_enqueue_pair(jolt_ctx* ctx, const jolt_srs* srs, const Fr* d_scalars, size_t n, size_t shift, int lane, MsmJob* job) {
+int32_t jolt_internal_msm_enqueue_shifted(jolt_ctx* ctx, const jolt_srs* srs, const Fr* d_scalars, size_t n, const size_t* shifts, int n_shifts, int lane, MsmJob* job) {
+    if (!shifts || n_shifts < 1 || n_shifts > kFxMaxShifts) return JOLT_ERR_INVALID_ARG;
     job->n = n;
     job->lane = lane;
-    job->results = 2;
-    if (shift > srs->n || n > srs->n - shift) return JOLT_ERR_SRS_TOO_SMALL;
+    job->results = n_shifts;
+    for (int k = 0; k < n_shifts; ++k)
+        if (shifts[k] > srs->n || n > srs->n - shifts[k]) return JOLT_ERR_SRS_TOO_SMALL;
     if (n == 0) return JOLT_OK;
     if (n >= ((size_t)1 << 31)) return JOLT_ERR_UNSUPPORTED;
     if (!(srs->pre && n >= srs->pre_min_n)) return JOLT_ERR_UNSUPPORTED;
-    return jolt_internal_msm_fixed_enqueue(ctx, srs, d_scalars, n, lane, job, shift);
+    return jolt_internal_msm_fixed_enqueue(ctx, srs, d_scalars, n, lane, job, shifts, n_shifts);
 }
 
 extern "C" int32_t jolt_host_owned_terms(size_t n, size_t block, int32_t rank, int32_t world, size_t* out) {
@@ -497,65 +501,13 @@
     return status;
 }
 
-int32_t jolt_internal_msm_pair_and_one(jolt_ctx* ctx, const jolt_srs* srs, const Fr* d_a, size_t n_a, size_t shift, const Fr* d_b, size_t n_b, G1Jac* out) {
-    if (shift > srs->n || n_a > srs->n - shift) return JOLT_ERR_SRS_TOO_SMALL;
-    if (n_a == 0 || !(srs->pre && n_a >= srs->pre_min_n) || ctx->msm_tables_pending) return JOLT_ERR_UNSUPPORTED;
-    JOLT_HIP_TRY(ctx, hipEventRecord(ctx->ev_fork, ctx->stream));
-    for (int k = 0; k < 3; ++k) JOLT_HIP_TRY(ctx, hipStreamWaitEvent(ctx->side[k], ctx->ev_fork, 0));
-    MsmJob pair, one;
-    int32_t status = jolt_internal_msm_enqueue_pair(ctx, srs, d_a, n_a, shift, 0, &pair);
-    if (status == JOLT_ERR_UNSUPPORTED) return status;
-    const int lane_b = ctx->msm_lanes > 1 ? 1 : 0;
-    if (status == JOLT_OK && lane_b == 0) status = jolt_internal_msm_collect(ctx, &pair, out);
-    if (status == JOLT_OK) status = jolt_internal_msm_enqueue(ctx, srs, d_b, n_b, lane_b, &one);
-    if (status == JOLT_OK && lane_b != 0) status = jolt_internal_msm_collect(ctx, &pair, out);
-    if (status == JOLT_OK) status = jolt_internal_msm_collect(ctx, &one, out + 2);
-    if (status != JOLT_OK)
-        for (int k = 0; k < 3; ++k) (void)hipStreamSynchronize(ctx->side[k]);
+int32_t jolt_internal_msm_shifted(jolt_ctx* ctx, const jolt_srs* srs, const Fr* d_scalars, size_t n, const size_t* shifts, int n_shifts, G1Jac* out) {
+    if (ctx->msm_tables_pending) return JOLT_ERR_UNSUPPORTED;
+    MsmJob job;
+    const int32_t status = jolt_internal_msm_enqueue_shifted(ctx, srs, d_scalars, n, shifts, n_shifts, 0, &job);
+    if (status == JOLT_OK) return jolt_internal_msm_collect(ctx, &job, out);
+    if (status != JOLT_ERR_UNSUPPORTED && status != JOLT_ERR_SRS_TOO_SMALL && status != JOLT_ERR_INVALID_ARG) (void)hipStreamSynchronize(ctx->stream);
     return status;
-}
-
-struct MsmPendingOne {
-    MsmJob job;
-};
-int32_t jolt_internal_msm_one_begin(jolt_ctx* ctx, const jolt_srs* srs, size_t n_a, size_t shift, const Fr* d_b, size_t n_b) {
-    if (shift > srs->n || n_a > srs->n - shift) return JOLT_ERR_SRS_TOO_SMALL;
-    if (n_a == 0 || !(srs->pre && n_a >= srs->pre_min_n) || ctx->msm_lanes < 2 || ctx->msm_pending_one || ctx->msm_tables_pending) return JOLT_ERR_UNSUPPORTED;
-    if ((size_t)srs->pre_W * n_a >= ((size_t)1 << 32)) return JOLT_ERR_UNSUPPORTED;
-    MsmPendingOne* p = new (std::nothrow) MsmPendingOne();
-    if (!p) return JOLT_ERR_OOM;
-    int32_t status = JOLT_OK;
-    hipError_t e = hipEventRecord(ctx->ev_fork, ctx->stream);
-    if (e == hipSuccess) e = hipStreamWaitEvent(ctx->side[0], ctx->ev_fork, 0);
-    if (e != hipSuccess) { ctx->last_error = hipGetErrorString(e); status = JOLT_ERR_HIP; }
-    if (status == JOLT_OK) status = jolt_internal_msm_enqueue(ctx, srs, d_b, n_b, 1, &p->job);
-    if (status != JOLT_OK) { (void)hipStreamSynchronize(ctx->side[0]); delete p; return status; }
-    ctx->msm_pending_one = p;
-    return JOLT_OK;
-}
-int32_t jolt_internal_msm_pair_finish(jolt_ctx* ctx, const jolt_srs* srs, const Fr* d_a, size_t n_a, size_t shift, G1Jac* out) {
-    MsmPendingOne* p = static_cast<MsmPendingOne*>(ctx->msm_pending_one);
-    if (!p) return JOLT_ERR_INVALID_ARG;
-    ctx->msm_pending_one = nullptr;
-    MsmJob pair;
-    int32_t status = jolt_internal_msm_enqueue_pair(ctx, srs, d_a, n_a, shift, 0, &pair);
-    if (status == JOLT_OK) status = jolt_internal_msm_collect(ctx, &pair, out);
-    else if (status == JOLT_ERR_UNSUPPORTED) {
-        status = jolt_internal_msm(ctx, srs, d_a, n_a, &out[0]);
-        const jolt_srs view = jolt_srs_range_view(*srs, shift);
-        if (status == JOLT_OK) status = jolt_internal_msm(ctx, &view, d_a, n_a, &out[1]);
-    }
-    const int32_t one_status = jolt_internal_msm_collect(ctx, &p->job, out + 2);
-    delete p;
-    if (status != JOLT_OK) (void)hipStreamSynchronize(ctx->side[0]);
-    return status != JOLT_OK ? status : one_status;
-}
-void jolt_internal_msm_one_abandon(jolt_ctx* ctx) {
-    MsmPendingOne* p = static_cast<MsmPendingOne*>(ctx->msm_pending_one);
-    if (!p) return;
-    ctx->msm_pending_one = nullptr;
-    (void)hipStreamSynchronize(ctx->side[0]);
-    delete p;
 }
 
 struct jolt_msm_pending {
@@ -565,7 +517,7 @@
 extern "C" int32_t jolt_msm_g1_tables_begin(jolt_ctx* ctx, const jolt_srs* srs, const jolt_table* const* scalars, const size_t* n, size_t count, jolt_msm_pending** out) {
     if (!ctx || !srs || !scalars || !n || !out || count == 0) return JOLT_ERR_INVALID_ARG;
     *out = nullptr;
-    if (count > 3 || (size_t)ctx->msm_lanes < count + 1 || ctx->msm_tables_pending || ctx->msm_pending_one) return JOLT_ERR_UNSUPPORTED;
+    if (count > 3 || (size_t)ctx->msm_lanes < count + 1 || ctx->msm_tables_pending) return JOLT_ERR_UNSUPPORTED;
     for (size_t i = 0; i < count; ++i) {
         if (!scalars[i]) return JOLT_ERR_INVALID_ARG;
         if (n[i] > scalars[i]->len) return JOLT_ERR_SIZE_MISMATCH;
diff --git a/jolt_amd/csrc/msm_fixed.hip b/jolt_amd/csrc/msm_fixed.hip
--- a/jolt_amd/csrc/msm_fixed.hip
+++ b/jolt_amd/csrc/msm_fixed.hip
@@ -14,6 +14,7 @@
     uint32_t nb = 0;
     int results = 1;
 };
+constexpr int kFxMaxShifts = 3;
 
 namespace {
 
@@ -919,7 +920,11 @@
     return JOLT_OK;
 }
 
-int32_t jolt_internal_msm_fixed_enqueue(jolt_ctx* ctx, const jolt_srs* srs, const Fr* d_scalars, size_t n, int lane, MsmJob* job, size_t pair_shift) {
+int32_t jolt_internal_msm_fixed_enqueue(jolt_ctx* ctx, const jolt_srs* srs, const Fr* d_scalars, size_t n, int lane, MsmJob* job, const size_t* shifts, int n_shifts) {
+    if (n_shifts < 0 || n_shifts > kFxMaxShifts || (n_shifts && !shifts)) return JOLT_ERR_INVALID_ARG;
+    const size_t shift_none = 0;
+    const int passes = n_shifts ? n_shifts : 1;
+    if (!n_shifts) shifts = &shift_none;
     const int c = srs->pre_c, W = srs->pre_W;
     const int lo_bits = fx_lo_bits(c);
     const uint32_t kSegBuckets = 1u << lo_bits;
@@ -971,7 +976,7 @@
                  o_seg = take((size_t)heavy_cap * sizeof(G1Jac)), o_cls = take(kClasses * 4 * 2), o_order = take(n_buckets * 4),
                  o_grouped = take(soa ? span * 6 + 512 : (ctx->msm_fx_partition == 2 ? total * 8 : 256)), o_gcur = take(kPartBins * 4), o_glim = take(kPartBins * 4);
     if (soa) o_keys = o_grouped;
-    const bool overlap_reduction = pair_shift != 0 && grid_reduce;
+    const bool overlap_reduction = passes > 1 && grid_reduce;
     const size_t o_buckets2 = take(overlap_reduction ? n_buckets * sizeof(G1Jac) : 256), o_red2 = take(overlap_reduction ? red_points * sizeof(G1Jac) : 256),
                  o_wsum2 = take(2 * sizeof(G1Jac));
     hipStream_t st = lane == 0 ? ctx->stream : ctx->side[lane - 1];
@@ -999,6 +1004,8 @@
     const uint32_t n_groups = (nb1 + kGroupBins - 1) >> kGroupBits;
     const size_t lds_bytes = (size_t)nb1 * sizeof(uint32_t);
     if (lds_bytes > ctx->max_lds_per_block) return JOLT_ERR_UNSUPPORTED;
+    const int per_result = grid_reduce ? 2 : 1;
+    static_assert((size_t)2 * kFxMaxShifts <= kMsmHostEntries, "msm_host takes the partial sums of every pass");
     if (!ctx->msm_fx_attr_set) {
         hipError_t a1 = hipFuncSetAttribute((const void*)k_fx_hist<8>, hipFuncAttributeMaxDynamicSharedMemorySize, (int)ctx->max_lds_per_block);
         hipError_t a2 = hipFuncSetAttribute((const void*)k_fx_scatter<8>, hipFuncAttributeMaxDynamicSharedMemorySize, (int)ctx->max_lds_per_block);
@@ -1131,8 +1138,6 @@
         lc.r256 = Fq::one();
     }
     const unsigned bucket_grid = (unsigned)((n_buckets + kBlock - 1) / kBlock);
-    const int per_result = grid_reduce ? 2 : 1;
-    if ((size_t)per_result * (pair_shift ? 2 : 1) > kMsmHostEntries) return JOLT_ERR_UNSUPPORTED;
     auto bucket_sums = [&](const G1Affine* bases, G1Jac* buckets) -> int32_t {
         const bool profile = ctx->fx_profile && ctx->ev_fx[0] && ctx->ev_fx[1];
         if (profile) JOLT_HIP_TRY(ctx, hipEventRecord(ctx->ev_fx[0], st));
@@ -1178,33 +1183,40 @@
         JOLT_HIP_TRY(ctx, hipMemcpyAsync((G1Jac*)ctx->msm_host[lane] + slot, wsum, (size_t)per_result * sizeof(G1Jac), hipMemcpyDeviceToHost, rs));
         return JOLT_OK;
     };
-    JOLT_TRY(bucket_sums((const G1Affine*)srs->pre, buckets));
-    if (!pair_shift) {
-        JOLT_TRY(reduction(buckets, o_red, wsum, 0, st));
-    } else if (overlap_reduction) {
+    if (!overlap_reduction) {
+        for (int k = 0; k < passes; ++k) {
+            if (k) JOLT_HIP_TRY(ctx, hipMemsetAsync(buckets, 0, n_buckets * sizeof(G1Jac), st));
+            JOLT_TRY(bucket_sums((const G1Affine*)srs->pre + shifts[k], buckets));
+            JOLT_TRY(reduction(buckets, o_red, wsum, k * per_result, st));
+        }
+    } else {
         if (!ctx->msm_aux_stream) JOLT_HIP_TRY(ctx, hipStreamCreateWithFlags(&ctx->msm_aux_stream, hipStreamNonBlocking));
         if (!ctx->ev_aux[lane][0]) for (hipEvent_t& ev : ctx->ev_aux[lane]) JOLT_HIP_TRY(ctx, hipEventCreateWithFlags(&ev, hipEventDisableTiming));
-        G1Jac* buckets2 = (G1Jac*)(ws + o_buckets2);
-        JOLT_HIP_TRY(ctx, hipEventRecord(ctx->ev_aux[lane][0], st));
-        JOLT_HIP_TRY(ctx, hipStreamWaitEvent(ctx->msm_aux_stream, ctx->ev_aux[lane][0], 0));
-        JOLT_TRY(reduction(buckets, o_red, wsum, 0, ctx->msm_aux_stream));
-        JOLT_HIP_TRY(ctx, hipEventRecord(ctx->ev_aux[lane][1], ctx->msm_aux_stream));
-        JOLT_HIP_TRY(ctx, hipMemsetAsync(buckets2, 0, n_buckets * sizeof(G1Jac), st));
-        JOLT_TRY(bucket_sums((const G1Affine*)srs->pre + pair_shift, buckets2));
-        JOLT_TRY(reduction(buckets2, o_red2, (G1Jac*)(ws + o_wsum2), per_result, st));
-        JOLT_HIP_TRY(ctx, hipStreamWaitEvent(st, ctx->ev_aux[lane][1], 0));
-    } else {
-        JOLT_TRY(reduction(buckets, o_red, wsum, 0, st));
-        JOLT_HIP_TRY(ctx, hipMemsetAsync(buckets, 0, n_buckets * sizeof(G1Jac), st));
-        JOLT_TRY(bucket_sums((const G1Affine*)srs->pre + pair_shift, buckets));
-        JOLT_TRY(reduction(buckets, o_red, wsum, per_result, st));
+        G1Jac* const set_buckets[2] = {buckets, (G1Jac*)(ws + o_buckets2)};
+        G1Jac* const set_wsum[2] = {wsum, (G1Jac*)(ws + o_wsum2)};
+        const size_t set_red[2] = {o_red, o_red2};
+        for (int k = 0; k < passes; ++k) {
+            const int set = k & 1;
+            if (k >= 2) JOLT_HIP_TRY(ctx, hipStreamWaitEvent(st, ctx->ev_aux[lane][2 * set + 1], 0));
+            if (k) JOLT_HIP_TRY(ctx, hipMemsetAsync(set_buckets[set], 0, n_buckets * sizeof(G1Jac), st));
+            JOLT_TRY(bucket_sums((const G1Affine*)srs->pre + shifts[k], set_buckets[set]));
+            if (k + 1 < passes) {
+                JOLT_HIP_TRY(ctx, hipEventRecord(ctx->ev_aux[lane][2 * set], st));
+                JOLT_HIP_TRY(ctx, hipStreamWaitEvent(ctx->msm_aux_stream, ctx->ev_aux[lane][2 * set], 0));
+                JOLT_TRY(reduction(set_buckets[set], set_red[set], set_wsum[set], k * per_result, ctx->msm_aux_stream));
+                JOLT_HIP_TRY(ctx, hipEventRecord(ctx->ev_aux[lane][2 * set + 1], ctx->msm_aux_stream));
+            } else {
+                JOLT_TRY(reduction(set_buckets[set], set_red[set], set_wsum[set], k * per_result, st));
+                JOLT_HIP_TRY(ctx, hipStreamWaitEvent(st, ctx->ev_aux[lane][2 * ((k - 1) & 1) + 1], 0));
+            }
+        }
     }
     job->n = n;
     job->lane = lane;
     job->c = grid_reduce ? kRedS : 0;
     job->W = per_result;
     job->nb = nb;
-    job->results = pair_shift ? 2 : 1;
+    job->results = passes;
     return JOLT_OK;
 }
 
diff --git a/jolt_amd/ffi.py b/jolt_amd/ffi.py
--- a/jolt_amd/ffi.py
+++ b/jolt_amd/ffi.py
@@ -1218,6 +1218,14 @@
     return out[0]
 
 
+def host_hyperkzg_witness_triple(c, g0, g1, r, a, alpha):
+    cs = np.ascontiguousarray(c, dtype=np.uint64).reshape(3, 12)
+    p0, p1 = (np.ascontiguousarray(p, dtype=np.uint64).reshape(12) for p in (g0, g1))
+    out = g1_array(3)
+    _ck(lib().jolt_host_hyperkzg_witness_triple(_p(cs), _p(p0), _p(p1), _p(fr(r)), _p(fr(a)), _p(fr(alpha)), _p(out)), "jolt_host_hyperkzg_witness_triple")
+    return out
+
+
 Context.dory_fold_rows_grid = _dory_fold_rows_grid
 Context.dory_combine_hints = _dory_combine_hints
 
diff --git a/rust/jolt-kernels-hip/src/ffi.rs b/rust/jolt-kernels-hip/src/ffi.rs
--- a/rust/jolt-kernels-hip/src/ffi.rs
+++ b/rust/jolt-kernels-hip/src/ffi.rs
@@ -389,6 +389,7 @@
     pub fn jolt_round_group_final_values(ctx: *mut jolt_ctx, members: *const *mut jolt_member, n_members: usize, out: *mut jolt_fr_t, capacity: usize) -> i32;
     pub fn jolt_host_hyperkzg_commit(ctx: *mut jolt_ctx, srs: *const jolt_srs, evals: *const jolt_table, out: *mut jolt_g1_t) -> i32;
     pub fn jolt_host_hyperkzg_open(ctx: *mut jolt_ctx, srs: *const jolt_srs, evals: *const jolt_table, point: *const jolt_fr_t, ell: usize, transcript_label: u64, com: *mut jolt_g1_t, w: *mut jolt_g1_t, v: *mut jolt_fr_t, challenges_out: *mut jolt_fr_t) -> i32;
+    pub fn jolt_host_hyperkzg_witness_triple(c: *const jolt_g1_t, g0: *const jolt_g1_t, g1: *const jolt_g1_t, r: *const jolt_fr_t, a: *const jolt_fr_t, alpha: *const jolt_fr_t, w: *mut jolt_g1_t) -> i32;
     pub fn jolt_host_hyperkzg_open_with_transcript(ctx: *mut jolt_ctx, srs: *const jolt_srs, evals: *const jolt_table, point: *const jolt_fr_t, ell: usize, r#fn: jolt_open_transcript_fn, user: *mut c_void, com: *mut jolt_g1_t, w: *mut jolt_g1_t, v: *mut jolt_fr_t, challenges_out: *mut jolt_fr_t) -> i32;
     pub fn jolt_host_hyperkzg_open_with_levels(ctx: *mut jolt_ctx, srs: *const jolt_srs, evals: *const jolt_table, point: *const jolt_fr_t, ell: usize, transcript_label: u64, r#fn: jolt_open_transcript_fn, user: *mut c_void, known_levels: *const jolt_g1_t, n_known: usize, com: *mut jolt_g1_t, w: *mut jolt_g1_t, v: *mut jolt_fr_t, challenges_out: *mut jolt_fr_t) -> i32;
     pub fn jolt_msm_g1_table_range(ctx: *mut jolt_ctx, srs: *const jolt_srs, base_offset: usize, scalars: *const jolt_table, scalar_offset: usize, n: usize, out: *mut jolt_g1_t) -> i32;
```

Result: faster. 11.58 million (median of 6 runs) (+2.3%).
